# hguo/ftk

Hardware: NVIDIA B200
Metric: space_time_simplices_tested_per_sec (higher is better)
Workload: dtype f64+int64

## Files before the change

### ftk_b200/csrc/context.cpp

```cpp
#include <algorithm>
#include <cfloat>
#include <chrono>
#include <cmath>
#include <cstdio>
#include <cstdlib>
#include <cstring>
#include <deque>
#include <string>
#include <thread>
#include <atomic>
#include <vector>

#include <memory>
#include "kernels.h"
#include "online.h"
#include "curves.h"

using namespace ftkb;

namespace {

thread_local std::string g_create_error;

struct Layer {
  double *S = nullptr, *V = nullptr, *J = nullptr;
  bool ownS = false, ownV = false, ownJ = false;
  int slot = 0;
  bool res_pending = false;
  uint4 *cells = nullptr;
  bool cells_valid = false;
  bool cells_foreign = false;
};

}

template <class T>
struct NoInitAlloc : std::allocator<T> {
  template <class U> struct rebind { using other = NoInitAlloc<U>; };
  template <class U, class... A>
  void construct(U *q, A &&...a) {
    if constexpr (sizeof...(A) > 0) ::new ((void *)q) U(std::forward<A>(a)...);
  }
};
template <class T> using RawVec = std::vector<T, NoInitAlloc<T>>;

struct ftkb_ctx {
  ftkb_config cfg{};
  int n = 0;
  size_t nvert = 0;
  uint64_t ncore = 0;
  int n_ord = 0, n_int = 0;
  cudaStream_t stream = nullptr;
  cudaEvent_t ev[8] = {nullptr, nullptr, nullptr, nullptr, nullptr, nullptr, nullptr, nullptr};
  bool derive_timed = false;
  std::string error;

  bool slab = false;
  void *d_f32 = nullptr;
  size_t f32_cap = 0;
  std::deque<Layer> layers;
  std::vector<double *> freeS, freeV, freeJ;
  int current_timestep = 0;
  double resolution = DBL_MAX;
  double factor = 1.0;
  int nbits = 0;
  int next_slot = 0;
  int sm_count = 148;
  bool cellsV = true;
  bool keys2d = true;
  std::vector<uint4 *> freeCells;
  std::vector<uint4 *> exportedCells;
  size_t ncells = 0;
  bool fused3d = false;

  unsigned long long *d_scalars = nullptr;
  unsigned long long *h_scalars = nullptr;
  static constexpr int SLOT_WL = 8, SLOT_PT = 9, SLOT_UQ = 10, SLOT_POISON = 11, SLOT_WL2 = 12, SLOT_TICKET = 13, SLOT_POISON2 = 14, NSLOTS = 16;

  struct Pending {
    int ring = 0, evset = 0, pops = 0, nbits = 0, wl_sel = 0;
    uint64_t seq = 0, npts_before = 0, pt_cap = 0;
    bool has_next = false;
    int res_slots[2] = {-1, -1};
  };
  bool defer = true;
  std::deque<Pending> pend;
  std::deque<Layer> limbo;
  unsigned long long *h_ring = nullptr;
  static constexpr int RING = 4;
  uint64_t step_seq = 0;
  bool primed = false;
  int wl_sel = 0;
  cudaEvent_t dev[2][3] = {{nullptr, nullptr, nullptr}, {nullptr, nullptr, nullptr}};
  bool push_d2h_outstanding = false;
  uint64_t wl_hint = 1 << 16;
  cudaEvent_t ev_input = nullptr;
  cudaStream_t producer = nullptr;
  cudaStream_t stream2 = nullptr;
  cudaEvent_t ev_join = nullptr;
  bool debug_timing = false;
  double gap_ms = 0; uint64_t gap_n = 0, last_confirmed_seq = 0;
  std::vector<float> gaps, tl_scan_end, tl_test_end;
  cudaEvent_t dbg_prev = nullptr; bool dbg_prev_valid = false;
  double host_wait_us = 0, host_enq_us = 0; uint64_t host_wait_n = 0, host_enq_n = 0;
  bool last_test_overlapped = false;
  bool has_producer = false;

  unsigned long long *d_wl = nullptr;
  unsigned long long *d_wl2 = nullptr;
  int last_wl_sel = 0;
  uint64_t wl_cap = 0, last_wl = 0;
  ftkb_point *d_pts = nullptr;
  uint64_t pt_cap = 0, npts = 0;
  uint64_t max_step_points = 0;
  std::vector<ftkb_point *> retired_pts;

  struct Scratch { void *p = nullptr; size_t cap = 0; bool in_slab = false; };
  void *fz_slab = nullptr;
  size_t fz_slab_cap = 0;
  Scratch fz[14];
  void *grow_stage = nullptr;
  size_t grow_stage_cap = 0;

  bool sorted = false, traced = false;
  RawVec<ftkb_point> pts_sorted;
  ftkb_point *d_pts_sorted = nullptr;
  unsigned long long *d_keys_sorted = nullptr;
  uint64_t nsorted = 0;
  RawVec<uint64_t> labels;
  RawVec<int32_t> deg;
  std::vector<uint64_t> traj_off, traj_idx;
  std::vector<uint8_t> traj_loop, traj_complete;

  int coords_mode = 0, coords_ncomp = 0;
  double coords_bounds[6] = {0, 0, 0, 0, 0, 0};
  double *d_coords = nullptr;

  bool streaming = false;
  std::unique_ptr<ftkb::OnlineTracer> online;
  uint64_t grown = 0;
  bool grow_failed = false;

  ftkb_stats stats{};
};

#define CK(call)                                                                                         \
  do {                                                                                                   \
    cudaError_t e_ = (call);                                                                             \
    if (e_ != cudaSuccess) {                                                                             \
      c->error = std::string(#call) + ": " + cudaGetErrorString(e_);                                     \
      return e_ == cudaErrorMemoryAllocation ? FTKB_ERR_NOMEM : FTKB_ERR_CUDA;                           \
    }                                                                                                    \
  } while (0)

static int fail(ftkb_ctx *c, int code, const std::string &msg) {
  if (c) c->error = msg;
  else g_create_error = msg;
  return code;
}

static int scratch_plan(ftkb_ctx *c, const size_t *bytes, int nslots) {
  bool enough = true;
  size_t total = 0;
  for (int i = 0; i < nslots; i++)
    if (bytes[i]) { enough = enough && c->fz[i].cap >= bytes[i]; total += (bytes[i] + bytes[i] / 4 + 511) / 256 * 256; }
  if (enough) return FTKB_OK;
  for (int i = 0; i < (int)(sizeof(c->fz) / sizeof(c->fz[0])); i++)
    if (c->fz[i].in_slab) c->fz[i] = ftkb_ctx::Scratch{};
  if (c->fz_slab_cap < total) {
    cudaFree(c->fz_slab);
    c->fz_slab = nullptr; c->fz_slab_cap = 0;
    if (cudaMalloc(&c->fz_slab, total) != cudaSuccess) { cudaGetLastError(); c->error = "finalize: out of device memory"; return FTKB_ERR_NOMEM; }
    c->fz_slab_cap = total;
  }
  size_t off = 0;
  for (int i = 0; i < nslots; i++) {
    if (!bytes[i]) continue;
    ftkb_ctx::Scratch &s = c->fz[i];
    if (s.p && !s.in_slab) cudaFree(s.p);
    const size_t sz = (bytes[i] + bytes[i] / 4 + 511) / 256 * 256;
    s.p = (char *)c->fz_slab + off; s.cap = sz; s.in_slab = true;
    off += sz;
  }
  return FTKB_OK;
}

static int scratch(ftkb_ctx *c, int i, size_t bytes, void **out) {
  ftkb_ctx::Scratch &s = c->fz[i];
  if (s.cap < bytes) {
    if (!s.in_slab) cudaFree(s.p);
    s.in_slab = false;
    s.p = nullptr; s.cap = 0;
    const size_t want = bytes + bytes / 4 + 256;
    if (cudaMalloc(&s.p, want) != cudaSuccess) { cudaGetLastError(); c->error = "finalize: out of device memory"; return FTKB_ERR_NOMEM; }
    s.cap = want;
  }
  *out = s.p;
  return FTKB_OK;
}

static int check_launch(ftkb_ctx *c, const char *what) {
  cudaError_t e = cudaGetLastError();
  if (e != cudaSuccess) return fail(c, FTKB_ERR_CUDA, std::string(what) + ": " + cudaGetErrorString(e));
  return FTKB_OK;
}

extern "C" int ftkb_abi_version(void) { return FTKB_ABI_VERSION; }

extern "C" int ftkb_device_count(void) {
  int n = 0;
  if (cudaGetDeviceCount(&n) != cudaSuccess) { cudaGetLastError(); return 0; }
  int usable = 0;
  for (int i = 0; i < n; i++) {
    cudaDeviceProp prop;
    if (cudaGetDeviceProperties(&prop, i) == cudaSuccess && prop.major == 10) usable++;
  }
  return usable;
}

extern "C" const char *ftkb_last_error(const ftkb_ctx *c) { return c ? c->error.c_str() : g_create_error.c_str(); }

static void release_layer(ftkb_ctx *c, Layer &l) {
  if (l.ownS && l.S) c->freeS.push_back(l.S);
  if (l.ownV && l.V) c->freeV.push_back(l.V);
  if (l.ownJ && l.J) c->freeJ.push_back(l.J);
  if (l.cells && !l.cells_foreign) c->freeCells.push_back(l.cells);
  l = Layer();
}

static void fill_trace_params(const ftkb_ctx *c, TraceParams &tp);
static int drain(ftkb_ctx *c);

extern "C" void ftkb_destroy(ftkb_ctx *c) {
  if (!c) return;
  if (c->debug_timing && c->gaps.size() > 8) {
    auto med = [](std::vector<float> v) { std::sort(v.begin(), v.end()); return 1e3 * v[v.size() / 2]; };
    std::fprintf(stderr, "[ftkb] deferred steps, relative to the previous scan's end (medians over %zu): scan starts +%.1f us, ends +%.1f us, test ends +%.1f us\n",
                 c->gaps.size(), med(c->gaps), med(c->tl_scan_end), med(c->tl_test_end));
    std::fprintf(stderr, "[ftkb] host: %.1f us to enqueue a step, %.1f us blocked per confirmation (avg over %llu / %llu)\n",
                 c->host_enq_us / std::max<uint64_t>(1, c->host_enq_n), c->host_wait_us / std::max<uint64_t>(1, c->host_wait_n),
                 (unsigned long long)c->host_enq_n, (unsigned long long)c->host_wait_n);
  }
  cudaSetDevice(c->cfg.device);
  if (c->stream) cudaStreamSynchronize(c->stream);
  for (auto &l : c->layers) release_layer(c, l);
  for (auto &l : c->limbo) release_layer(c, l);
  c->limbo.clear();
  for (auto *p : c->freeS) cudaFree(p);
  for (auto *p : c->freeV) cudaFree(p);
  for (auto *p : c->freeJ) cudaFree(p);
  for (auto *p : c->freeCells) cudaFree(p);
  for (auto *p : c->exportedCells) cudaFree(p);
  cudaFree(c->d_scalars);
  if (c->h_scalars) cudaFreeHost(c->h_scalars);
  if (c->grow_stage) cudaFreeHost(c->grow_stage);
  for (ftkb_point *q : c->retired_pts) cudaFree(q);
  if (c->h_ring) cudaFreeHost(c->h_ring);
  for (auto &es : c->dev) for (auto &e : es) if (e) cudaEventDestroy(e);
  if (c->ev_input) cudaEventDestroy(c->ev_input);
  if (c->dbg_prev) cudaEventDestroy(c->dbg_prev);
  cudaFree(c->d_wl);
  cudaFree(c->d_wl2);
  if (c->stream2) { cudaStreamSynchronize(c->stream2); cudaStreamDestroy(c->stream2); }
  if (c->ev_join) cudaEventDestroy(c->ev_join);
  cudaFree(c->d_pts);
  cudaFree(c->d_coords);
  cudaFree(c->d_f32);
  for (auto &s : c->fz) if (!s.in_slab) cudaFree(s.p);
  cudaFree(c->fz_slab);
  for (auto &e : c->ev) if (e) cudaEventDestroy(e);
  if (c->stream) cudaStreamDestroy(c->stream);
  delete c;
}

extern "C" int ftkb_create(const ftkb_config *cfg, ftkb_ctx **out) {
  if (!cfg || !out) return fail(nullptr, FTKB_ERR_INVALID, "ftkb_create: null argument");
  *out = nullptr;
  if (cfg->abi_version != FTKB_ABI_VERSION) return fail(nullptr, FTKB_ERR_INVALID, "ftkb_create: ABI version mismatch");
  if (cfg->nd != 2 && cfg->nd != 3) return fail(nullptr, FTKB_ERR_INVALID, "ftkb_create: nd must be 2 or 3");
  const int n = cfg->nd;
  for (int j = 0; j < n; j++) {
    if (cfg->dims[j] < 2) return fail(nullptr, FTKB_ERR_INVALID, "ftkb_create: array dims must be >= 2");
    if (cfg->lb[j] < 0 || cfg->ub[j] > cfg->dims[j] - 1 || cfg->lb[j] > cfg->ub[j])
      return fail(nullptr, FTKB_ERR_INVALID, "ftkb_create: domain must lie inside the array");
  }
  if (cfg->start_timestep < 0) return fail(nullptr, FTKB_ERR_INVALID, "ftkb_create: start_timestep must be >= 0");
  int ndev = 0;
  if (cudaGetDeviceCount(&ndev) != cudaSuccess || ndev == 0) {
    cudaGetLastError();
    return fail(nullptr, FTKB_ERR_NO_DEVICE, "ftkb_create: no CUDA device (this engine has no CPU fallback)");
  }
  if (cfg->device < 0 || cfg->device >= ndev) return fail(nullptr, FTKB_ERR_NO_DEVICE, "ftkb_create: device ordinal out of range");
  cudaDeviceProp prop;
  if (cudaGetDeviceProperties(&prop, cfg->device) != cudaSuccess || prop.major != 10)
    return fail(nullptr, FTKB_ERR_NO_DEVICE, "ftkb_create: device is not compute capability 10.x (kernels are built for sm_100a only)");

  if (cfg->slab_global_dim != 0) {
    if (n != 3) return fail(nullptr, FTKB_ERR_INVALID, "ftkb_create: spatial slabs are 3D (along z)");
    if (cfg->slab_offset < 0 || cfg->slab_offset + cfg->dims[2] > cfg->slab_global_dim || cfg->slab_global_lb < 0 ||
        cfg->slab_global_ub >= cfg->slab_global_dim || cfg->slab_global_lb > cfg->slab_global_ub ||
        cfg->slab_offset + cfg->lb[2] < cfg->slab_global_lb || cfg->slab_offset + cfg->ub[2] > cfg->slab_global_ub)
      return fail(nullptr, FTKB_ERR_INVALID, "ftkb_create: the slab does not lie inside the whole array / domain");
  }
  ftkb_ctx *c = new ftkb_ctx();
  c->cfg = *cfg;
  c->slab = cfg->slab_global_dim != 0;
  c->sm_count = prop.multiProcessorCount > 0 ? prop.multiProcessorCount : 148;
  {
    const char *e = std::getenv("FTKB_SCAN3D");
    c->fused3d = n == 3 && cfg->vector_source == FTKB_SOURCE_DERIVED && cfg->robust_detection && cfg->dims[0] % 2 == 0 &&
                 !(e && std::string(e) == "plain");
    const char *ev = std::getenv("FTKB_VSCAN");
    c->cellsV = cfg->vector_source == FTKB_SOURCE_GIVEN && !(n == 3 && !cfg->robust_detection) && (n == 2 || cfg->dims[0] % 2 == 0) &&
                !(ev && std::string(ev) == "twolayer");
    const char *e2 = std::getenv("FTKB_SCAN2D");
    c->keys2d = !(e2 && std::string(e2) == "f32");
  }
  c->n = n;
  c->nvert = (size_t)cfg->dims[0] * cfg->dims[1] * (n == 3 ? cfg->dims[2] : 1);
  c->ncore = 1;
  for (int j = 0; j < n; j++) c->ncore *= (uint64_t)(cfg->ub[j] - cfg->lb[j] + 1);
  {
    const long double cap = 18446744073709551616.0L / (long double)(1ull << (KEY_TIME_BITS + KEY_TYPE_BITS));
    long double key_cells = (long double)c->ncore;
    if (c->slab) key_cells = key_cells / (long double)(cfg->ub[2] - cfg->lb[2] + 1) * (long double)(cfg->slab_global_ub - cfg->slab_global_lb + 1);
    if (key_cells >= cap) { delete c; return fail(nullptr, FTKB_ERR_OVERFLOW, "ftkb_create: domain too large for 64-bit element ids"); }
  }
  const MeshTables &mt = mesh_tables(n + 1);
  c->n_ord = (int)mt.ordinal_types[n].size();
  c->n_int = (int)mt.interval_types[n].size();
  c->current_timestep = cfg->start_timestep;
  c->resolution = cfg->resolution_init > 0 ? cfg->resolution_init : DBL_MAX;

  auto bail = [&](const std::string &m, int code) { g_create_error = m; ftkb_destroy(c); return code; };
  cudaError_t e;
  if ((e = cudaSetDevice(cfg->device)) != cudaSuccess) return bail(std::string("cudaSetDevice: ") + cudaGetErrorString(e), FTKB_ERR_CUDA);
  if ((e = cudaStreamCreateWithFlags(&c->stream, cudaStreamNonBlocking)) != cudaSuccess) return bail(std::string("cudaStreamCreate: ") + cudaGetErrorString(e), FTKB_ERR_CUDA);
  for (auto &ev : c->ev)
    if ((e = cudaEventCreate(&ev)) != cudaSuccess) return bail(std::string("cudaEventCreate: ") + cudaGetErrorString(e), FTKB_ERR_CUDA);
  if ((e = cudaMalloc(&c->d_scalars, sizeof(unsigned long long) * ftkb_ctx::NSLOTS)) != cudaSuccess) return bail("cudaMalloc(scalars) failed", FTKB_ERR_NOMEM);
  if ((e = cudaMallocHost(&c->h_scalars, sizeof(unsigned long long) * ftkb_ctx::NSLOTS)) != cudaSuccess) return bail("cudaMallocHost failed", FTKB_ERR_NOMEM);
  std::memset(c->h_scalars, 0, sizeof(unsigned long long) * ftkb_ctx::NSLOTS);
  if ((e = cudaHostAlloc(&c->h_ring, sizeof(unsigned long long) * 8 * ftkb_ctx::RING, cudaHostAllocMapped | cudaHostAllocPortable)) != cudaSuccess) return bail("cudaHostAlloc(ring) failed", FTKB_ERR_NOMEM);
  std::memset(c->h_ring, 0xff, sizeof(unsigned long long) * 8 * ftkb_ctx::RING);
  for (auto &es : c->dev)
    for (auto &ev : es)
      if ((e = cudaEventCreate(&ev)) != cudaSuccess) return bail(std::string("cudaEventCreate: ") + cudaGetErrorString(e), FTKB_ERR_CUDA);
  if ((e = cudaEventCreateWithFlags(&c->ev_input, cudaEventDisableTiming)) != cudaSuccess) return bail(std::string("cudaEventCreate: ") + cudaGetErrorString(e), FTKB_ERR_CUDA);
  if (const char *d = std::getenv("FTKB_DEFER")) c->defer = std::string(d) != "0";
  cudaMemsetAsync(c->d_scalars, 0, sizeof(unsigned long long) * ftkb_ctx::NSLOTS, c->stream);
  c->wl_cap = std::max<uint64_t>(1 << 16, c->ncore / 64);
  if (const char *w = std::getenv("FTKB_WL_CAP")) c->wl_cap = std::max<uint64_t>(1, std::strtoull(w, nullptr, 10));
  if ((e = cudaMalloc(&c->d_wl, sizeof(unsigned long long) * c->wl_cap)) != cudaSuccess) return bail("cudaMalloc(worklist) failed", FTKB_ERR_NOMEM);
  if ((e = cudaMalloc(&c->d_wl2, sizeof(unsigned long long) * c->wl_cap)) != cudaSuccess) return bail("cudaMalloc(worklist) failed", FTKB_ERR_NOMEM);
  {
    int lo = 0, hi = 0;
    cudaDeviceGetStreamPriorityRange(&lo, &hi);
    if ((e = cudaStreamCreateWithPriority(&c->stream2, cudaStreamNonBlocking, hi)) != cudaSuccess) return bail(std::string("cudaStreamCreate: ") + cudaGetErrorString(e), FTKB_ERR_CUDA);
    if ((e = cudaEventCreateWithFlags(&c->ev_join, cudaEventDisableTiming)) != cudaSuccess) return bail(std::string("cudaEventCreate: ") + cudaGetErrorString(e), FTKB_ERR_CUDA);
    if (const char *o = std::getenv("FTKB_DEBUG_TIMING")) c->debug_timing = std::string(o) == "1";
    if (c->debug_timing) cudaEventCreate(&c->dbg_prev);
  }
  c->pt_cap = cfg->point_capacity ? cfg->point_capacity : (1 << 20);
  if ((e = cudaMalloc(&c->d_pts, sizeof(ftkb_point) * c->pt_cap)) != cudaSuccess) return bail("cudaMalloc(points) failed", FTKB_ERR_NOMEM);
  DeviceMeshTables t2, t3;
  fill_device_tables(3, &t2);
  fill_device_tables(4, &t3);
  upload_mesh_tables(t2, t3);
  init_kernel_attributes();
  if ((e = cudaStreamSynchronize(c->stream)) != cudaSuccess) return bail(std::string("init: ") + cudaGetErrorString(e), FTKB_ERR_CUDA);
  *out = c;
  return FTKB_OK;
}

static int take_buffer(ftkb_ctx *c, std::vector<double *> &pool, size_t count, double **out) {
  if (pool.empty() && !c->pend.empty() && c->layers.size() + c->limbo.size() >= 4) {
    const int rc = drain(c);
    if (rc) return rc;
  }
  if (!pool.empty()) { *out = pool.back(); pool.pop_back(); return FTKB_OK; }
  CK(cudaMalloc(out, sizeof(double) * count));
  return FTKB_OK;
}

static int queue_resolution(ftkb_ctx *c, Layer &l, bool fused_in_gradient) {
  if (!fused_in_gradient) launch_resolution(l.V, (uint64_t)c->nvert * c->n, c->d_scalars + l.slot, c->stream);
  c->stats.kernel_launches += fused_in_gradient ? 0 : 1;
  CK(cudaMemcpyAsync(c->h_scalars + l.slot, c->d_scalars + l.slot, sizeof(unsigned long long), cudaMemcpyDeviceToHost, c->stream));
  c->stats.d2h_bytes += 8;
  c->push_d2h_outstanding = true;
  return check_launch(c, "resolution");
}

static int derive_layer(ftkb_ctx *c, Layer &l) {
  bool fused = false;
  if (!l.V && c->cfg.vector_source == FTKB_SOURCE_DERIVED && l.S && (c->n == 2 || (c->fused3d && (uintptr_t)l.S % 16 == 0))) {
    l.res_pending = true;
    c->h_scalars[l.slot] = ~0ull;
    return FTKB_OK;
  }
  if (l.V && c->cellsV && c->cfg.vector_source == FTKB_SOURCE_GIVEN && (uintptr_t)l.V % 16 == 0) {
    l.res_pending = true;
    c->h_scalars[l.slot] = ~0ull;
    return FTKB_OK;
  }
  CK(cudaMemsetAsync(c->d_scalars + l.slot, 0xff, sizeof(unsigned long long), c->stream));
  if (!l.V && c->cfg.vector_source == FTKB_SOURCE_DERIVED && l.S) {
    int rc = take_buffer(c, c->freeV, c->nvert * c->n, &l.V);
    if (rc) return rc;
    l.ownV = true;
    CK(cudaEventRecord(c->ev[4], c->stream));
    launch_gradient(c->n, l.S, l.V, c->cfg.dims[0], c->cfg.dims[1], c->n == 3 ? c->cfg.dims[2] : 1, c->d_scalars + l.slot, c->stream);
    CK(cudaEventRecord(c->ev[5], c->stream));
    c->derive_timed = true;
    c->stats.kernel_launches++;
    fused = true;
  }
  if (l.V) {
    int rc = queue_resolution(c, l, fused);
    if (rc) return rc;
  }
  return check_launch(c, "derive");
}

static int new_layer(ftkb_ctx *c, Layer &l) {
  if (c->layers.size() >= 4) return fail(c, FTKB_ERR_INVALID, "push: more than 4 resident snapshots (call advance_timestep)");
  l.slot = c->next_slot;
  c->next_slot = (c->next_slot + 1) % 8;
  return FTKB_OK;
}

extern "C" int ftkb_push_snapshot(ftkb_ctx *c, const double *scalar, const double *vector, const double *jacobian, int where) {
  if (!c) return FTKB_ERR_INVALID;
  if (where < FTKB_MEM_HOST || where > FTKB_MEM_DEVICE_BORROW) return fail(c, FTKB_ERR_INVALID, "push: bad memory kind");
  if (c->cfg.scalar_source == FTKB_SOURCE_GIVEN && !scalar) return fail(c, FTKB_ERR_INVALID, "push: scalar field is GIVEN but no scalar array was passed");
  if (c->cfg.vector_source == FTKB_SOURCE_GIVEN && !vector) return fail(c, FTKB_ERR_INVALID, "push: vector field is GIVEN but no vector array was passed");
  if (c->cfg.vector_source == FTKB_SOURCE_DERIVED && !vector && !scalar) return fail(c, FTKB_ERR_INVALID, "push: vector field is DERIVED but no scalar array was passed");
  if (c->cfg.jacobian_source == FTKB_SOURCE_GIVEN && !jacobian) return fail(c, FTKB_ERR_INVALID, "push: jacobian is GIVEN but no jacobian array was passed");
  CK(cudaSetDevice(c->cfg.device));
  for (const double *q : {scalar, vector, jacobian})
    if ((uintptr_t)q % 8 != 0) return fail(c, FTKB_ERR_INVALID, "push: arrays must be 8-byte aligned");
  Layer l;
  int rc = new_layer(c, l);
  if (rc) return rc;
  if (where != FTKB_MEM_HOST && c->has_producer) {
    CK(cudaEventRecord(c->ev_input, c->producer));
    CK(cudaStreamWaitEvent(c->stream, c->ev_input, 0));
  }
  const size_t nS = c->nvert, nV = c->nvert * c->n, nJ = c->nvert * c->n * c->n;
  auto ingest = [&](const double *src, size_t count, std::vector<double *> &pool, double **dst, bool *own) -> int {
    if (!src) return FTKB_OK;
    if (where == FTKB_MEM_DEVICE_BORROW) { *dst = const_cast<double *>(src); *own = false; return FTKB_OK; }
    int r = take_buffer(c, pool, count, dst);
    if (r) return r;
    *own = true;
    CK(cudaMemcpyAsync(*dst, src, sizeof(double) * count, where == FTKB_MEM_HOST ? cudaMemcpyHostToDevice : cudaMemcpyDeviceToDevice, c->stream));
    if (where == FTKB_MEM_HOST) c->stats.h2d_bytes += sizeof(double) * count;
    return FTKB_OK;
  };
  if ((rc = ingest(scalar, nS, c->freeS, &l.S, &l.ownS))) { release_layer(c, l); return rc; }
  if ((rc = ingest(vector, nV, c->freeV, &l.V, &l.ownV))) { release_layer(c, l); return rc; }
  if ((rc = ingest(jacobian, nJ, c->freeJ, &l.J, &l.ownJ))) { release_layer(c, l); return rc; }
  if ((rc = derive_layer(c, l))) { release_layer(c, l); return rc; }
  if (where != FTKB_MEM_DEVICE_BORROW) CK(cudaStreamSynchronize(c->stream));
  c->layers.push_back(l);
  return FTKB_OK;
}

extern "C" int ftkb_push_snapshot_f32(ftkb_ctx *c, const float *scalar, const float *vector) {
  if (!c) return FTKB_ERR_INVALID;
  if (c->cfg.jacobian_source == FTKB_SOURCE_GIVEN) return fail(c, FTKB_ERR_INVALID, "push_snapshot_f32: a GIVEN jacobian has no float32 form");
  if (c->cfg.scalar_source == FTKB_SOURCE_GIVEN && !scalar) return fail(c, FTKB_ERR_INVALID, "push: scalar field is GIVEN but no scalar array was passed");
  if (c->cfg.vector_source == FTKB_SOURCE_GIVEN && !vector) return fail(c, FTKB_ERR_INVALID, "push: vector field is GIVEN but no vector array was passed");
  if (c->cfg.vector_source == FTKB_SOURCE_DERIVED && !vector && !scalar) return fail(c, FTKB_ERR_INVALID, "push: vector field is DERIVED but no scalar array was passed");
  if ((uintptr_t)scalar % 4 != 0 || (uintptr_t)vector % 4 != 0) return fail(c, FTKB_ERR_INVALID, "push: arrays must be 4-byte aligned");
  CK(cudaSetDevice(c->cfg.device));
  Layer l;
  int rc = new_layer(c, l);
  if (rc) return rc;
  const size_t nS = c->nvert, nV = c->nvert * c->n;
  const size_t need = 4 * std::max(scalar ? nS : 0, vector ? nV : 0) + 16;
  if (c->f32_cap < need) {
    cudaFree(c->d_f32);
    c->d_f32 = nullptr; c->f32_cap = 0;
    CK(cudaMalloc(&c->d_f32, need));
    c->f32_cap = need;
  }
  auto ingest = [&](const float *src, size_t count, std::vector<double *> &pool, double **dst, bool *own) -> int {
    if (!src) return FTKB_OK;
    const int r = take_buffer(c, pool, count, dst);
    if (r) return r;
    *own = true;
    CK(cudaMemcpyAsync(c->d_f32, src, 4 * count, cudaMemcpyHostToDevice, c->stream));
    launch_widen_f32(static_cast<const float *>(c->d_f32), *dst, count, c->stream);
    c->stats.h2d_bytes += 4 * count;
    c->stats.kernel_launches++;
    return check_launch(c, "widen");
  };
  if ((rc = ingest(scalar, nS, c->freeS, &l.S, &l.ownS))) { release_layer(c, l); return rc; }
  if ((rc = ingest(vector, nV, c->freeV, &l.V, &l.ownV))) { release_layer(c, l); return rc; }
  if ((rc = derive_layer(c, l))) { release_layer(c, l); return rc; }
  CK(cudaStreamSynchronize(c->stream));
  c->layers.push_back(l);
  return FTKB_OK;
}

extern "C" int ftkb_set_producer_stream(ftkb_ctx *c, void *stream, int enable) {
  if (!c) return FTKB_ERR_INVALID;
  c->producer = reinterpret_cast<cudaStream_t>(stream);
  c->has_producer = enable != 0;
  return FTKB_OK;
}

extern "C" int ftkb_push_synthetic(ftkb_ctx *c, int kind, const double *params, int nparams, double t) {
  if (!c) return FTKB_ERR_INVALID;
  if (nparams < 0 || nparams > 8 || (nparams && !params)) return fail(c, FTKB_ERR_INVALID, "push_synthetic: bad params");
  const bool vector_kind = kind == FTKB_SYN_DOUBLE_GYRE || kind == FTKB_SYN_ABC || kind == FTKB_SYN_TORNADO;
  const bool ok2 = kind == FTKB_SYN_WOVEN || kind == FTKB_SYN_DOUBLE_GYRE || kind == FTKB_SYN_MERGER;
  if (kind < 0 || kind > FTKB_SYN_TORNADO || (ok2 && c->n != 2) || ((kind == FTKB_SYN_ABC || kind == FTKB_SYN_TORNADO) && c->n != 3))
    return fail(c, FTKB_ERR_INVALID, "push_synthetic: generator does not match the context's dimensionality");
  if (vector_kind ? c->cfg.vector_source != FTKB_SOURCE_GIVEN : c->cfg.scalar_source != FTKB_SOURCE_GIVEN)
    return fail(c, FTKB_ERR_INVALID, "push_synthetic: generator kind does not match the configured field sources");
  CK(cudaSetDevice(c->cfg.device));
  double p[8] = {0, 0, 0, 0, 0, 0, 0, 0};
  for (int i = 0; i < nparams; i++) p[i] = params[i];
  Layer l;
  int rc = new_layer(c, l);
  if (rc) return rc;
  double **dst = vector_kind ? &l.V : &l.S;
  if ((rc = take_buffer(c, vector_kind ? c->freeV : c->freeS, vector_kind ? c->nvert * c->n : c->nvert, dst))) { release_layer(c, l); return rc; }
  (vector_kind ? l.ownV : l.ownS) = true;
  launch_synthetic(kind, c->n, c->cfg.dims[0], c->cfg.dims[1], c->n == 3 ? c->cfg.dims[2] : 1, p, t, *dst, c->stream,
                   c->slab ? c->cfg.slab_offset : 0, c->slab ? c->cfg.slab_global_dim : 0);
  c->stats.kernel_launches++;
  if ((rc = derive_layer(c, l))) { release_layer(c, l); return rc; }
  c->layers.push_back(l);
  return FTKB_OK;
}

static int resolve_pending(ftkb_ctx *c, Layer &l);

static double slot_value(const ftkb_ctx *c, int slot) {
  double v;
  std::memcpy(&v, c->h_scalars + slot, 8);
  return (c->h_scalars[slot] >> 52) >= 0x7ff ? DBL_MAX : v;
}

extern "C" int ftkb_last_layer_resolution(ftkb_ctx *c, double *res) {
  if (!c || !res) return FTKB_ERR_INVALID;
  if (c->layers.empty()) return fail(c, FTKB_ERR_INVALID, "last_layer_resolution: no resident snapshot");
  CK(cudaSetDevice(c->cfg.device));
  { const int rc = drain(c); if (rc) return rc; }
  Layer &l = c->layers.back();
  if (l.res_pending) {
    const int rc = resolve_pending(c, l);
    if (rc) return rc;
  }
  CK(cudaStreamSynchronize(c->stream));
  *res = (l.V || l.S) ? slot_value(c, l.slot) : DBL_MAX;
  return FTKB_OK;
}

extern "C" int ftkb_set_resolution(ftkb_ctx *c, double res) {
  if (!c) return FTKB_ERR_INVALID;
  if (!c->pend.empty()) {
    cudaSetDevice(c->cfg.device);
    const int rc = drain(c);
    if (rc) return rc;
  }
  if (res > 0 && res < c->resolution) c->resolution = res;
  return FTKB_OK;
}

extern "C" int ftkb_current_timestep(const ftkb_ctx *c, int32_t *t) {
  if (!c || !t) return FTKB_ERR_INVALID;
  *t = c->current_timestep;
  return FTKB_OK;
}

static int grow_points(ftkb_ctx *c, uint64_t need) {
  uint64_t cap = c->pt_cap;
  while (cap < need) cap *= 2;
  ftkb_point *np = nullptr;
  CK(cudaMalloc(&np, sizeof(ftkb_point) * cap));
  CK(cudaMemcpyAsync(np, c->d_pts, sizeof(ftkb_point) * c->npts, cudaMemcpyDeviceToDevice, c->stream));
  CK(cudaStreamSynchronize(c->stream));
  cudaFree(c->d_pts);
  c->d_pts = np;
  c->pt_cap = cap;
  return FTKB_OK;
}

static int nbits_of(double resolution) {
  int nbits = (int)std::ceil(std::log2(1.0 / resolution));
  const int minbits = 8, maxbits = 21;
  return std::max(minbits, std::min(nbits, maxbits));
}

extern "C" int ftkb_set_coords(ftkb_ctx *c, int mode, const double *data, uint64_t n) {
  if (!c || mode < FTKB_COORDS_SIMPLE || mode > FTKB_COORDS_EXPLICIT || (mode != FTKB_COORDS_SIMPLE && !data)) return FTKB_ERR_INVALID;
  if (c->slab && mode != FTKB_COORDS_SIMPLE) return fail(c, FTKB_ERR_INVALID, "set_coords: physical coordinates are not available on a spatial slab");
  CK(cudaSetDevice(c->cfg.device));
  const uint64_t W = c->cfg.dims[0], H = c->cfg.dims[1], D = c->n == 3 ? c->cfg.dims[2] : 0;
  if (mode == FTKB_COORDS_BOUNDS && n != 2u * c->n) return fail(c, FTKB_ERR_INVALID, "set_coords: bounds take 2 * nd values");
  if (mode == FTKB_COORDS_RECTILINEAR && n != W + H + D) return fail(c, FTKB_ERR_INVALID, "set_coords: rectilinear coordinates take W + H [+ D] values");
  if (mode == FTKB_COORDS_EXPLICIT && (n % (W * H) != 0 || n / (W * H) < (c->n == 3 ? 3u : 2u)))
    return fail(c, FTKB_ERR_INVALID, "set_coords: explicit coordinates are (ncomp, W, H) with ncomp >= nd");
  { const int rc = drain(c); if (rc) return rc; }
  CK(cudaStreamSynchronize(c->stream));
  cudaFree(c->d_coords);
  c->d_coords = nullptr;
  c->coords_mode = mode;
  c->coords_ncomp = mode == FTKB_COORDS_EXPLICIT ? (int)(n / (W * H)) : 0;
  if (mode == FTKB_COORDS_BOUNDS) for (uint64_t k = 0; k < n; k++) c->coords_bounds[k] = data[k];
  if (mode == FTKB_COORDS_RECTILINEAR || mode == FTKB_COORDS_EXPLICIT) {
    CK(cudaMalloc(&c->d_coords, 8 * n));
    CK(cudaMemcpy(c->d_coords, data, 8 * n, cudaMemcpyHostToDevice));
    c->stats.h2d_bytes += 8 * n;
  }
  return FTKB_OK;
}

static void fill_sweep_geometry(const ftkb_ctx *c, SweepParams &p) {
  p.coords_mode = c->coords_mode;
  p.coords_ncomp = c->coords_ncomp;
  for (int k = 0; k < 6; k++) p.coords_bounds[k] = c->coords_bounds[k];
  p.coords = c->d_coords;
  p.nd = c->n;
  p.sm_count = c->sm_count;
  p.W = c->cfg.dims[0]; p.H = c->cfg.dims[1]; p.D = c->n == 3 ? c->cfg.dims[2] : 1;
  for (int j = 0; j < 3; j++) {
    const bool used = j < c->n;
    p.lb[j] = used ? c->cfg.lb[j] : 0;
    p.ub[j] = used ? c->cfg.ub[j] : 0;
    p.nc[j] = p.ub[j] - p.lb[j] + 1;
    p.vmax[j] = p.ub[j];
    p.voff[j] = 0; p.rank_lb[j] = p.lb[j]; p.rank_nc[j] = p.nc[j];
  }
  for (int j = 0; j < 3; j++)
    p.res_thr[j] = res_threshold_key(c->resolution, c->n == 2 ? (double)(c->cfg.dims[j < 2 ? j : 0] - 1) : 0.5);
  if (c->slab) {
    p.voff[2] = c->cfg.slab_offset;
    p.rank_lb[2] = c->cfg.slab_global_lb;
    p.rank_nc[2] = c->cfg.slab_global_ub - c->cfg.slab_global_lb + 1;
  }
}

static void fused2d_decomposition(const ftkb_ctx *c, SweepParams &p, bool aligned) {
  if (aligned) {
    const int R = SCAN2D_CELL_ROWS;
    p.nsx = std::max(1, (p.W + 7 * 62 - 1) / (7 * 62));
    const int64_t want = std::max<int64_t>(1, (8 * (int64_t)c->sm_count * 3) / p.nsx);
    p.rows = std::max(2 * R, (int)((p.H + want - 1) / want));
    p.rows = (p.rows + R - 1) / R * R;
    p.rows = std::min(p.rows, 64 * R);
  } else {
    p.nsx = std::max(1, (p.W - 1 + 59) / 60);
    int64_t nsy = (2 * (int64_t)c->sm_count * 2 * 8) / p.nsx;
    nsy = std::max<int64_t>(1, std::min<int64_t>(nsy, (p.H + 31) / 32));
    p.rows = (int)((p.H + nsy - 1) / nsy);
  }
  p.nsy = (p.H + p.rows - 1) / p.rows;
  p.nsz = 1;
}

static void fused3d_decomposition(const ftkb_ctx *c, SweepParams &p) {
  p.nsx = (p.W + F3_STRIDE - 1) / F3_STRIDE;
  p.nsy = (p.H + F3_TROWS - 1) / F3_TROWS;
  const int64_t tiles = (int64_t)p.nsx * p.nsy;
  const int64_t slots = 2 * (int64_t)c->sm_count;
  const int64_t nsz = std::max<int64_t>(1, std::min<int64_t>((6 * slots + tiles - 1) / tiles, std::max(1, p.D / 16)));
  p.rows = (int)((p.D + nsz - 1) / nsz);
  p.rows = std::min(p.rows, 63);
  p.nsz = (p.D + p.rows - 1) / p.rows;
}

static void vcells_decomposition(const ftkb_ctx *c, SweepParams &p) {
  if (c->n == 3) { fused3d_decomposition(c, p); return; }
  const int R = VSCAN2D_CELL_ROWS;
  p.nsx = std::max(1, (p.W + 61) / 62);
  const int64_t want = std::max<int64_t>(1, (6 * (int64_t)c->sm_count * 16) / p.nsx);
  p.rows = std::max(2 * R, (int)((p.H + want - 1) / want));
  p.rows = (p.rows + R - 1) / R * R;
  p.nsy = (p.H + p.rows - 1) / p.rows;
  p.nsz = 1;
}

static int ensure_cells(ftkb_ctx *c, Layer &l, const SweepParams &p) {
  if (l.cells) return FTKB_OK;
  if (!c->ncells) c->ncells = c->n == 3 ? scan3d_cells_per_layer(p) : (p.fused ? scan2d_cells_per_layer(p) : vscan2d_cells_per_layer(p));
  if (!c->freeCells.empty()) { l.cells = c->freeCells.back(); c->freeCells.pop_back(); return FTKB_OK; }
  CK(cudaMalloc(&l.cells, sizeof(uint4) * c->ncells));
  return FTKB_OK;
}

static int materialise_gradient(ftkb_ctx *c, Layer &l) {
  if (l.V || !l.S) return FTKB_OK;
  CK(cudaMemsetAsync(c->d_scalars + l.slot, 0xff, sizeof(unsigned long long), c->stream));
  int rc = take_buffer(c, c->freeV, c->nvert * c->n, &l.V);
  if (rc) return rc;
  l.ownV = true;
  l.cells_valid = false;
  launch_gradient(c->n, l.S, l.V, c->cfg.dims[0], c->cfg.dims[1], c->n == 3 ? c->cfg.dims[2] : 1, c->d_scalars + l.slot, c->stream);
  c->stats.kernel_launches++;
  l.res_pending = false;
  CK(cudaMemcpyAsync(c->h_scalars + l.slot, c->d_scalars + l.slot, sizeof(unsigned long long), cudaMemcpyDeviceToHost, c->stream));
  c->stats.d2h_bytes += 8;
  c->push_d2h_outstanding = true;
  return check_launch(c, "gradient");
}

static int abandon_fused3d(ftkb_ctx *c) {
  c->fused3d = false;
  for (Layer &l : c->layers) {
    const int rc = materialise_gradient(c, l);
    if (rc) return rc;
  }
  CK(cudaStreamSynchronize(c->stream));
  return FTKB_OK;
}

static bool rows_aligned16(const ftkb_ctx *c, const double *a, const double *b) {
  return (c->cfg.dims[0] % 2 == 0) && ((uintptr_t)a % 16 == 0) && (!b || (uintptr_t)b % 16 == 0);
}

static int resolve_pending(ftkb_ctx *c, Layer &l) {
  c->primed = false;
  CK(cudaMemsetAsync(c->d_scalars + l.slot, 0xff, sizeof(unsigned long long), c->stream));
  if (l.V) {
    if (c->cellsV && c->cfg.vector_source == FTKB_SOURCE_GIVEN && (uintptr_t)l.V % 16 == 0 && !l.cells_valid) {
      SweepParams p{};
      fill_sweep_geometry(c, p);
      p.fused = 0;
      p.has_next = 0;
      p.nbits = c->nbits ? c->nbits : 8;
      p.L[0].V = l.V; p.L[1].V = l.V;
      p.res_slot[0] = c->d_scalars + l.slot;
      p.poison = c->d_scalars + ftkb_ctx::SLOT_POISON;
      p.wl_count = c->d_scalars + ftkb_ctx::SLOT_WL;
      p.wl = c->d_wl; p.wl_cap = 0;
      vcells_decomposition(c, p);
      const int rc = ensure_cells(c, l, p);
      if (rc) return rc;
      CK(cudaMemsetAsync(p.poison, 0, sizeof(unsigned long long), c->stream));
      p.sum_mode = SUM_BUILD; p.build_layer = 0; p.sum_out = l.cells;
      launch_vscan_cells(p, c->stream);
      c->stats.kernel_launches++;
      CK(cudaMemcpyAsync(c->h_scalars + l.slot, c->d_scalars + l.slot, sizeof(unsigned long long), cudaMemcpyDeviceToHost, c->stream));
      CK(cudaMemcpyAsync(c->h_scalars + ftkb_ctx::SLOT_POISON, p.poison, sizeof(unsigned long long), cudaMemcpyDeviceToHost, c->stream));
      c->stats.d2h_bytes += 16;
      const int rl = check_launch(c, "resolution (vector cells)");
      if (rl) return rl;
      CK(cudaStreamSynchronize(c->stream));
      if (!c->h_scalars[ftkb_ctx::SLOT_POISON]) {
        l.cells_valid = true;
        l.res_pending = false;
        return FTKB_OK;
      }
      c->cellsV = false;
      for (Layer &x : c->layers) x.cells_valid = false;
      CK(cudaMemsetAsync(c->d_scalars + l.slot, 0xff, sizeof(unsigned long long), c->stream));
    }
    l.res_pending = false;
    return queue_resolution(c, l, false);
  }
  SweepParams p{};
  fill_sweep_geometry(c, p);
  p.lb[1] = 1; p.ub[1] = 0;
  p.fused = 1;
  p.has_next = 0;
  p.thrp_f = 1.f; p.thr2_f = 1.f; p.lim_f = 0.f;
  p.L[0].S = l.S; p.L[1].S = l.S;
  p.res_slot[0] = c->d_scalars + l.slot;
  p.wl_count = c->d_scalars + ftkb_ctx::SLOT_WL;
  p.wl = c->d_wl; p.wl_cap = 0;
  if (c->n == 3) {
    p.nbits = 8;
    p.poison = c->d_scalars + ftkb_ctx::SLOT_POISON;
    if (!encode_scalar_tmap3d(l.S, p.W, p.H, p.D, &p.tmap[0])) { c->fused3d = false; return materialise_gradient(c, l); }
    p.tmap[1] = p.tmap[0];
    CK(cudaMemsetAsync(p.poison, 0, sizeof(unsigned long long), c->stream));
    fused3d_decomposition(c, p);
    fill_sweep_geometry(c, p);
    int rc = ensure_cells(c, l, p);
    if (rc) return rc;
    p.sum_mode = SUM_BUILD; p.build_layer = 0; p.sum_out = l.cells;
    launch_scan3d_cells(p, c->stream);
    l.cells_valid = true;
    c->stats.kernel_launches++;
    CK(cudaMemcpyAsync(c->h_scalars + l.slot, c->d_scalars + l.slot, sizeof(unsigned long long), cudaMemcpyDeviceToHost, c->stream));
    CK(cudaMemcpyAsync(c->h_scalars + ftkb_ctx::SLOT_POISON, p.poison, sizeof(unsigned long long), cudaMemcpyDeviceToHost, c->stream));
    c->stats.d2h_bytes += 16;
    rc = check_launch(c, "resolution (fused 3D)");
    if (rc) return rc;
    CK(cudaStreamSynchronize(c->stream));
    l.res_pending = false;
    if (c->h_scalars[ftkb_ctx::SLOT_POISON]) return abandon_fused3d(c);
    return FTKB_OK;
  }
  const bool aligned = rows_aligned16(c, l.S, nullptr);
  fused2d_decomposition(c, p, aligned);
  if (aligned) {
    fill_sweep_geometry(c, p);
    int rc = ensure_cells(c, l, p);
    if (rc) return rc;
    p.sum_mode = SUM_BUILD; p.build_layer = 0; p.sum_out = l.cells;
    launch_scan2d_cells(p, c->stream);
    l.cells_valid = true;
  } else {
    launch_scan(p, c->stream);
  }
  c->stats.kernel_launches++;
  CK(cudaMemcpyAsync(c->h_scalars + l.slot, c->d_scalars + l.slot, sizeof(unsigned long long), cudaMemcpyDeviceToHost, c->stream));
  c->stats.d2h_bytes += 8;
  l.res_pending = false;
  c->push_d2h_outstanding = true;
  return check_launch(c, "resolution (fused)");
}

static int wait_grow(ftkb_ctx *c) {
  return c->grow_failed ? FTKB_ERR_NOMEM : FTKB_OK;
}

static int grow_trajectories(ftkb_ctx *c) {
  const uint64_t n = c->npts - c->grown;
  if (n >= 0xffffffffull) return fail(c, FTKB_ERR_OVERFLOW, "more than 2^32 punctured simplices in one step");
  { const int rc = wait_grow(c); if (rc) return rc; }
  const size_t per = 8 + 4 * 9 + 1;
  if (n && c->grow_stage_cap < per * n) {
    if (c->grow_stage) cudaFreeHost(c->grow_stage);
  for (ftkb_point *q : c->retired_pts) cudaFree(q);
    c->grow_stage = nullptr; c->grow_stage_cap = 0;
    const size_t want = per * (n + n / 2 + 1024);
    if (cudaMallocHost(&c->grow_stage, want) != cudaSuccess) { cudaGetLastError(); return fail(c, FTKB_ERR_NOMEM, "streaming grow step: out of page-locked memory"); }
    c->grow_stage_cap = want;
  }
  uint64_t *h_keys = (uint64_t *)c->grow_stage;
  uint32_t *h_nb = (uint32_t *)(h_keys + n);
  uint8_t *h_cnt = (uint8_t *)(h_nb + 9 * n);
  uint64_t nu = n;
  if (n) {
    TraceParams tp{};
    fill_trace_params(c, tp);
    unsigned long long *k0 = nullptr, *k1 = nullptr;
    uint32_t *i0 = nullptr, *i1 = nullptr, *d_nb = nullptr;
    uint8_t *d_cnt = nullptr;
    void *temp = nullptr;
    unsigned long long *d_nu = c->d_scalars + ftkb_ctx::SLOT_UQ;
    { int rs = scratch(c, 0, 8 * n, (void **)&k0); if (!rs) rs = scratch(c, 1, 8 * n, (void **)&k1); if (!rs) rs = scratch(c, 2, 4 * n, (void **)&i0);
      if (!rs) rs = scratch(c, 3, 4 * n, (void **)&i1);
      if (!rs) rs = scratch(c, 10, 4 * 9 * n, (void **)&d_nb); if (!rs) rs = scratch(c, 11, n, (void **)&d_cnt); if (rs) return rs; }
    CK(cudaEventRecord(c->ev[0], c->stream));
    launch_point_keys(c->d_pts + c->grown, n, tp, k0, i0, c->stream);
    const size_t tb = std::max(sort_pairs_u64(nullptr, 0, k0, k1, i0, i1, n, c->stream), unique_by_key_u64(nullptr, 0, k1, i1, k0, i0, d_nu, n, c->stream));
    { const int rs = scratch(c, 4, tb, &temp); if (rs) return rs; }
    sort_pairs_u64(temp, tb, k0, k1, i0, i1, n, c->stream);
    unique_by_key_u64(temp, tb, k1, i1, k0, i0, d_nu, n, c->stream);
    tp.keys = k0;
    launch_batch_neighbors(tp, d_nu, n, c->d_pts + c->grown, i0, nullptr, d_nb, d_cnt, c->stream);
    CK(cudaEventRecord(c->ev[1], c->stream));
    CK(cudaMemcpyAsync(c->h_scalars + ftkb_ctx::SLOT_UQ, d_nu, 8, cudaMemcpyDeviceToHost, c->stream));
    CK(cudaMemcpyAsync(h_keys, k0, 8 * n, cudaMemcpyDeviceToHost, c->stream));
    CK(cudaMemcpyAsync(h_nb, d_nb, 4 * 9 * n, cudaMemcpyDeviceToHost, c->stream));
    CK(cudaMemcpyAsync(h_cnt, d_cnt, n, cudaMemcpyDeviceToHost, c->stream));
    CK(cudaStreamSynchronize(c->stream));
    { const int rc = check_launch(c, "streaming grow step (batch preparation)"); if (rc) return rc; }
    nu = c->h_scalars[ftkb_ctx::SLOT_UQ];
    float ms = 0;
    CK(cudaEventElapsedTime(&ms, c->ev[0], c->ev[1]));
    c->stats.ms_finalize_device += ms;
    c->stats.kernel_launches += 4;
    c->stats.d2h_bytes += per * n + 8;
  }
  try {
    const auto t0 = std::chrono::steady_clock::now();
    if (n) c->online->grow_sorted(nullptr, h_keys, (uint32_t)nu, h_nb, h_cnt);
    else c->online->grow(nullptr, 0);
    c->stats.ms_finalize_host += std::chrono::duration<double, std::milli>(std::chrono::steady_clock::now() - t0).count();
  }
  catch (const std::bad_alloc &) { c->grow_failed = true; return fail(c, FTKB_ERR_NOMEM, "streaming grow step: out of memory (trajectories are incomplete)"); }
  catch (const std::exception &e) { c->grow_failed = true; return fail(c, FTKB_ERR_INVALID, std::string("streaming grow step: ") + e.what()); }
  c->grown = c->npts;
  c->traced = false;
  return FTKB_OK;
}

extern "C" int ftkb_set_streaming_trajectories(ftkb_ctx *c, int enable) {
  if (!c) return FTKB_ERR_INVALID;
  if (c->stats.scan_launches || c->npts) return fail(c, FTKB_ERR_INVALID, "set_streaming_trajectories: call it before the first update_timestep");
  if (c->slab && enable) return fail(c, FTKB_ERR_INVALID, "set_streaming_trajectories: not available on a spatial slab");
  c->streaming = enable != 0;
  c->grow_failed = false;
  c->online.reset(c->streaming ? new ftkb::OnlineTracer(c->n, c->cfg.lb, c->cfg.ub) : nullptr);
  c->grown = 0;
  return FTKB_OK;
}

static int update_impl(ftkb_ctx *c, bool allow_defer);
static int abandon_fused3d(ftkb_ctx *c);

static void absorb_resolutions(ftkb_ctx *c, const ftkb_ctx::Pending &pd) {
  const volatile unsigned long long *r = c->h_ring + 8 * pd.ring;
  if (r[5] != pd.seq) return;
  for (int k = 0; k < 2; k++)
    if (pd.res_slots[k] >= 0) {
      c->h_scalars[pd.res_slots[k]] = r[3 + k];
      c->resolution = std::min(c->resolution, slot_value(c, pd.res_slots[k]));
    }
}

static int replay(ftkb_ctx *c, bool poison) {
  CK(cudaStreamSynchronize(c->stream));
  CK(cudaStreamSynchronize(c->stream2));
  for (const auto &pd : c->pend) absorb_resolutions(c, pd);
  std::vector<int> pops;
  for (const auto &pd : c->pend) pops.push_back(pd.pops);
  const uint64_t npts0 = c->pend.front().npts_before;
  c->pend.clear();
  c->primed = false;
  while (!c->limbo.empty()) {
    c->layers.push_front(c->limbo.back());
    c->limbo.pop_back();
    c->current_timestep--;
  }
  c->npts = npts0;
  c->stats.points = npts0;
  c->sorted = false;
  c->traced = false;
  if (poison) {
    if (c->cfg.vector_source == FTKB_SOURCE_GIVEN) {
      c->cellsV = false;
      for (Layer &l : c->layers) l.cells_valid = false;
    } else if (c->n == 3) {
      const int rc = abandon_fused3d(c);
      if (rc) return rc;
    } else {
      c->keys2d = false;
      for (Layer &l : c->layers) l.cells_valid = false;
    }
  }
  c->stats.sweeps_repeated += pops.size();
  for (size_t i = 0; i < pops.size(); i++) {
    const int rc = update_impl(c, false);
    if (rc) return rc;
    for (int j = 0; j < pops[i] && !c->layers.empty(); j++) {
      release_layer(c, c->layers.front());
      c->layers.pop_front();
      c->current_timestep++;
    }
  }
  return FTKB_OK;
}

static int confirm_front(ftkb_ctx *c) {
  const ftkb_ctx::Pending pd = c->pend.front();
  const auto tw0 = std::chrono::steady_clock::now();
  CK(cudaEventSynchronize(c->dev[pd.evset][2]));
  if (c->debug_timing) { c->host_wait_us += std::chrono::duration<double, std::micro>(std::chrono::steady_clock::now() - tw0).count(); c->host_wait_n++; }
  const volatile unsigned long long *r = c->h_ring + 8 * pd.ring;
  if (r[5] != pd.seq) return fail(c, FTKB_ERR_CUDA, "deferred step: the test kernel did not publish its counters");
  const uint64_t nwl = r[0], npt = r[1];
  const bool poison = r[2] != 0;
  c->stats.d2h_bytes += 48;
  absorb_resolutions(c, pd);
  const bool stale = nbits_of(c->resolution) != pd.nbits;
  if (poison || stale || nwl > c->wl_cap || npt > pd.pt_cap) return replay(c, poison);
  c->nbits = pd.nbits;
  c->factor = (double)(uint64_t)(1 << pd.nbits);
  float ms_scan = 0, ms_test = 0;
  CK(cudaEventElapsedTime(&ms_scan, c->dev[pd.evset][0], c->dev[pd.evset][1]));
  CK(cudaEventElapsedTime(&ms_test, c->dev[pd.evset][1], c->dev[pd.evset][2]));
  c->stats.ms_scan += ms_scan; c->stats.ms_test += ms_test; c->stats.last_ms_scan = ms_scan;
  if (c->debug_timing) {
    float s0 = 0, s1 = 0, s2 = 0;
    if (c->dbg_prev_valid && cudaEventElapsedTime(&s0, c->dbg_prev, c->dev[pd.evset][0]) == cudaSuccess &&
        cudaEventElapsedTime(&s1, c->dbg_prev, c->dev[pd.evset][1]) == cudaSuccess && cudaEventElapsedTime(&s2, c->dbg_prev, c->dev[pd.evset][2]) == cudaSuccess) {
      c->gaps.push_back(s0);
      c->tl_scan_end.push_back(s1);
      c->tl_test_end.push_back(s2);
    } else cudaGetLastError();
    std::swap(c->dbg_prev, c->dev[pd.evset][1]);
    c->dbg_prev_valid = true;
  }
  c->stats.scan_launches++;
  c->stats.cells_scanned += c->ncore;
  c->stats.cells_refined += nwl;
  c->last_wl = nwl;
  c->last_wl_sel = pd.wl_sel;
  c->wl_hint = nwl;
  c->stats.simplices_tested += c->ncore * (uint64_t)(c->n_ord + (pd.has_next ? c->n_int : 0));
  if (npt != c->npts) { c->sorted = false; c->traced = false; }
  if (npt > c->npts) c->max_step_points = std::max(c->max_step_points, npt - c->npts);
  c->npts = npt;
  c->stats.points = npt;
  for (int j = 0; j < pd.pops && !c->limbo.empty(); j++) {
    release_layer(c, c->limbo.front());
    c->limbo.pop_front();
  }
  c->pend.pop_front();
  if (!c->pend.empty()) c->pend.front().npts_before = c->npts;
  return FTKB_OK;
}

static int drain(ftkb_ctx *c) {
  while (!c->pend.empty()) {
    const int rc = confirm_front(c);
    if (rc) return rc;
  }
  if (!c->retired_pts.empty()) {
    CK(cudaStreamSynchronize(c->stream));
    for (ftkb_point *q : c->retired_pts) cudaFree(q);
    c->retired_pts.clear();
  }
  return FTKB_OK;
}

static int grow_points_ahead(ftkb_ctx *c) {
  const uint64_t per = c->max_step_points;
  if (!per) return FTKB_OK;
  const uint64_t need = c->npts + (c->pend.size() + 2) * (per + per / 2);
  if (need <= c->pt_cap) return FTKB_OK;
  uint64_t cap = 4 * c->pt_cap;
  while (cap < need) cap *= 2;
  if (cap >= 0xffffffffull) return FTKB_OK;
  ftkb_point *np = nullptr;
  if (cudaMalloc(&np, sizeof(ftkb_point) * cap) != cudaSuccess) { cudaGetLastError(); return FTKB_OK; }
  if (!c->pend.empty()) CK(cudaStreamWaitEvent(c->stream, c->dev[c->pend.back().evset][2], 0));
  CK(cudaMemcpyAsync(np, c->d_pts, sizeof(ftkb_point) * c->pt_cap, cudaMemcpyDeviceToDevice, c->stream));
  c->retired_pts.push_back(c->d_pts);
  c->d_pts = np;
  c->pt_cap = cap;
  return FTKB_OK;
}

static int test_grid(const ftkb_ctx *c) {
  const uint64_t cpb = c->n == 2 ? 10 : 2;
  const uint64_t want = (c->wl_hint * 2 + 256 + cpb - 1) / cpb;
  return (int)std::max<uint64_t>(8, std::min<uint64_t>(want, (uint64_t)c->sm_count * 8));
}

extern "C" int ftkb_update_timestep(ftkb_ctx *c) {
  if (!c) return FTKB_ERR_INVALID;
  return update_impl(c, c->defer);
}

static int update_impl(ftkb_ctx *c, bool allow_defer) {
  if (c->layers.empty()) return fail(c, FTKB_ERR_INVALID, "update_timestep: no snapshot has been pushed");
  CK(cudaSetDevice(c->cfg.device));
  bool may_defer = allow_defer && !c->streaming && !c->push_d2h_outstanding;
  if (!may_defer) { const int rc = drain(c); if (rc) return rc; }
  if (c->n == 3 && c->fused3d && c->cfg.vector_source == FTKB_SOURCE_DERIVED) {
    bool anyV = false, anyS = false;
    for (const Layer &l : c->layers) { anyV = anyV || l.V; anyS = anyS || (!l.V && l.S); }
    if (anyV && anyS) c->fused3d = false;
  }
  if (c->n == 3 && !c->fused3d) {
    bool any = false;
    for (Layer &l : c->layers)
      if (!l.V && l.S && c->cfg.vector_source == FTKB_SOURCE_DERIVED) {
        int rc = drain(c);
        if (!rc) rc = materialise_gradient(c, l);
        if (rc) return rc;
        any = true;
      }
    if (any) { CK(cudaStreamSynchronize(c->stream)); may_defer = false; }
  }
  const bool fused = !c->layers[0].V && c->layers[0].S && c->cfg.vector_source == FTKB_SOURCE_DERIVED && (c->n == 2 || c->fused3d);
  if (!c->layers[0].V && !fused) return fail(c, FTKB_ERR_INVALID, "update_timestep: the snapshot has no vector field");
  if (c->current_timestep + 1 >= (1 << KEY_TIME_BITS)) return fail(c, FTKB_ERR_OVERFLOW, "update_timestep: timestep exceeds the element id range");
  if (c->push_d2h_outstanding) {
    CK(cudaStreamSynchronize(c->stream));
    c->push_d2h_outstanding = false;
  }
  if (c->derive_timed) {
    float ms = 0;
    if (cudaEventElapsedTime(&ms, c->ev[4], c->ev[5]) == cudaSuccess) { c->stats.ms_derive += ms; c->stats.last_ms_derive = ms; }
    else cudaGetLastError();
    c->derive_timed = false;
  }
  const bool has_next = c->layers.size() >= 2;
  if (has_next && !c->layers[1].V && !(fused && c->layers[1].S)) return fail(c, FTKB_ERR_INVALID, "update_timestep: the next snapshot has no vector field");
  bool vcells = !fused && c->cellsV && c->layers[0].V && c->cfg.vector_source == FTKB_SOURCE_GIVEN;
  for (size_t k = 0; vcells && k < (has_next ? 2u : 1u); k++)
    if (!c->layers[k].V || (uintptr_t)c->layers[k].V % 16 != 0) vcells = false;
  {
    bool any = false;
    for (size_t k = 0; k < c->layers.size(); k++) {
      Layer &l = c->layers[k];
      if (l.V && l.res_pending && !(vcells && k < 2)) {
        int rc = drain(c);
        if (!rc) rc = resolve_pending(c, l);
        if (rc) return rc;
        any = true;
      }
    }
    if (any) { CK(cudaStreamSynchronize(c->stream)); c->push_d2h_outstanding = false; may_defer = false; }
  }
  if (has_next && fused && c->layers[1].V) return fail(c, FTKB_ERR_INVALID, "update_timestep: resident snapshots mix derived and given vector fields");
  for (const Layer &l : c->layers)
    if ((l.V || l.S) && !l.res_pending) c->resolution = std::min(c->resolution, slot_value(c, l.slot));
  int nbits = nbits_of(c->resolution);

  SweepParams p{};
  fill_sweep_geometry(c, p);
  p.t = c->current_timestep;
  p.has_next = has_next;
  p.no_filter = (c->n == 3 && !c->cfg.robust_detection);
  p.scalar_source = c->layers[0].S ? c->cfg.scalar_source : FTKB_SOURCE_NONE;
  p.jacobian_source = c->cfg.jacobian_source;
  p.jacobian_symmetric = c->cfg.jacobian_symmetric;
  p.derived_symmetric = c->cfg.vector_source == FTKB_SOURCE_DERIVED;
  p.robust = c->cfg.robust_detection;
  p.compute_degrees = c->cfg.compute_degrees;
  p.use_type_filter = c->cfg.use_type_filter;
  p.type_filter = c->cfg.type_filter;
  Layer *lay[2] = {&c->layers[0], &c->layers[has_next ? 1 : 0]};
  for (int k = 0; k < 2; k++) { p.L[k].S = lay[k]->S; p.L[k].V = lay[k]->V; p.L[k].J = lay[k]->J; }
  if (has_next && p.scalar_source != FTKB_SOURCE_NONE && !c->layers[1].S) return fail(c, FTKB_ERR_INVALID, "update_timestep: the next snapshot has no scalar field");
  p.fused = fused;
  p.poison = c->d_scalars + ftkb_ctx::SLOT_POISON;
  const bool aligned = rows_aligned16(c, lay[0]->S, lay[1]->S);
  if (fused && c->n == 3) {
    if (!encode_scalar_tmap3d(lay[0]->S, p.W, p.H, p.D, &p.tmap[0]) || !encode_scalar_tmap3d(lay[1]->S, p.W, p.H, p.D, &p.tmap[1])) {
      int rc = drain(c);
      if (!rc) rc = abandon_fused3d(c);
      return rc ? rc : update_impl(c, allow_defer);
    }
    fused3d_decomposition(c, p);
  } else if (fused) {
    fused2d_decomposition(c, p, aligned);
  } else if (vcells) {
    vcells_decomposition(c, p);
  } else {
    p.nsx = (p.nc[0] + 30) / 31;
    if (c->n == 2) {
      p.rows = 64;
      p.nsy = (p.nc[1] + p.rows - 1) / p.rows;
      p.nsz = 1;
    } else {
      p.rows = 32;
      p.nsy = (p.nc[1] + 14) / 15;
      p.nsz = (p.nc[2] + p.rows - 1) / p.rows;
    }
  }
  p.keys2d = c->keys2d;
  p.pt_count = c->d_scalars + ftkb_ctx::SLOT_PT;
  p.ticket = c->d_scalars + ftkb_ctx::SLOT_TICKET;
  p.test_blocks = test_grid(c);
  const bool cells_path = vcells || (fused && (c->n == 3 || aligned));
  void (*launch_cells)(const SweepParams &, cudaStream_t) = vcells ? launch_vscan_cells : (c->n == 3 ? launch_scan3d_cells : launch_scan2d_cells);

  if (may_defer && cells_path && lay[0]->cells_valid && !p.no_filter) {
    if (has_next && !lay[1]->cells) {
      const int rc0 = ensure_cells(c, *lay[1], p);
      if (rc0) return rc0;
    }
    p.nbits = nbits;
    p.factor = (double)(uint64_t)(1 << nbits);
    p.thrp_f = (float)((1.0 / p.factor) * (1.0 + 1.0 / 1048576.0));
    p.thr2_f = (float)(2.0 / p.factor);
    p.lim_f = (float)(0.999 * 4.5e18 / (p.factor * p.factor));
    const auto te0 = std::chrono::steady_clock::now();
    ftkb_ctx::Pending pd;
    pd.seq = ++c->step_seq;
    pd.ring = (int)(pd.seq % ftkb_ctx::RING);
    pd.evset = (int)(pd.seq & 1);
    pd.has_next = has_next;
    pd.nbits = nbits;
    pd.npts_before = c->npts;
    p.res_slot[0] = p.res_slot[1] = nullptr;
    for (int k = 0; k < (has_next ? 2 : 1); k++)
      if (lay[k]->res_pending) {
        p.res_slot[k] = c->d_scalars + lay[k]->slot;
        pd.res_slots[k] = lay[k]->slot;
        lay[k]->res_pending = false;
      }
    pd.wl_sel = c->wl_sel;
    p.wl = c->wl_sel ? c->d_wl2 : c->d_wl; p.wl_cap = c->wl_cap;
    { const int rcg = grow_points_ahead(c); if (rcg) return rcg; }
    p.pts = c->d_pts; p.pt_cap = c->pt_cap;
    pd.pt_cap = c->pt_cap;
    p.wl_count = c->d_scalars + (c->wl_sel ? ftkb_ctx::SLOT_WL2 : ftkb_ctx::SLOT_WL);
    p.poison = c->d_scalars + (c->wl_sel ? ftkb_ctx::SLOT_POISON2 : ftkb_ctx::SLOT_POISON);
    p.step_out = c->h_ring + 8 * pd.ring;
    p.step_seq = pd.seq;
    auto slot_at = [&](size_t idx) { return idx < c->layers.size() ? c->layers[idx].slot : (int)((c->next_slot + (idx - c->layers.size())) % 8); };
    p.res_reset = c->d_scalars + slot_at(3);
    if (!c->primed) {
      c->h_scalars[ftkb_ctx::SLOT_WL] = 0;
      c->h_scalars[ftkb_ctx::SLOT_WL2] = 0;
      c->h_scalars[ftkb_ctx::SLOT_PT] = c->npts;
      c->h_scalars[ftkb_ctx::SLOT_UQ] = 0;
      c->h_scalars[ftkb_ctx::SLOT_POISON] = 0;
      c->h_scalars[ftkb_ctx::SLOT_POISON2] = 0;
      c->h_scalars[ftkb_ctx::SLOT_TICKET] = 0;
      if (c->layers.size() < 3) c->h_scalars[slot_at(2)] = ~0ull;
      CK(cudaMemcpyAsync(c->d_scalars, c->h_scalars, 15 * sizeof(unsigned long long), cudaMemcpyHostToDevice, c->stream));
    }
    CK(cudaEventRecord(c->dev[pd.evset][0], c->stream));
    p.sum_in[0] = lay[0]->cells; p.sum_in[1] = lay[1]->cells;
    if (has_next && !lay[1]->cells_valid) {
      p.sum_mode = SUM_BUILD_TEST2; p.build_layer = 1; p.sum_out = lay[1]->cells;
      lay[1]->cells_valid = true;
    } else {
      p.sum_mode = has_next ? SUM_TEST2 : SUM_TEST1;
    }
    launch_cells(p, c->stream);
    CK(cudaEventRecord(c->dev[pd.evset][1], c->stream));
    const bool overlap = c->wl_hint < 100000;
    if (!overlap && c->last_test_overlapped && !c->pend.empty())
      CK(cudaStreamWaitEvent(c->stream, c->dev[c->pend.back().evset][2], 0));
    c->last_test_overlapped = overlap;
    cudaStream_t ts = overlap ? c->stream2 : c->stream;
    if (overlap) CK(cudaStreamWaitEvent(c->stream2, c->dev[pd.evset][1], 0));
    launch_test(p, ts);
    CK(cudaEventRecord(c->dev[pd.evset][2], ts));
    c->stats.kernel_launches += 2;
    const int rc = check_launch(c, "sweep");
    if (rc) return rc;
    c->pend.push_back(pd);
    c->primed = true;
    c->wl_sel ^= 1;
    if (c->debug_timing) { c->host_enq_us += std::chrono::duration<double, std::micro>(std::chrono::steady_clock::now() - te0).count(); c->host_enq_n++; }
    while (c->pend.size() > 1) {
      const int rc2 = confirm_front(c);
      if (rc2) return rc2;
    }
    return FTKB_OK;
  }
  { const int rc = drain(c); if (rc) return rc; }
  c->primed = false;
  p.wl_count = c->d_scalars + ftkb_ctx::SLOT_WL;
  p.step_out = nullptr;

  for (int attempt = 0; attempt < 12; attempt++) {
    p.nbits = nbits;
    p.factor = (double)(uint64_t)(1 << nbits);
    p.thrp_f = (float)((1.0 / p.factor) * (1.0 + 1.0 / 1048576.0));
    p.thr2_f = (float)(2.0 / p.factor);
    p.lim_f = (float)(0.999 * 4.5e18 / (p.factor * p.factor));
    p.res_slot[0] = p.res_slot[1] = nullptr;
    bool pending = false;
    if (fused || vcells)
      for (int k = 0; k < (has_next ? 2 : 1); k++)
        if (lay[k]->res_pending) { p.res_slot[k] = c->d_scalars + lay[k]->slot; pending = true; }
    p.wl = c->d_wl; p.wl_cap = c->wl_cap;
    p.pts = c->d_pts; p.pt_cap = c->pt_cap;
    p.test_blocks = test_grid(c);
    c->h_scalars[ftkb_ctx::SLOT_WL] = 0;
    c->h_scalars[ftkb_ctx::SLOT_PT] = c->npts;
    c->h_scalars[ftkb_ctx::SLOT_UQ] = 0;
    c->h_scalars[ftkb_ctx::SLOT_POISON] = 0;
    c->h_scalars[ftkb_ctx::SLOT_WL2] = 0;
    c->h_scalars[ftkb_ctx::SLOT_TICKET] = 0;
    c->h_scalars[ftkb_ctx::SLOT_POISON2] = 0;
    CK(cudaMemcpyAsync(c->d_scalars, c->h_scalars, 15 * sizeof(unsigned long long), cudaMemcpyHostToDevice, c->stream));
    CK(cudaEventRecord(c->ev[0], c->stream));
    if (cells_path) {
      int rc0 = ensure_cells(c, *lay[0], p);
      if (!rc0 && has_next) rc0 = ensure_cells(c, *lay[1], p);
      if (rc0) return rc0;
      p.sum_in[0] = lay[0]->cells; p.sum_in[1] = lay[1]->cells;
      if (!lay[0]->cells_valid) {
        p.sum_mode = has_next ? SUM_BUILD : SUM_BUILD_TEST1; p.build_layer = 0; p.sum_out = lay[0]->cells;
        launch_cells(p, c->stream);
        lay[0]->cells_valid = true;
        if (has_next) {
          c->stats.kernel_launches++;
          p.sum_mode = lay[1]->cells_valid ? SUM_TEST2 : SUM_BUILD_TEST2; p.build_layer = 1; p.sum_out = lay[1]->cells;
          launch_cells(p, c->stream);
          lay[1]->cells_valid = true;
        }
      } else if (has_next && !lay[1]->cells_valid) {
        p.sum_mode = SUM_BUILD_TEST2; p.build_layer = 1; p.sum_out = lay[1]->cells;
        launch_cells(p, c->stream);
        lay[1]->cells_valid = true;
      } else {
        p.sum_mode = has_next ? SUM_TEST2 : SUM_TEST1;
        launch_cells(p, c->stream);
      }
    } else {
      launch_scan(p, c->stream);
    }
    CK(cudaEventRecord(c->ev[1], c->stream));
    launch_test(p, c->stream);
    CK(cudaEventRecord(c->ev[2], c->stream));
    c->stats.kernel_launches += 2;
    int rc = check_launch(c, "sweep");
    if (rc) return rc;
    if (pending) {
      CK(cudaMemcpyAsync(c->h_scalars, c->d_scalars, 12 * sizeof(unsigned long long), cudaMemcpyDeviceToHost, c->stream));
      c->stats.d2h_bytes += 64;
    } else {
      CK(cudaMemcpyAsync(c->h_scalars + ftkb_ctx::SLOT_WL, c->d_scalars + ftkb_ctx::SLOT_WL, 32, cudaMemcpyDeviceToHost, c->stream));
    }
    CK(cudaStreamSynchronize(c->stream));
    c->stats.d2h_bytes += 32;
    if (vcells && c->h_scalars[ftkb_ctx::SLOT_POISON]) {
      c->stats.sweeps_repeated++;
      c->cellsV = false;
      for (Layer &l : c->layers) l.cells_valid = false;
      return update_impl(c, false);
    }
    if (fused && c->n == 3 && c->h_scalars[ftkb_ctx::SLOT_POISON]) {
      c->stats.sweeps_repeated++;
      const int rc2 = abandon_fused3d(c);
      return rc2 ? rc2 : update_impl(c, false);
    }
    if (fused && c->n == 2 && c->h_scalars[ftkb_ctx::SLOT_POISON]) {
      c->stats.sweeps_repeated++;
      c->keys2d = false;
      for (Layer &l : c->layers) l.cells_valid = false;
      return update_impl(c, false);
    }
    float ms_scan = 0, ms_test = 0;
    CK(cudaEventElapsedTime(&ms_scan, c->ev[0], c->ev[1]));
    CK(cudaEventElapsedTime(&ms_test, c->ev[1], c->ev[2]));
    c->stats.ms_scan += ms_scan; c->stats.ms_test += ms_test; c->stats.last_ms_scan = ms_scan;
    c->stats.scan_launches++;
    if (pending) {
      for (int k = 0; k < (has_next ? 2 : 1); k++)
        if (lay[k]->res_pending) {
          lay[k]->res_pending = false;
          c->resolution = std::min(c->resolution, slot_value(c, lay[k]->slot));
        }
      const int nb = nbits_of(c->resolution);
      if (nb != nbits) {
        nbits = nb;
        c->stats.sweeps_repeated++;
        continue;
      }
    }
    const uint64_t nwl = c->h_scalars[ftkb_ctx::SLOT_WL], npt = c->h_scalars[ftkb_ctx::SLOT_PT];
    c->wl_hint = std::min<uint64_t>(nwl, c->wl_cap);
    if (nwl > c->wl_cap) {
      cudaFree(c->d_wl); cudaFree(c->d_wl2);
      c->d_wl = c->d_wl2 = nullptr;
      c->wl_cap = nwl + nwl / 8 + 1024;
      CK(cudaMalloc(&c->d_wl, sizeof(unsigned long long) * c->wl_cap));
      CK(cudaMalloc(&c->d_wl2, sizeof(unsigned long long) * c->wl_cap));
      c->wl_hint = nwl;
      c->stats.sweeps_repeated++;
      continue;
    }
    if (npt > c->pt_cap) {
      int rc2 = grow_points(c, npt);
      if (rc2) return rc2;
      c->stats.sweeps_repeated++;
      continue;
    }
    c->nbits = nbits;
    c->factor = p.factor;
    c->stats.cells_scanned += c->ncore;
    c->stats.cells_refined += nwl;
    c->last_wl = nwl;
    c->last_wl_sel = 0;
    c->stats.simplices_tested += c->ncore * (uint64_t)(c->n_ord + (has_next ? c->n_int : 0));
    if (npt != c->npts) { c->sorted = false; c->traced = false; }
    c->npts = npt;
    c->stats.points = npt;
    if (c->streaming && has_next) { const int rc2 = grow_trajectories(c); if (rc2) return rc2; }
    return FTKB_OK;
  }
  return fail(c, FTKB_ERR_CUDA, "update_timestep: buffers kept overflowing");
}

extern "C" int ftkb_advance_timestep(ftkb_ctx *c) {
  if (!c) return FTKB_ERR_INVALID;
  const int rc = ftkb_update_timestep(c);
  if (rc) return rc;
  if (!c->layers.empty()) {
    if (!c->pend.empty()) {
      c->limbo.push_back(c->layers.front());
      c->pend.back().pops++;
    } else {
      release_layer(c, c->layers.front());
    }
    c->layers.pop_front();
  }
  c->current_timestep++;
  return FTKB_OK;
}

static void fill_trace_params(const ftkb_ctx *c, TraceParams &tp) {
  tp.nd = c->n;
  for (int j = 0; j < 3; j++) {
    const bool used = j < c->n;
    tp.lb[j] = used ? c->cfg.lb[j] : 0;
    tp.ub[j] = used ? c->cfg.ub[j] : 0;
  }
  if (c->slab) { tp.lb[2] = c->cfg.slab_global_lb; tp.ub[2] = c->cfg.slab_global_ub; }
  tp.ny = tp.ub[1] - tp.lb[1] + 1;
  tp.nz = tp.ub[2] - tp.lb[2] + 1;
}

struct Laps {
  bool on;
  const char *what;
  std::chrono::steady_clock::time_point t;
  std::string line;
  Laps(bool enabled, const char *w) : on(enabled), what(w), t(std::chrono::steady_clock::now()) {}
  void lap(const char *name) {
    if (!on) return;
    const auto now = std::chrono::steady_clock::now();
    char buf[96];
    std::snprintf(buf, sizeof(buf), " %s=%.2f", name, std::chrono::duration<double, std::milli>(now - t).count());
    line += buf;
    t = now;
  }
  ~Laps() { if (on) std::fprintf(stderr, "[ftkb timing] %s (ms):%s\n", what, line.c_str()); }
};

static int ensure_sorted(ftkb_ctx *c) {
  CK(cudaSetDevice(c->cfg.device));
  { const int rc = drain(c); if (rc) return rc; }
  if (c->sorted) return FTKB_OK;
  c->d_pts_sorted = nullptr;
  c->d_keys_sorted = nullptr;
  c->pts_sorted.clear();
  c->nsorted = 0;
  const uint64_t n = c->npts;
  if (n == 0) { c->sorted = true; return FTKB_OK; }
  if (n >= 0xffffffffull) return fail(c, FTKB_ERR_OVERFLOW, "more than 2^32 punctured simplices");
  TraceParams tp{};
  fill_trace_params(c, tp);
  const auto tw0 = std::chrono::steady_clock::now();
  Laps laps(c->debug_timing, "sort");
  unsigned long long *k0 = nullptr, *k1 = nullptr;
  uint32_t *i0 = nullptr, *i1 = nullptr;
  void *temp = nullptr;
#define CKC(call) do { cudaError_t e_ = (call); if (e_ != cudaSuccess) { c->error = std::string(#call) + ": " + cudaGetErrorString(e_); return FTKB_ERR_CUDA; } } while (0)
  {
    const size_t tb0 = std::max(sort_pairs_u64(nullptr, 0, nullptr, nullptr, nullptr, nullptr, n, c->stream),
                                unique_by_key_u64(nullptr, 0, nullptr, nullptr, nullptr, nullptr, c->d_scalars + ftkb_ctx::SLOT_UQ, n, c->stream));
    const size_t plan[14] = {8 * n, 8 * n, 4 * n, 4 * n, tb0, c->streaming ? 0 : 4 * 8 * n, c->streaming ? 0 : 4 * n, c->streaming ? 0 : 4 * n, c->streaming ? 0 : 4 * n,
                             0, 0, 0, sizeof(ftkb_point) * n, 8 * n};
    const int rp = scratch_plan(c, plan, 14);
    if (rp) return rp;
  }
  { int rs = scratch(c, 0, 8 * n, (void **)&k0); if (!rs) rs = scratch(c, 1, 8 * n, (void **)&k1); if (!rs) rs = scratch(c, 2, 4 * n, (void **)&i0);
    if (!rs) rs = scratch(c, 3, 4 * n, (void **)&i1); if (rs) return rs; }
  CKC(cudaEventRecord(c->ev[0], c->stream));
  launch_point_keys(c->d_pts, n, tp, k0, i0, c->stream);
  size_t tb = std::max(sort_pairs_u64(nullptr, 0, k0, k1, i0, i1, n, c->stream),
                       unique_by_key_u64(nullptr, 0, k1, i1, k0, i0, c->d_scalars + ftkb_ctx::SLOT_UQ, n, c->stream));
  { const int rs = scratch(c, 4, tb, &temp); if (rs) return rs; }
  sort_pairs_u64(temp, tb, k0, k1, i0, i1, n, c->stream);
  unique_by_key_u64(temp, tb, k1, i1, k0, i0, c->d_scalars + ftkb_ctx::SLOT_UQ, n, c->stream);
  CKC(cudaMemcpyAsync(c->h_scalars + ftkb_ctx::SLOT_UQ, c->d_scalars + ftkb_ctx::SLOT_UQ, 8, cudaMemcpyDeviceToHost, c->stream));
  CKC(cudaStreamSynchronize(c->stream));
  const uint64_t nu = c->h_scalars[ftkb_ctx::SLOT_UQ];
  laps.lap("sort+unique");
  { int rs = scratch(c, 12, sizeof(ftkb_point) * nu, (void **)&c->d_pts_sorted); if (!rs) rs = scratch(c, 13, 8 * nu, (void **)&c->d_keys_sorted); if (rs) return rs; }
  launch_gather_points(c->d_pts, i0, nu, c->d_pts_sorted, c->stream);
  CKC(cudaMemcpyAsync(c->d_keys_sorted, k0, 8 * nu, cudaMemcpyDeviceToDevice, c->stream));
  CKC(cudaEventRecord(c->ev[1], c->stream));
  laps.lap("malloc+gather");
  CKC(cudaStreamSynchronize(c->stream));
  laps.lap("sync");
  CKC(cudaGetLastError());
  float ms = 0;
  CKC(cudaEventElapsedTime(&ms, c->ev[0], c->ev[1]));
  c->stats.ms_finalize_device += ms;
  c->stats.kernel_launches += 4;
  c->nsorted = nu;
  c->stats.ms_sort_wall += std::chrono::duration<double, std::milli>(std::chrono::steady_clock::now() - tw0).count();
#undef CKC
  c->sorted = true;
  return FTKB_OK;
}

static int host_points(ftkb_ctx *c) {
  const int rc = ensure_sorted(c);
  if (rc) return rc;
  if (c->pts_sorted.size() == c->nsorted) return FTKB_OK;
  c->pts_sorted.resize(c->nsorted);
  if (c->nsorted) {
    CK(cudaMemcpyAsync(c->pts_sorted.data(), c->d_pts_sorted, sizeof(ftkb_point) * c->nsorted, cudaMemcpyDeviceToHost, c->stream));
    CK(cudaStreamSynchronize(c->stream));
    c->stats.d2h_bytes += sizeof(ftkb_point) * c->nsorted;
  }
  return FTKB_OK;
}

extern "C" int ftkb_num_points(ftkb_ctx *c, uint64_t *n) {
  if (!c || !n) return FTKB_ERR_INVALID;
  const int rc = ensure_sorted(c);
  if (rc) return rc;
  *n = c->nsorted;
  return FTKB_OK;
}

extern "C" int ftkb_get_points(ftkb_ctx *c, ftkb_point *out, uint64_t cap) {
  if (!c || (!out && cap)) return FTKB_ERR_INVALID;
  const int rc = ensure_sorted(c);
  if (rc) return rc;
  if (cap < c->nsorted) return fail(c, FTKB_ERR_INVALID, "get_points: output buffer too small");
  if (!c->nsorted) return FTKB_OK;
  if (c->pts_sorted.size() == c->nsorted) { std::memcpy(out, c->pts_sorted.data(), sizeof(ftkb_point) * c->nsorted); return FTKB_OK; }
  CK(cudaSetDevice(c->cfg.device));
  CK(cudaMemcpyAsync(out, c->d_pts_sorted, sizeof(ftkb_point) * c->nsorted, cudaMemcpyDeviceToHost, c->stream));
  CK(cudaStreamSynchronize(c->stream));
  c->stats.d2h_bytes += sizeof(ftkb_point) * c->nsorted;
  return FTKB_OK;
}

extern "C" int ftkb_import_points(ftkb_ctx *c, const ftkb_point *pts, uint64_t n) {
  if (!c || (!pts && n)) return FTKB_ERR_INVALID;
  if (c->streaming) return fail(c, FTKB_ERR_INVALID, "import_points: not available with streaming trajectories");
  if (!n) return FTKB_OK;
  CK(cudaSetDevice(c->cfg.device));
  { const int rc = drain(c); if (rc) return rc; }
  c->primed = false;
  if (c->npts + n > c->pt_cap) {
    const int rc = grow_points(c, c->npts + n);
    if (rc) return rc;
  }
  CK(cudaMemcpyAsync(c->d_pts + c->npts, pts, sizeof(ftkb_point) * n, cudaMemcpyHostToDevice, c->stream));
  CK(cudaStreamSynchronize(c->stream));
  c->stats.h2d_bytes += sizeof(ftkb_point) * n;
  c->npts += n;
  c->stats.points = c->npts;
  c->sorted = false;
  c->traced = false;
  return FTKB_OK;
}

extern "C" int ftkb_finalize(ftkb_ctx *c) {
  if (!c) return FTKB_ERR_INVALID;
  int rc = drain(c);
  if (rc) return rc;
  if (c->traced) return FTKB_OK;
// ... 142 lines not shown
  c->traj_idx.reserve(n);
  for (size_t si = 0; si < S; si++) {
    const Piece &pc = pieces[si];
    const uint32_t *src = bufs[pc.thread].data() + pc.off;
    c->traj_idx.insert(c->traj_idx.end(), src, src + pc.len);
    c->traj_loop.push_back(pc.loop);
    c->traj_off.push_back(c->traj_idx.size());
  }
  laps.lap("layout");
  c->stats.ms_finalize_host += std::chrono::duration<double, std::milli>(std::chrono::steady_clock::now() - t0).count();
  c->stats.ms_trace_wall += std::chrono::duration<double, std::milli>(std::chrono::steady_clock::now() - tw0).count();
  c->traced = true;
  return FTKB_OK;
}

extern "C" int ftkb_num_trajectories(ftkb_ctx *c, uint64_t *n) {
  if (!c || !n) return FTKB_ERR_INVALID;
  if (!c->traced) return fail(c, FTKB_ERR_INVALID, "num_trajectories: call finalize first");
  *n = c->traj_loop.size();
  return FTKB_OK;
}

extern "C" int ftkb_get_trajectory_complete(ftkb_ctx *c, uint8_t *complete) {
  if (!c || !complete) return FTKB_ERR_INVALID;
  if (!c->traced) return fail(c, FTKB_ERR_INVALID, "get_trajectory_complete: call finalize first");
  for (size_t k = 0; k < c->traj_loop.size(); k++) complete[k] = k < c->traj_complete.size() ? c->traj_complete[k] : 0;
  return FTKB_OK;
}

extern "C" int ftkb_get_trajectories(ftkb_ctx *c, uint64_t *offsets, uint64_t *point_idx, uint8_t *loop) {
  if (!c || !offsets) return FTKB_ERR_INVALID;
  if (!c->traced) return fail(c, FTKB_ERR_INVALID, "get_trajectories: call finalize first");
  std::memcpy(offsets, c->traj_off.data(), 8 * c->traj_off.size());
  if (point_idx && !c->traj_idx.empty()) std::memcpy(point_idx, c->traj_idx.data(), 8 * c->traj_idx.size());
  if (loop && !c->traj_loop.empty()) std::memcpy(loop, c->traj_loop.data(), c->traj_loop.size());
  return FTKB_OK;
}

extern "C" int ftkb_ipc_export(const void *dev_ptr, ftkb_ipc_handle *out) {
  if (!dev_ptr || !out) return FTKB_ERR_INVALID;
  typedef CUresult (*RangeFn)(CUdeviceptr *, size_t *, CUdeviceptr);
  static RangeFn range = nullptr;
  if (!range) {
    void *fp = nullptr;
    cudaDriverEntryPointQueryResult q;
    if (cudaGetDriverEntryPoint("cuMemGetAddressRange", &fp, cudaEnableDefault, &q) != cudaSuccess || q != cudaDriverEntryPointSuccess) { cudaGetLastError(); return FTKB_ERR_CUDA; }
    range = reinterpret_cast<RangeFn>(fp);
  }
  CUdeviceptr base = 0;
  size_t size = 0;
  if (range(&base, &size, (CUdeviceptr)(uintptr_t)dev_ptr) != CUDA_SUCCESS) return FTKB_ERR_CUDA;
  cudaIpcMemHandle_t h;
  if (cudaIpcGetMemHandle(&h, reinterpret_cast<void *>(base)) != cudaSuccess) { cudaGetLastError(); return FTKB_ERR_CUDA; }
  static_assert(sizeof(h) == 64, "cudaIpcMemHandle_t is 64 bytes");
  std::memcpy(out->bytes, &h, 64);
  out->offset = (uint64_t)((uintptr_t)dev_ptr - (uintptr_t)base);
  return FTKB_OK;
}

extern "C" int ftkb_ipc_import(const ftkb_ipc_handle *h, int device, void **dev_ptr) {
  if (!h || !dev_ptr) return FTKB_ERR_INVALID;
  if (cudaSetDevice(device) != cudaSuccess) { cudaGetLastError(); return FTKB_ERR_NO_DEVICE; }
  cudaIpcMemHandle_t ih;
  std::memcpy(&ih, h->bytes, 64);
  void *base = nullptr;
  if (cudaIpcOpenMemHandle(&base, ih, cudaIpcMemLazyEnablePeerAccess) != cudaSuccess) { cudaGetLastError(); return FTKB_ERR_CUDA; }
  *dev_ptr = static_cast<char *>(base) + h->offset;
  return FTKB_OK;
}

extern "C" int ftkb_ipc_close(void *dev_ptr, const ftkb_ipc_handle *h) {
  if (!dev_ptr || !h) return FTKB_ERR_INVALID;
  if (cudaIpcCloseMemHandle(static_cast<char *>(dev_ptr) - h->offset) != cudaSuccess) { cudaGetLastError(); return FTKB_ERR_CUDA; }
  return FTKB_OK;
}

extern "C" int ftkb_export_layer_cells(ftkb_ctx *c, int index, void **cells, uint64_t *bytes, double *resolution) {
  if (!c || !cells || !bytes) return FTKB_ERR_INVALID;
  if (index < 0 || (size_t)index >= c->layers.size()) return fail(c, FTKB_ERR_INVALID, "export_layer_cells: no such resident layer");
  { const int rc = drain(c); if (rc) return rc; }
  if ((size_t)index >= c->layers.size()) return fail(c, FTKB_ERR_INVALID, "export_layer_cells: no such resident layer");
  Layer &l = c->layers[index];
  if (!l.cells || !l.cells_valid) return fail(c, FTKB_ERR_INVALID, "export_layer_cells: the layer has no range cells yet (a sweep must have read it)");
  CK(cudaSetDevice(c->cfg.device));
  CK(cudaStreamSynchronize(c->stream));
  if (!l.cells_foreign) { l.cells_foreign = true; c->exportedCells.push_back(l.cells); }
  *cells = l.cells;
  *bytes = (uint64_t)c->ncells * sizeof(uint4);
  if (resolution) *resolution = l.res_pending ? DBL_MAX : slot_value(c, l.slot);
  return FTKB_OK;
}

extern "C" int ftkb_push_snapshot_remote(ftkb_ctx *c, const double *scalar, const double *vector, const void *cells, double resolution) {
  if (!c || !cells || (!scalar && !vector)) return FTKB_ERR_INVALID;
  if (c->cfg.jacobian_source == FTKB_SOURCE_GIVEN) return fail(c, FTKB_ERR_INVALID, "push_snapshot_remote: a GIVEN jacobian cannot be remote");
  if (c->cfg.vector_source == FTKB_SOURCE_GIVEN ? !vector : !scalar) return fail(c, FTKB_ERR_INVALID, "push_snapshot_remote: the field the sweep reads is missing");
  CK(cudaSetDevice(c->cfg.device));
  if ((uintptr_t)scalar % 8 != 0 || (uintptr_t)vector % 8 != 0 || (uintptr_t)cells % 16 != 0)
    return fail(c, FTKB_ERR_INVALID, "push_snapshot_remote: arrays must be 8-byte aligned, cells 16-byte aligned");
  Layer l;
  int rc = new_layer(c, l);
  if (rc) return rc;
  l.S = const_cast<double *>(scalar);
  l.V = const_cast<double *>(vector);
  l.cells = reinterpret_cast<uint4 *>(const_cast<void *>(cells));
  l.cells_valid = true;
  l.cells_foreign = true;
  l.res_pending = false;
  unsigned long long bits;
  const double r = resolution > 0 ? resolution : DBL_MAX;
  std::memcpy(&bits, &r, 8);
  if (!(resolution > 0) || resolution >= DBL_MAX) bits = ~0ull;
  c->h_scalars[l.slot] = bits;
  CK(cudaMemcpyAsync(c->d_scalars + l.slot, c->h_scalars + l.slot, sizeof(unsigned long long), cudaMemcpyHostToDevice, c->stream));
  c->layers.push_back(l);
  return FTKB_OK;
}

extern "C" int ftkb_get_curveset(ftkb_ctx *c, ftkb_curveset **out) {
  if (!c || !out) return FTKB_ERR_INVALID;
  if (!c->traced) return fail(c, FTKB_ERR_INVALID, "get_curveset: call finalize first");
  const uint64_t ntraj = c->traj_off.empty() ? 0 : c->traj_off.size() - 1;
  static const uint64_t zero = 0;
  { const int rch = host_points(c); if (rch) return rch; }
  const int rc = ftkb_curveset_create(c->pts_sorted.data(), c->pts_sorted.size(), ntraj ? c->traj_off.data() : &zero, c->traj_idx.data(),
                                      c->traj_loop.data(), ntraj, out);
  if (rc == FTKB_OK)
    for (size_t k = 0; k < c->traj_complete.size() && k < (*out)->curves.size(); k++) (*out)->curves[k].complete = c->traj_complete[k] != 0;
  return rc;
}

extern "C" int ftkb_get_component_labels(ftkb_ctx *c, uint64_t *labels) {
  if (!c || !labels) return FTKB_ERR_INVALID;
  if (!c->traced) return fail(c, FTKB_ERR_INVALID, "get_component_labels: call finalize first");
  if (!c->labels.empty()) std::memcpy(labels, c->labels.data(), 8 * c->labels.size());
  return FTKB_OK;
}

extern "C" int ftkb_get_degrees(ftkb_ctx *c, int32_t *deg) {
  if (!c || !deg) return FTKB_ERR_INVALID;
  if (!c->traced) return fail(c, FTKB_ERR_INVALID, "get_degrees: call finalize first");
  if (!c->deg.empty()) std::memcpy(deg, c->deg.data(), 4 * c->deg.size());
  return FTKB_OK;
}

extern "C" int ftkb_get_last_worklist(ftkb_ctx *c, uint64_t *out, uint64_t cap, uint64_t *n) {
  if (!c || !n || (!out && cap)) return FTKB_ERR_INVALID;
  CK(cudaSetDevice(c->cfg.device));
  { const int rc = drain(c); if (rc) return rc; }
  CK(cudaStreamSynchronize(c->stream));
  const uint64_t have = std::min<uint64_t>(c->last_wl, c->wl_cap);
  *n = have;
  const uint64_t m = std::min(have, cap);
  if (m) CK(cudaMemcpy(out, c->last_wl_sel ? c->d_wl2 : c->d_wl, sizeof(uint64_t) * m, cudaMemcpyDeviceToHost));
  return FTKB_OK;
}

extern "C" int ftkb_get_layer(ftkb_ctx *c, int index, double *scalar, double *vector) {
  if (!c || (!scalar && !vector)) return FTKB_ERR_INVALID;
  CK(cudaSetDevice(c->cfg.device));
  { const int rc = drain(c); if (rc) return rc; }
  if (index < 0 || (size_t)index >= c->layers.size()) return fail(c, FTKB_ERR_INVALID, "get_layer: no such resident snapshot");
  const Layer &l = c->layers[index];
  if ((scalar && !l.S) || (vector && !l.V)) return fail(c, FTKB_ERR_INVALID, "get_layer: the snapshot does not hold that field");
  CK(cudaStreamSynchronize(c->stream));
  if (scalar) CK(cudaMemcpy(scalar, l.S, sizeof(double) * c->nvert, cudaMemcpyDeviceToHost));
  if (vector) CK(cudaMemcpy(vector, l.V, sizeof(double) * c->nvert * c->n, cudaMemcpyDeviceToHost));
  c->stats.d2h_bytes += sizeof(double) * c->nvert * ((scalar ? 1 : 0) + (vector ? c->n : 0));
  return FTKB_OK;
}

static bool device_local_cpus(int device, cpu_set_t *set) {
  char bus[32] = {0};
  if (cudaDeviceGetPCIBusId(bus, sizeof(bus) - 1, device) != cudaSuccess) { cudaGetLastError(); return false; }
  for (char *q = bus; *q; q++) *q = (char)std::tolower((unsigned char)*q);
  FILE *f = std::fopen((std::string("/sys/bus/pci/devices/") + bus + "/local_cpulist").c_str(), "r");
  if (!f) return false;
  char line[4096];
  const bool got = std::fgets(line, sizeof(line), f) != nullptr;
  std::fclose(f);
  cpu_set_t allowed;
  if (!got || sched_getaffinity(0, sizeof(allowed), &allowed) != 0) return false;
  CPU_ZERO(set);
  int n = 0;
  for (const char *q = line; *q && *q != '\n';) {
    char *e = nullptr;
    long a = std::strtol(q, &e, 10), b = a;
    if (e == q) break;
    if (*e == '-') { q = e + 1; b = std::strtol(q, &e, 10); }
    for (long i = a; i <= b && i < CPU_SETSIZE; i++)
      if (CPU_ISSET(i, &allowed)) { CPU_SET(i, set); n++; }
    if (*e != ',') break;
    q = e + 1;
  }
  return n > 0;
}

extern "C" int ftkb_bind_thread_to_device(int device) {
  cpu_set_t set;
  if (!device_local_cpus(device, &set)) return 0;
  if (sched_setaffinity(0, sizeof(set), &set) != 0) return 0;
  return CPU_COUNT(&set);
}

extern "C" int ftkb_host_alloc(uint64_t bytes, void **out) {
  if (!out || !bytes) return FTKB_ERR_INVALID;
  *out = nullptr;
  cpu_set_t before, local;
  int device = 0;
  bool moved = false;
  if (cudaGetDevice(&device) == cudaSuccess && sched_getaffinity(0, sizeof(before), &before) == 0 && device_local_cpus(device, &local))
    moved = sched_setaffinity(0, sizeof(local), &local) == 0;
  const cudaError_t e = cudaHostAlloc(out, bytes, cudaHostAllocPortable);
  if (moved) sched_setaffinity(0, sizeof(before), &before);
  if (e != cudaSuccess) { cudaGetLastError(); return FTKB_ERR_NOMEM; }
  return FTKB_OK;
}

extern "C" void ftkb_host_free(void *p) {
  if (p && cudaFreeHost(p) != cudaSuccess) cudaGetLastError();
}

extern "C" int ftkb_get_stats(ftkb_ctx *c, ftkb_stats *out) {
  if (!c || !out) return FTKB_ERR_INVALID;
  if (!c->pend.empty()) {
    cudaSetDevice(c->cfg.device);
    const int rc = drain(c);
    if (rc) return rc;
  }
  { const int rc = wait_grow(c); if (rc) return rc; }
  c->stats.scaling_factor = c->factor;
  c->stats.resolution = c->resolution;
  *out = c->stats;
  return FTKB_OK;
}

extern "C" int ftkb_reset_stats(ftkb_ctx *c) {
  if (!c) return FTKB_ERR_INVALID;
  if (!c->pend.empty()) {
    cudaSetDevice(c->cfg.device);
    const int rc = drain(c);
    if (rc) return rc;
  }
  { const int rc = wait_grow(c); if (rc) return rc; }
  const uint64_t pts = c->stats.points;
  c->stats = ftkb_stats{};
  c->stats.points = pts;
  return FTKB_OK;
}

extern "C" int ftkb_synchronize(ftkb_ctx *c) {
  if (!c) return FTKB_ERR_INVALID;
  CK(cudaSetDevice(c->cfg.device));
  { const int rc = drain(c); if (rc) return rc; }
  CK(cudaStreamSynchronize(c->stream));
  CK(cudaStreamSynchronize(c->stream2));
  return wait_grow(c);
}

extern "C" int ftkb_timer_start(ftkb_ctx *c) {
  if (!c) return FTKB_ERR_INVALID;
  CK(cudaSetDevice(c->cfg.device));
  CK(cudaEventRecord(c->ev[6], c->stream));
  return FTKB_OK;
}

extern "C" int ftkb_timer_stop(ftkb_ctx *c, double *ms) {
  if (!c || !ms) return FTKB_ERR_INVALID;
  CK(cudaSetDevice(c->cfg.device));
  CK(cudaEventRecord(c->ev_join, c->stream2));
  CK(cudaStreamWaitEvent(c->stream, c->ev_join, 0));
  CK(cudaEventRecord(c->ev[7], c->stream));
  CK(cudaEventSynchronize(c->ev[7]));
  float f = 0;
  CK(cudaEventElapsedTime(&f, c->ev[6], c->ev[7]));
  *ms = f;
  return FTKB_OK;
}

extern "C" int ftkb_mesh_ntypes(int nd_mesh, int k, int scope) {
  if ((nd_mesh != 3 && nd_mesh != 4) || k < 0 || k > nd_mesh) return -1;
  const MeshTables &m = mesh_tables(nd_mesh);
  return scope == 0 ? m.ntypes(k) : scope == 1 ? (int)m.ordinal_types[k].size() : (int)m.interval_types[k].size();
}

extern "C" int ftkb_mesh_unit_simplex(int nd_mesh, int k, int type, int32_t *out) {
  if ((nd_mesh != 3 && nd_mesh != 4) || k < 0 || k > nd_mesh || !out) return -1;
  const MeshTables &m = mesh_tables(nd_mesh);
  if (type < 0 || type >= m.ntypes(k)) return -1;
  for (int i = 0; i <= k; i++)
    for (int j = 0; j < nd_mesh; j++) out[i * nd_mesh + j] = (m.unit[k][type][i] >> j) & 1;
  return 0;
}

extern "C" int ftkb_mesh_scope_type(int nd_mesh, int k, int scope, int itype) {
  if ((nd_mesh != 3 && nd_mesh != 4) || k < 0 || k > nd_mesh) return -1;
  const MeshTables &m = mesh_tables(nd_mesh);
  const std::vector<int> *v = scope == 1 ? &m.ordinal_types[k] : scope == 2 ? &m.interval_types[k] : nullptr;
  if (!v) return itype;
  return itype >= 0 && itype < (int)v->size() ? (*v)[itype] : -1;
}

static int copy_offsets(const std::vector<TypeOffset> &v, int nd, int32_t *out) {
  for (size_t i = 0; i < v.size(); i++) {
    out[i * (nd + 1)] = v[i].type;
    for (int j = 0; j < nd; j++) out[i * (nd + 1) + 1 + j] = v[i].off[j];
  }
  return (int)v.size();
}

extern "C" int ftkb_mesh_sides(int nd_mesh, int k, int type, int32_t *out) {
  if ((nd_mesh != 3 && nd_mesh != 4) || k < 0 || k > nd_mesh || !out) return -1;
  const MeshTables &m = mesh_tables(nd_mesh);
  if (type < 0 || type >= m.ntypes(k)) return -1;
  return copy_offsets(m.sides[k][type], nd_mesh, out);
}

extern "C" int ftkb_mesh_side_of(int nd_mesh, int k, int type, int32_t *out) {
  if ((nd_mesh != 3 && nd_mesh != 4) || k < 0 || k > nd_mesh || !out) return -1;
  const MeshTables &m = mesh_tables(nd_mesh);
  if (type < 0 || type >= m.ntypes(k)) return -1;
  return copy_offsets(m.side_of[k][type], nd_mesh, out);
}
```

### ftk_b200/csrc/kernels.cu

```cuda
#include "kernels.h"

#include <algorithm>
#include <cfloat>
#include <cstdlib>
#include <string>
#include <climits>
#include <cub/device/device_radix_sort.cuh>
#include <cub/device/device_select.cuh>

namespace ftkb {

typedef long long i64;
typedef unsigned long long u64;

__constant__ DeviceMeshTables c_mesh[2];

void upload_mesh_tables(const DeviceMeshTables &t2, const DeviceMeshTables &t3) {
  DeviceMeshTables h[2] = {t2, t3};
  cudaMemcpyToSymbol(c_mesh, h, sizeof(h));
}

constexpr int KEY_ONE = 0x3FF00000;
constexpr int KEY_POISON_EXP = 0x43E00000;

// ... 489 lines not shown
    const double2 t = *reinterpret_cast<const double2 *>(lane_base + st * C2_SEG + 2);
    dst[0] = t.x; dst[1] = t.y;
  };
  auto release = [&](const int st) {
    __syncwarp();
    if (elect_one()) mbar_arrive(empty0 + 8u * st);
  };
  auto finish_block = [&](const int kb, FRange bx, FRange by, const uint4 prevc) {
    bx = fmerge(bx, fshfl_down1(bx));
    by = fmerge(by, fshfl_down1(by));
    sum_out[(size_t)kb * 32u] = make_uint4(__float_as_uint(bx.mn), __float_as_uint(bx.mx), __float_as_uint(by.mn), __float_as_uint(by.mx));
    if (TEST) {
      if (NPREV) {
        bx = fmerge(bx, FRange{__uint_as_float(prevc.x), __uint_as_float(prevc.y)});
        by = fmerge(by, FRange{__uint_as_float(prevc.z), __uint_as_float(prevc.w)});
      }
      const int y0 = kb * C2_R;
      const bool own = own_cols && y0 <= p.ub[1] && y0 + C2_R - 1 >= p.lb[1];
      cells2d_decide(p, bx, by, own, e, y0, NPREV + 1);
    }
  };

  double win[3][2];
  mbar_wait(full0, 0);
  centre(0, win[0]);
  mbar_wait(full0 + 8, 0);
  centre(1, win[1]);
  release(0);
  FRange bx{0.f, 0.f}, by{0.f, 0.f};
  uint4 prevc = make_uint4(0x7FC00000u, 0x7FC00000u, 0x7FC00000u, 0x7FC00000u);

  auto step = [&](auto KC, const int j, const int i) {
    constexpr int K = decltype(KC)::value;
    constexpr int ST_J = (1 + K) % C2_NST, ST_P = (2 + K) % C2_NST;
    double (&m1)[2] = win[K % 3];
    double (&c0v)[2] = win[(K + 1) % 3];
    double (&p1)[2] = win[(K + 2) % 3];
    mbar_wait(full0 + 8u * ST_P, (uint32_t)((i + (2 + K >= C2_NST ? 1 : 0)) & 1));
    centre(ST_P, p1);
    const double *rowj = lane_base + ST_J * C2_SEG;
    double left = rowj[1], right = rowj[4];
    double mid_e = c0v[1];
    if (BORDER) {
      if (e == 0) left = c0v[0];
      if (!o_in) mid_e = c0v[0];
      if (!o1_in) right = c0v[1];
    }
    const double dxe = mid_e - left, dxo = right - c0v[0], dye = p1[0] - m1[0], dyo = p1[1] - m1[1];
    const float fxe = __double2float_rn(dxe) * cwf, fxo = __double2float_rn(dxo) * cwf;
    const float fye = __double2float_rn(dye) * chf, fyo = __double2float_rn(dyo) * chf;
    if (want_res && j < H) {
      float a = fminf(fminf(fabsf(fxe), fabsf(fye)), fminf(fabsf(fxo), fabsf(fyo)));
      if (BORDER) a = fminf(e_in ? fminf(fabsf(fxe), fabsf(fye)) : 3.4028234e38f, o_in ? fminf(fabsf(fxo), fabsf(fyo)) : 3.4028234e38f);
      if (a < rminf) res_update4(rmin, rminf, e_in, o_in, dxe, dye, dxo, dyo, (double)(W - 1), (double)(H - 1));
    }
    const FRange rx{fminf(fxe, fxo), fmaxf(fxe, fxo)}, ry{fminf(fye, fyo), fmaxf(fye, fyo)};
    if (K == 0) {
      if (j > r0) finish_block(j / C2_R - 1, fmerge(bx, rx), fmerge(by, ry), prevc);
      bx = rx; by = ry;
      if (NPREV && j < jl) prevc = __ldg(sum_prev + (size_t)(j / C2_R) * 32u);
    } else {
      bx = fmerge(bx, rx); by = fmerge(by, ry);
    }
    release(ST_J);
  };

  for (int j = r0, i = 0; j <= jl; j += C2_NST, i++) {
    step(IC<0>{}, j, i);
    if (j + 1 <= jl) step(IC<1>{}, j + 1, i);
    if (j + 2 <= jl) step(IC<2>{}, j + 2, i);
    if (j + 3 <= jl) step(IC<3>{}, j + 3, i);
    if (j + 4 <= jl) step(IC<4>{}, j + 4, i);
    if (j + 5 <= jl) step(IC<5>{}, j + 5, i);
    if (j + 6 <= jl) step(IC<6>{}, j + 6, i);
    if (j + 7 <= jl) step(IC<7>{}, j + 7, i);
    if (j + 8 <= jl) step(IC<8>{}, j + 8, i);
  }
  if (jl % C2_R != 0) finish_block(jl / C2_R, bx, by, prevc);
  if (want_res) warp_res_commit(fabs(rmin), p.res_slot[B]);
}

template <int NPREV, bool TEST>
__global__ void __launch_bounds__((C2_CW + 1) * 32, 3) scan2d_build_kernel(const __grid_constant__ SweepParams p) {
  constexpr uint32_t STAGE_BYTES = C2_SEG * 8;
  extern __shared__ __align__(128) unsigned char fb_smem[];
  const int lane = threadIdx.x & 31;
  const int wib = __shfl_sync(0xffffffffu, (int)(threadIdx.x >> 5), 0);
  double *ring = reinterpret_cast<double *>(fb_smem);
  const uint32_t full0 = smem_u32(fb_smem + (size_t)C2_NST * STAGE_BYTES), empty0 = full0 + 8u * C2_NST;
  const int W = p.W, H = p.H;
  const int bx = blockIdx.x % p.nsx, cy = blockIdx.x / p.nsx;
  const int C0 = bx * (C2_CW * FB_STRIDE);
  const int nactive = min(C2_CW, (W - C0 + FB_STRIDE - 1) / FB_STRIDE);
  if (threadIdx.x == 0) {
#pragma unroll
    for (int q = 0; q < C2_NST; q++) { mbar_init(full0 + 8u * q, 1); mbar_init(empty0 + 8u * q, (uint32_t)nactive); }
    asm volatile("fence.mbarrier_init.release.cluster;" ::: "memory");
    asm volatile("fence.proxy.async.shared::cta;" ::: "memory");
  }
  __syncthreads();
  const int r0 = cy * p.rows;
  const int r1 = min(r0 + p.rows - 1, H - 1);
  const int nrows = (r1 + 1) - r0 + 3;
  if (wib == C2_CW) {
    if (elect_one()) {
      const double *S = p.L[p.build_layer].S;
      const int col_lo = max(C0 - 2, 0), col_hi = min(C0 - 2 + C2_SEG, W);
      const uint32_t seg_bytes = (uint32_t)(col_hi - col_lo) * 8u;
      const uint32_t dst0 = smem_u32(ring) + (uint32_t)(col_lo - (C0 - 2)) * 8u;
      for (int rr = 0; rr < nrows; rr++) {
        const int st = rr % C2_NST;
        if (rr >= C2_NST) mbar_wait(empty0 + 8u * st, (uint32_t)((rr / C2_NST - 1) & 1));
        const size_t off = (size_t)W * (size_t)clampi(r0 - 1 + rr, H) + (size_t)col_lo;
        mbar_expect_tx(full0 + 8u * st, seg_bytes);
        bulk_g2s(dst0 + (uint32_t)st * STAGE_BYTES, S + off, seg_bytes, full0 + 8u * st);
      }
    }
    return;
  }
  if (wib >= nactive) return;
  const int c0 = C0 + wib * FB_STRIDE;
  const double *tile = ring + wib * FB_STRIDE;
  const bool border = c0 == 0 || c0 + FB_SEG - 2 > W;
  if (border) cells2d_strip<true, NPREV, TEST>(p, c0, r0, r1, lane, tile, full0, empty0, bx * C2_CW + wib);
  else cells2d_strip<false, NPREV, TEST>(p, c0, r0, r1, lane, tile, full0, empty0, bx * C2_CW + wib);
}

template <int NL>
__global__ void __launch_bounds__(256) scan2d_cells_kernel(const __grid_constant__ SweepParams p, const int nstrips, const int nblk_used) {
  const int lane = threadIdx.x & 31;
  const long long w = (long long)blockIdx.x * 8 + (threadIdx.x >> 5);
  if (w >= (long long)nstrips * nblk_used) return;
  const int strip = (int)(w / nblk_used), kb = (int)(w % nblk_used);
  const int e = strip * FB_STRIDE + 2 * lane, y0 = kb * C2_R;
  const bool own = lane <= 30 && ((e >= p.lb[0] && e <= p.ub[0]) || (e + 1 >= p.lb[0] && e + 1 <= p.ub[0])) && y0 <= p.ub[1] && y0 + C2_R - 1 >= p.lb[1];
  if (!__any_sync(0xffffffffu, own)) return;
  const float nanf_ = __int_as_float(0x7FC00000);
  FRange ux{nanf_, nanf_}, uy{nanf_, nanf_};
#pragma unroll
  for (int L = 0; L < NL; L++) {
    const uint4 c = __ldg(p.sum_in[L] + cells2d_index(p, strip, kb, lane));
    ux = fmerge(ux, FRange{__uint_as_float(c.x), __uint_as_float(c.y)});
    uy = fmerge(uy, FRange{__uint_as_float(c.z), __uint_as_float(c.w)});
  }
  cells2d_decide(p, ux, uy, own, e, y0, NL);
}

constexpr int K2_R = 3;
constexpr int K2_NST = 4;
constexpr int K2_CTAS = 3;
constexpr uint32_t K2_ROW_BYTES = C2_SEG * 8;
constexpr uint32_t K2_STAGE_BYTES = K2_R * K2_ROW_BYTES;
static_assert(C2_R % K2_R == 0, "cell block = whole stages");

__device__ __forceinline__ double2 lds128_f64(uint32_t a) {
  double2 v;
  asm volatile("ld.shared.v2.f64 {%0, %1}, [%2];" : "=d"(v.x), "=d"(v.y) : "r"(a));
  return v;
}
__device__ __forceinline__ double lds64_f64(uint32_t a) {
  double v;
  asm volatile("ld.shared.f64 %0, [%1];" : "=d"(v) : "r"(a));
  return v;
}
__device__ __forceinline__ void cp_async16(uint32_t dst, const void *src) {
  asm volatile("cp.async.cg.shared.global [%0], [%1], 16;" ::"r"(dst), "l"(src) : "memory");
}
__device__ __forceinline__ void cp_async_wait_all() { asm volatile("cp.async.wait_all;" ::: "memory"); }
__device__ __forceinline__ void cp_async_commit() { asm volatile("cp.async.commit_group;" ::: "memory"); }
template <int N> __device__ __forceinline__ void cp_async_wait_group() { asm volatile("cp.async.wait_group %0;" ::"n"(N) : "memory"); }
__device__ __forceinline__ uint4 lds128_u32(uint32_t a) {
  uint4 v;
  asm volatile("ld.shared.v4.u32 {%0, %1, %2, %3}, [%4];" : "=r"(v.x), "=r"(v.y), "=r"(v.z), "=r"(v.w) : "r"(a) : "memory");
  return v;
}
__device__ __forceinline__ void sts64_f64(uint32_t a, double v) { asm volatile("st.shared.f64 [%0], %1;" ::"r"(a), "d"(v) : "memory"); }
__device__ __forceinline__ float fmax_nan(float a, float b) {
  float r;
  asm("max.NaN.f32 %0, %1, %2;" : "=f"(r) : "f"(a), "f"(b));
  return r;
}

__device__ __forceinline__ double nzmin(double m, double d) {
  double r;
  asm("{\n\t.reg .pred p, q;\n\t.reg .f64 ad, am;\n\tabs.f64 ad, %2;\n\tabs.f64 am, %1;\n\t"
      "setp.neu.f64 q, %2, 0d0000000000000000;\n\tsetp.lt.and.f64 p, ad, am, q;\n\tselp.f64 %0, %2, %1, p;\n\t}"
      : "=d"(r) : "d"(m), "d"(d));
  return r;
}

__device__ __forceinline__ FRange k2_vrange(float kmn, float kmx, double c) {
  const int a = __float_as_int(kmn), b = __float_as_int(kmx);
  const double lo = __hiloint2double(a < 0 ? a + 1 : a, 0);
  const double hi = __hiloint2double(b < 0 ? b : b + 1, 0);
  return FRange{__double2float_rd(lo * c), __double2float_ru(hi * c)};
}

__device__ __forceinline__ void prefetch_l2(const void *q) { asm volatile("prefetch.global.L2 [%0];" ::"l"(q)); }

struct K2Acc { double mdx, mdy; float big; };

template <bool BORDER, int NPREV, bool TEST>
__device__ __forceinline__ K2Acc keys2d_strip(const SweepParams &p, const int c0, const int r0, const int r1, const int lane,
                                           const uint32_t tile_u32 ,
                                           const uint32_t full0, const uint32_t empty0, const int strip,
                                           const uint32_t sbase ,
                                           const uint32_t res_u32 ,
                                           const uint32_t wl_stage ,
                                           const uint32_t cell_stage ,
                                           const K2Acc acc) {
  float big = acc.big;
  const int W = p.W, H = p.H, B = p.build_layer;
  const int e = c0 + 2 * lane, o = e + 1;
  const bool e_in = !BORDER || e < W, o_in = !BORDER || o < W, o1_in = !BORDER || o + 1 < W;
  const bool own_cols = lane <= 30 && ((e >= p.lb[0] && e <= p.ub[0]) || (o >= p.lb[0] && o <= p.ub[0]));
  const int jl = r1 + 1;
  const int nrows = jl - r0 + 1;
  const int ngroups = (nrows + K2_R - 1) / K2_R, nstages = (nrows + 2 + K2_R - 1) / K2_R;
  const double cw = (double)(W - 1), ch = (double)(H - 1);
  const bool want_res = p.res_slot[B] != nullptr;
  const float thrx = p.res_thr[0], thry = p.res_thr[1];
  const uint4 *sum_prev = NPREV ? p.sum_in[0] + cells2d_index(p, strip, 0, lane) : nullptr;
  uint4 *sum_out = p.sum_out + cells2d_index(p, strip, 0, lane);
  const uint32_t lane_u32 = tile_u32 + (uint32_t)lane * 16u;
  const int kb0 = r0 / C2_R;
  unsigned long long failbits = 0;
  const int kb_end = ((r1 + 1) + C2_R - 1) / C2_R;

  auto finish_block = [&](const int kb, float xmn, float xmx, float ymn, float ymx) {
    xmn = fminf(xmn, __shfl_down_sync(0xffffffffu, xmn, 1)); xmx = fmaxf(xmx, __shfl_down_sync(0xffffffffu, xmx, 1));
    ymn = fminf(ymn, __shfl_down_sync(0xffffffffu, ymn, 1)); ymx = fmaxf(ymx, __shfl_down_sync(0xffffffffu, ymx, 1));
    FRange bx = k2_vrange(xmn, xmx, cw), by = k2_vrange(ymn, ymx, ch);
    sum_out[(size_t)kb * 32u] = make_uint4(__float_as_uint(bx.mn), __float_as_uint(bx.mx), __float_as_uint(by.mn), __float_as_uint(by.mx));
    if (TEST) {
      if (NPREV && kb < kb_end) {
        cp_async_wait_all();
        const uint4 prevc = lds128_u32(cell_stage + ((uint32_t)kb & 1u) * 512u);
        bx = fmerge(bx, FRange{__uint_as_float(prevc.x), __uint_as_float(prevc.y)});
        by = fmerge(by, FRange{__uint_as_float(prevc.z), __uint_as_float(prevc.w)});
      }
      const int y0 = kb * C2_R;
      const bool own = own_cols && y0 <= p.ub[1] && y0 + C2_R - 1 >= p.lb[1];
      if (own && !cube_excluded2_f(bx, by, p.thrp_f, p.thr2_f, p.lim_f)) failbits |= 1ull << (kb - kb0);
    }
  };

  double C[2][K2_R][2];
  float KX[2][K2_R][2];
  auto load_stage = [&](auto PC, const int s) {
    constexpr int P = decltype(PC)::value;
    const uint32_t gs = sbase + (uint32_t)s, slot = gs % K2_NST;
    mbar_wait(full0 + 8u * slot, (gs / K2_NST) & 1u);
    const uint32_t base = lane_u32 + slot * K2_STAGE_BYTES;
    double nl[K2_R], nr[K2_R];
#pragma unroll
    for (int i = 0; i < K2_R; i++) {
      const double2 c = lds128_f64(base + (uint32_t)i * K2_ROW_BYTES + 16u);
      C[P][i][0] = c.x; C[P][i][1] = c.y;
      nl[i] = lds64_f64(base + (uint32_t)i * K2_ROW_BYTES + 8u);
      nr[i] = lds64_f64(base + (uint32_t)i * K2_ROW_BYTES + 32u);
    }
    float ax = __int_as_float(0x7F800000);
#pragma unroll
    for (int i = 0; i < K2_R; i++) {
      const float ke = fabsf(hikey(C[P][i][0])), ko = fabsf(hikey(C[P][i][1]));
      big = fmax_nan(big, BORDER ? (e_in ? ke : 0.f) : ke);
      big = fmax_nan(big, BORDER ? (o_in ? ko : 0.f) : ko);
      double left = nl[i], right = nr[i], mid_e = C[P][i][1];
      if (BORDER) {
        if (e == 0) left = C[P][i][0];
        if (!o_in) mid_e = C[P][i][0];
        if (!o1_in) right = C[P][i][1];
      }
      const double dxe = mid_e - left, dxo = right - C[P][i][0];
      KX[P][i][0] = hikey(dxe); KX[P][i][1] = hikey(dxo);
      ax = fminf(ax, fminf(fabsf(KX[P][i][0]), fabsf(KX[P][i][1])));
    }
    if (want_res && __any_sync(0xffffffffu, ax <= thrx)) {
      double mdx = lds64_f64(res_u32);
#pragma unroll
      for (int i = 0; i < K2_R; i++) {
        const int j = r0 + K2_R * s + i - 1;
        if (j >= r0 && j <= jl && j < H) {
          double left = lds64_f64(base + (uint32_t)i * K2_ROW_BYTES + 8u), right = lds64_f64(base + (uint32_t)i * K2_ROW_BYTES + 32u), mid_e = C[P][i][1];
          if (BORDER) {
            if (e == 0) left = C[P][i][0];
            if (!o_in) mid_e = C[P][i][0];
            if (!o1_in) right = C[P][i][1];
          }
          if (e_in) mdx = nzmin(mdx, mid_e - left);
          if (o_in) mdx = nzmin(mdx, right - C[P][i][0]);
        }
      }
      sts64_f64(res_u32, mdx);
    }
    __syncwarp();
    if (elect_one()) mbar_arrive(empty0 + 8u * slot);
  };

  float bxmn = 0.f, bxmx = 0.f, bymn = 0.f, bymx = 0.f;
  const uint4 nanc = make_uint4(0x7FC00000u, 0x7FC00000u, 0x7FC00000u, 0x7FC00000u);
  int kb = r0 / C2_R;
  if (NPREV && kb < kb_end) prefetch_l2(sum_prev + (size_t)kb * 32u);
  if (NPREV && kb + 1 < kb_end) prefetch_l2(sum_prev + (size_t)(kb + 1) * 32u);

  int gphase = 0;
  static_assert(C2_R == 3 * K2_R, "a cell block is three groups");
  auto group = [&](auto PC, const int g) {
    constexpr int P = decltype(PC)::value;
    if (g + 1 < nstages) load_stage(IC<1 - P>{}, g + 1);
    const bool opens_group = gphase == 0;
    gphase = gphase == 2 ? 0 : gphase + 1;
    const int j0 = r0 + K2_R * g;
    const bool full = j0 + K2_R - 1 <= min(jl, H - 1);
    float ay = __int_as_float(0x7F800000);
#pragma unroll
    for (int i = 0; i < K2_R; i++) {
      const int j = j0 + i;
      if (!full && j > jl) break;
      const double *m1 = C[P][i];
      const float *kx = i + 1 < K2_R ? KX[P][i + 1] : KX[1 - P][i + 1 - K2_R];
      const double *p1 = i + 2 < K2_R ? C[P][i + 2] : C[1 - P][i + 2 - K2_R];
      const double dye = p1[0] - m1[0], dyo = p1[1] - m1[1];
      const float kxe = kx[0], kxo = kx[1], kye = hikey(dye), kyo = hikey(dyo);
      ay = fminf(ay, fminf(fabsf(kye), fabsf(kyo)));
      if (i == 0 && opens_group) {
        const float rxmn = fminf(kxe, kxo), rxmx = fmaxf(kxe, kxo), rymn = fminf(kye, kyo), rymx = fmaxf(kye, kyo);
        if (j > r0) finish_block(kb - 1, fminf(bxmn, rxmn), fmaxf(bxmx, rxmx), fminf(bymn, rymn), fmaxf(bymx, rymx));
        bxmn = rxmn; bxmx = rxmx; bymn = rymn; bymx = rymx;
        if (NPREV && kb < kb_end) cp_async16(cell_stage + ((uint32_t)kb & 1u) * 512u, sum_prev + (size_t)kb * 32u);
        kb++;
        if (NPREV && kb + 1 < kb_end) prefetch_l2(sum_prev + (size_t)(kb + 1) * 32u);
      } else {
        bxmn = fminf(fminf(bxmn, kxe), kxo); bxmx = fmaxf(fmaxf(bxmx, kxe), kxo);
        bymn = fminf(fminf(bymn, kye), kyo); bymx = fmaxf(fmaxf(bymx, kye), kyo);
      }
    }
    if (want_res && __any_sync(0xffffffffu, ay <= thry)) {
      double mdy = lds64_f64(res_u32 + 8u);
#pragma unroll
      for (int i = 0; i < K2_R; i++) {
        const int j = j0 + i;
        if (!full && (j > jl || j >= H)) break;
        const double *m1 = C[P][i];
        const double *p1 = i + 2 < K2_R ? C[P][i + 2] : C[1 - P][i + 2 - K2_R];
        if (e_in) mdy = nzmin(mdy, p1[0] - m1[0]);
        if (o_in) mdy = nzmin(mdy, p1[1] - m1[1]);
      }
      sts64_f64(res_u32 + 8u, mdy);
    }
  };

  load_stage(IC<0>{}, 0);
#pragma unroll 1
  for (int g = 0; g < ngroups; g += 2) {
    group(IC<0>{}, g);
    if (g + 1 < ngroups) group(IC<1>{}, g + 1);
  }
  if (jl % C2_R != 0) finish_block(jl / C2_R, bxmn, bxmx, bymn, bymx);
  if (TEST) {
    for (int b = 0; b < 64; b++) {
      if (!__any_sync(0xffffffffu, (failbits >> b) != 0)) break;
      const unsigned fm = __ballot_sync(0xffffffffu, (failbits >> b) & 1ull);
      if (fm) cells2d_slow_cubes(p, fm, c0, (kb0 + b) * C2_R, NPREV + 1, wl_stage);
    }
    flush_survivors(p, wl_stage);
  }
  return K2Acc{lds64_f64(res_u32), lds64_f64(res_u32 + 8u), big};
}

template <int NPREV, bool TEST>
__global__ void __launch_bounds__((C2_CW + 1) * 32, K2_CTAS) scan2d_keys_build_kernel(const __grid_constant__ SweepParams p) {
  extern __shared__ __align__(128) unsigned char fb_smem[];
  const int lane = threadIdx.x & 31;
  const int wib = __shfl_sync(0xffffffffu, (int)(threadIdx.x >> 5), 0);
  const uint32_t ring0 = smem_u32(fb_smem);
  const uint32_t full0 = ring0 + (uint32_t)K2_NST * K2_STAGE_BYTES, empty0 = full0 + 8u * K2_NST;
  const uint32_t res_u32 = empty0 + 8u * K2_NST + 16u * threadIdx.x;
  const uint32_t wl_stage = empty0 + 8u * K2_NST + 16u * (C2_CW + 1) * 32u + 32u + WL_STAGE_BYTES * (uint32_t)wib;
  const uint32_t cell_stage = empty0 + 8u * K2_NST + 16u * (C2_CW + 1) * 32u + 32u + WL_STAGE_BYTES * (uint32_t)C2_CW + 1024u * (uint32_t)wib + 16u * (uint32_t)lane;
  const int W = p.W, H = p.H;
  const int bx = blockIdx.x % p.nsx, cy = blockIdx.x / p.nsx;
  const int C0 = bx * (C2_CW * FB_STRIDE);
  const int nactive = min(C2_CW, (W - C0 + FB_STRIDE - 1) / FB_STRIDE);
  if (threadIdx.x == 0) {
#pragma unroll
    for (int q = 0; q < K2_NST; q++) { mbar_init(full0 + 8u * q, 1); mbar_init(empty0 + 8u * q, (uint32_t)nactive); }
    asm volatile("fence.mbarrier_init.release.cluster;" ::: "memory");
    asm volatile("fence.proxy.async.shared::cta;" ::: "memory");
  }
  __syncthreads();
  const int r0 = cy * p.rows;
  const int r1 = min(r0 + p.rows - 1, H - 1);
  const int nstages = ((r1 + 1) - r0 + 1 + 2 + K2_R - 1) / K2_R;
  if (wib == C2_CW) {
    if (elect_one()) {
      const double *S = p.L[p.build_layer].S;
      const int col_lo = max(C0 - 2, 0), col_hi = min(C0 - 2 + C2_SEG, W);
      const uint32_t seg_bytes = (uint32_t)(col_hi - col_lo) * 8u;
      const uint32_t dst0 = ring0 + (uint32_t)(col_lo - (C0 - 2)) * 8u;
      for (int s = 0; s < nstages; s++) {
        const uint32_t slot = (uint32_t)s % K2_NST;
        if (s >= K2_NST) mbar_wait(empty0 + 8u * slot, (uint32_t)((s / K2_NST - 1) & 1));
        mbar_expect_tx(full0 + 8u * slot, seg_bytes * K2_R);
#pragma unroll
        for (int i = 0; i < K2_R; i++) {
          const size_t off = (size_t)W * (size_t)clampi(r0 - 1 + K2_R * s + i, H) + (size_t)col_lo;
          bulk_g2s(dst0 + slot * K2_STAGE_BYTES + (uint32_t)i * K2_ROW_BYTES, S + off, seg_bytes, full0 + 8u * slot);
        }
      }
    }
    return;
  }
  if (wib >= nactive) return;
  const int c0 = C0 + wib * FB_STRIDE;
  const uint32_t tile_u32 = ring0 + (uint32_t)(wib * FB_STRIDE) * 8u;
  const bool border = c0 == 0 || c0 + FB_SEG - 2 > W;
  K2Acc acc{DBL_MAX, DBL_MAX, 0.f};
  sts64_f64(res_u32, DBL_MAX); sts64_f64(res_u32 + 8u, DBL_MAX);
  if (lane == 0) asm volatile("st.shared.s32 [%0], %1;" ::"r"(wl_stage), "r"(0) : "memory");
  __syncwarp();
  if (border) acc = keys2d_strip<true, NPREV, TEST>(p, c0, r0, r1, lane, tile_u32, full0, empty0, bx * C2_CW + wib, 0u, res_u32, wl_stage, cell_stage, acc);
  else acc = keys2d_strip<false, NPREV, TEST>(p, c0, r0, r1, lane, tile_u32, full0, empty0, bx * C2_CW + wib, 0u, res_u32, wl_stage, cell_stage, acc);
  if (p.res_slot[p.build_layer] != nullptr) {
    const double cw = (double)(W - 1), ch = (double)(H - 1);
    const double ax = fabs(acc.mdx), ay = fabs(acc.mdy);
    const double vx = ax < DBL_MAX ? ax * cw : DBL_MAX, vy = ay < DBL_MAX ? ay * ch : DBL_MAX;
    warp_res_commit(fmin(vx > 0.0 ? vx : DBL_MAX, vy > 0.0 ? vy : DBL_MAX), p.res_slot[p.build_layer]);
  }
  if (!(acc.big < __int_as_float(KEYF_BIG))) atomicExch(p.poison, 1ull);
}

static size_t k2_smem_bytes() { return (size_t)K2_NST * K2_STAGE_BYTES + (size_t)2 * K2_NST * 8 + (size_t)16 * (C2_CW + 1) * 32 + 32 + (size_t)WL_STAGE_BYTES * C2_CW + (size_t)1024 * C2_CW; }
static size_t c2_smem_bytes() { return (size_t)C2_NST * C2_SEG * 8 + (size_t)2 * C2_NST * 8; }

size_t scan2d_cells_per_layer(const SweepParams &p) {
  return (size_t)p.nsx * C2_CW * (size_t)(p.H / C2_R + 2) * 32u;
}

void launch_scan2d_cells(const SweepParams &p, cudaStream_t s) {
  const unsigned grid = (unsigned)((i64)p.nsx * p.nsy);
  const int nstrips = (p.W + FB_STRIDE - 1) / FB_STRIDE, nblk = (p.H + C2_R - 1) / C2_R;
  const unsigned tgrid = (unsigned)(((i64)nstrips * nblk + 7) / 8);
  if (p.keys2d && p.sum_mode <= SUM_BUILD_TEST2) {
    switch (p.sum_mode) {
      case SUM_BUILD: scan2d_keys_build_kernel<0, false><<<grid, (C2_CW + 1) * 32, k2_smem_bytes(), s>>>(p); break;
      case SUM_BUILD_TEST1: scan2d_keys_build_kernel<0, true><<<grid, (C2_CW + 1) * 32, k2_smem_bytes(), s>>>(p); break;
      default: scan2d_keys_build_kernel<1, true><<<grid, (C2_CW + 1) * 32, k2_smem_bytes(), s>>>(p); break;
    }
    return;
  }
  switch (p.sum_mode) {
    case SUM_BUILD: scan2d_build_kernel<0, false><<<grid, (C2_CW + 1) * 32, c2_smem_bytes(), s>>>(p); break;
    case SUM_BUILD_TEST1: scan2d_build_kernel<0, true><<<grid, (C2_CW + 1) * 32, c2_smem_bytes(), s>>>(p); break;
    case SUM_BUILD_TEST2: scan2d_build_kernel<1, true><<<grid, (C2_CW + 1) * 32, c2_smem_bytes(), s>>>(p); break;
    case SUM_TEST1: scan2d_cells_kernel<1><<<tgrid, 256, 0, s>>>(p, nstrips, nblk); break;
    default: scan2d_cells_kernel<2><<<tgrid, 256, 0, s>>>(p, nstrips, nblk); break;
  }
}

constexpr int F3_LAYER_BYTES = ((F3_ROWS * F3_COLS * 8 + 127) / 128) * 128;
constexpr uint32_t F3_BOX_BYTES = F3_ROWS * F3_COLS * 8;

__device__ __noinline__ void fused3d_slow_cubes(const SweepParams &p, unsigned failmask, const int C0, const int y0, const int z, const int nl) {
  static_assert(2 * F3_RW * 4 == 32, "four lanes per cube");
  const int lane = threadIdx.x & 31;
  const bool vec = !p.fused;
  const int nbits20 = (p.nbits - (vec ? 0 : 1)) << 20;
  const size_t sy = (size_t)p.W, sz = (size_t)p.W * (size_t)p.H;
  const int cube = lane >> 2, sub = lane & 3;
  const int r = cube >> 1, q = cube & 1;
  while (failmask) {
    const int src = __ffs(failmask) - 1;
    failmask &= failmask - 1;
    const int x = C0 + 2 * src + q, y = y0 + r;
    const bool in = x >= p.lb[0] && x <= p.ub[0] && y >= p.lb[1] && y <= p.ub[1];
    KeyRange rg[3] = {neutral_range(), neutral_range(), neutral_range()};
#pragma unroll
    for (int vv = 0; vv < 2; vv++) {
      const int v = 2 * sub + vv;
      const int vx = x + (v & 1), vy = y + ((v >> 1) & 1), vz = z + (v >> 2);
      if (!in || vx > p.ub[0] || vy > p.ub[1] || vz > p.ub[2]) continue;
      const bool border = vx < 1 || vx > p.W - 2 || vy < 1 || vy > p.H - 2 || vz < 1 || vz > p.D - 2;
      const size_t idx = (size_t)vx + sy * (size_t)vy + sz * (size_t)vz;
      for (int L = 0; L < nl; L++) {
        const double *S = p.L[L].S;
        int h0 = 0, h1 = 0, h2 = 0;
        if (vec) {
          const int *Vh = reinterpret_cast<const int *>(p.L[L].V) + idx * 6 + 1;
          h0 = __ldg(Vh); h1 = __ldg(Vh + 2); h2 = __ldg(Vh + 4);
        } else if (!border) {
          h0 = __double2hiint(__ldg(S + idx + 1) - __ldg(S + idx - 1));
          h1 = __double2hiint(__ldg(S + idx + sy) - __ldg(S + idx - sy));
          h2 = __double2hiint(__ldg(S + idx + sz) - __ldg(S + idx - sz));
        }
        rg[0] = merge(rg[0], vertex_range(h0, nbits20));
        rg[1] = merge(rg[1], vertex_range(h1, nbits20));
        rg[2] = merge(rg[2], vertex_range(h2, nbits20));
      }
    }
#pragma unroll
    for (int c = 0; c < 3; c++)
#pragma unroll
      for (int off = 1; off <= 2; off <<= 1) {
        rg[c].mn = min(rg[c].mn, __shfl_xor_sync(0xffffffffu, rg[c].mn, off));
        rg[c].mx = max(rg[c].mx, __shfl_xor_sync(0xffffffffu, rg[c].mx, off));
      }
    const bool surv = in && sub == 0 && !cube_excluded3(rg[0], rg[1], rg[2]);
    append_survivors(p, surv, (u64)(x - p.lb[0]) + (u64)p.nc[0] * ((u64)(y - p.lb[1]) + (u64)p.nc[1] * (u64)(z - p.lb[2])));
  }
}

__device__ __forceinline__ void res_update3(double &m, const bool in, const double dx, const double dy, const double dz) {
  if (!in) return;
  const double vx = 0.5 * dx, vy = 0.5 * dy, vz = 0.5 * dz;
  if (vx != 0.0 && fabs(vx) < fabs(m)) m = vx;
  if (vy != 0.0 && fabs(vy) < fabs(m)) m = vy;
  if (vz != 0.0 && fabs(vz) < fabs(m)) m = vz;
}

constexpr int S3_RW = F3_RW;
constexpr int S3_WR = S3_RW + 1;
constexpr int S3_NST = 5;
constexpr int S3_STAGE_BYTES = F3_LAYER_BYTES;

__device__ __forceinline__ uint32_t pack_keys(float mn, float mx) {
  return __byte_perm((uint32_t)__float_as_int(mn), (uint32_t)__float_as_int(mx), 0x7632);
}
__device__ __forceinline__ void merge_cell(float (&mn)[3], float (&mx)[3], const uint4 w) {
  mn[0] = fminf(mn[0], __int_as_float((int)(w.x << 16))); mx[0] = fmaxf(mx[0], __int_as_float((int)(w.x & 0xffff0000u)));
  mn[1] = fminf(mn[1], __int_as_float((int)(w.y << 16))); mx[1] = fmaxf(mx[1], __int_as_float((int)(w.y & 0xffff0000u)));
  mn[2] = fminf(mn[2], __int_as_float((int)(w.z << 16))); mx[2] = fmaxf(mx[2], __int_as_float((int)(w.z & 0xffff0000u)));
}

struct S3Thresholds { float kthr, kfloor; int esum_max, nbits20; double half_factor; };
__device__ __forceinline__ S3Thresholds s3_thresholds(const int nbits, const bool vec) {
  const int s = vec ? 1 : 0;
  S3Thresholds t;
  t.kthr = __int_as_float((1023 + 1 - s - nbits) << 20);
  t.kfloor = __int_as_float((1023 - s - nbits) << 20);
  t.esum_max = 3119 - 3 * s - 3 * nbits;
  t.nbits20 = (nbits - 1 + s) << 20;
  t.half_factor = __hiloint2double((1023 + nbits - 1 + s) << 20, 0);
  return t;
}

__device__ __noinline__ bool s3_union_excluded_precise(const float mn0, const float mx0, const float mn1, const float mx1,
                                                       const float mn2, const float mx2, const int nbits20) {
  const auto lo = [](float f) { const int k = __float_as_int(f); return k < 0 ? (k | 0xFFFF) : k; };
  const auto hi = [](float f) { const int k = __float_as_int(f); return k < 0 ? k : (k | 0xFFFF); };
  const KeyRange x{vertex_range(lo(mn0), nbits20).mn, vertex_range(hi(mx0), nbits20).mx};
  const KeyRange y{vertex_range(lo(mn1), nbits20).mn, vertex_range(hi(mx1), nbits20).mx};
  const KeyRange z{vertex_range(lo(mn2), nbits20).mn, vertex_range(hi(mx2), nbits20).mx};
  return cube_excluded3(x, y, z);
}

__device__ __forceinline__ bool s3_excluded_level1(const S3Thresholds &T, const float (&cmn)[3], const float (&cmx)[3]) {
  bool sided = false;
  int esum = 0;
#pragma unroll
  for (int c = 0; c < 3; c++) {
    sided = sided || cmn[c] >= T.kthr || cmx[c] <= -T.kthr;
    esum += (__float_as_int(fmaxf(fmaxf(fabsf(cmn[c]), fabsf(cmx[c])), T.kfloor)) >> 20);
  }
  return sided && esum <= T.esum_max && !(cmn[0] != cmn[0]);
}

__device__ __noinline__ bool s3_excluded_levels23(const float mn0, const float mx0, const float mn1, const float mx1, const float mn2, const float mx2,
                                                  const double half_factor, const int nbits20) {
  const float mag[3] = {fmaxf(fabsf(mn0), fabsf(mx0)), fmaxf(fabsf(mn1), fabsf(mx1)), fmaxf(fabsf(mn2), fabsf(mx2))};
  double P = 48.0;
#pragma unroll
  for (int c = 0; c < 3; c++) P *= fma(__hiloint2double((__float_as_int(mag[c]) | 0xFFFF) + 1, 0), half_factor, 1.0);
  if (P < 9.0e18) return true;
  return s3_union_excluded_precise(mn0, mx0, mn1, mx1, mn2, mx2, nbits20);
}

__device__ __forceinline__ void s3_test(const SweepParams &p, const S3Thresholds &T, const float (&cmn)[3], const float (&cmx)[3],
                                        const bool own_any, const int e, const int y0, const int zc, const int nl) {
  bool sided = false;
  int esum = 0;
  float mag[3];
#pragma unroll
  for (int c = 0; c < 3; c++) {
    sided = sided || cmn[c] >= T.kthr || cmx[c] <= -T.kthr;
    mag[c] = fmaxf(fabsf(cmn[c]), fabsf(cmx[c]));
    esum += (__float_as_int(fmaxf(mag[c], T.kfloor)) >> 20);
  }
  bool excl = sided && esum <= T.esum_max && !(cmn[0] != cmn[0]);
  if (sided && !excl && own_any && !(cmn[0] != cmn[0])) {
    double P = 48.0;
#pragma unroll
    for (int c = 0; c < 3; c++) P *= fma(__hiloint2double((__float_as_int(mag[c]) | 0xFFFF) + 1, 0), T.half_factor, 1.0);
    excl = P < 9.0e18;
    if (!excl) excl = s3_union_excluded_precise(cmn[0], cmx[0], cmn[1], cmx[1], cmn[2], cmx[2], T.nbits20);
  }
  const bool fail = own_any && !excl;
  const unsigned fm = __ballot_sync(0xffffffffu, fail);
  if (fm) fused3d_slow_cubes(p, fm, e - 2 * (int)(threadIdx.x & 31), y0, zc, nl);
}

__device__ __forceinline__ size_t s3_cell_index(const SweepParams &p, const int tile, const int wib, const int z, const int lane) {
  return (((size_t)tile * F3_CW + (size_t)wib) * (size_t)(p.D + 1) + (size_t)z) * 32u + (size_t)lane;
}

__device__ __noinline__ void s3_retest_plane(const SweepParams &p, const uint4 *built, const uint4 *other, const bool fail, const bool vec,
                                             const int e, const int y0, const int zc, const int zc0) {
  if (!__any_sync(0xffffffffu, fail)) return;
  const S3Thresholds T = s3_thresholds(p.nbits, vec);
  const float nanf_ = __int_as_float(KEYF_NAN);
  float cmn[3] = {nanf_, nanf_, nanf_}, cmx[3] = {nanf_, nanf_, nanf_};
// ... 526 lines not shown
  const size_t cell0 = s3_cell_index(p, tile, wib, zc0, lane);
  const uint4 *sum_prev = NPREV ? p.sum_in[0] + cell0 : nullptr;
  uint4 *sum_out = p.sum_out + cell0;
  const size_t row3 = (size_t)W * 3 / 2;
  for (int zg = zc0; zg <= zc1 + 1; zg++) {
    uint4 prev = make_uint4(0x7FC07FC0u, 0x7FC07FC0u, 0x7FC07FC0u, 0u);
    if (NPREV) prev = __ldg(sum_prev);
    const bool zok = zg < D;
    const bool zdom = zg >= p.lb[2] && zg <= p.ub[2];
    float umin[3] = {nanf_, nanf_, nanf_}, umax[3] = {nanf_, nanf_, nanf_};
    if (zok) {
      unsigned m2 = mk;
      if (EDGE) asm volatile("" : "+r"(m2));
      int4 a[S3_RW + 1][3];
      const int4 *base = V + ((size_t)zg * (size_t)H + (size_t)y0) * row3 + (size_t)e * 3 / 2;
#pragma unroll
      for (int r = 0; r <= S3_RW; r++) {
        const bool ld = !EDGE || (((m2 >> r) | (m2 >> (r + 8))) & 1u);
#pragma unroll
        for (int q = 0; q < 3; q++) a[r][q] = ld ? __ldg(base + (size_t)r * row3 + q) : make_int4(0, 0, 0, 0);
      }
#pragma unroll
      for (int r = 0; r <= S3_RW; r++) {
        float kxe = __int_as_float(a[r][0].y), kye = __int_as_float(a[r][0].w), kze = __int_as_float(a[r][1].y);
        float kxo = __int_as_float(a[r][1].w), kyo = __int_as_float(a[r][2].y), kzo = __int_as_float(a[r][2].w);
        big = max(big, max(max(a[r][0].y & 0x7fffffff, a[r][0].w & 0x7fffffff), a[r][1].y & 0x7fffffff));
        big = max(big, max(max(a[r][1].w & 0x7fffffff, a[r][2].y & 0x7fffffff), a[r][2].w & 0x7fffffff));
        if (want_res) {
          float ma = fminf(fminf(fabsf(kxe), fabsf(kye)), fabsf(kze)), mb = fminf(fminf(fabsf(kxo), fabsf(kyo)), fabsf(kzo));
          bool in_e = true, in_o = true;
          if (EDGE) { in_e = (m2 >> r) & 1u; in_o = (m2 >> (r + 8)) & 1u; ma = in_e ? ma : inff_; mb = in_o ? mb : inff_; }
          const float m = fminf(ma, mb);
          if (m <= rkey) {
            const double vxe = __hiloint2double(a[r][0].y, a[r][0].x), vye = __hiloint2double(a[r][0].w, a[r][0].z), vze = __hiloint2double(a[r][1].y, a[r][1].x);
            const double vxo = __hiloint2double(a[r][1].w, a[r][1].z), vyo = __hiloint2double(a[r][2].y, a[r][2].x), vzo = __hiloint2double(a[r][2].w, a[r][2].z);
            bool go = m < rkey;
            const double ar = fabs(rmin);
            if (!go) go = (in_e && (fabs(vxe) < ar || fabs(vye) < ar || fabs(vze) < ar)) || (in_o && (fabs(vxo) < ar || fabs(vyo) < ar || fabs(vzo) < ar));
            if (go) {
              if (in_e) rmin = vres_vertex<3>(rmin, vxe, vye, vze);
              if (in_o) rmin = vres_vertex<3>(rmin, vxo, vyo, vzo);
              rkey = rmin == DBL_MAX ? inff_ : hikey(fabs(rmin));
            }
          }
        }
        if (EDGE) {
          const bool de = (m2 >> (r + 16)) & 1u, dq = (m2 >> (r + 24)) & 1u;
          kxe = de ? kxe : nanf_; kye = de ? kye : nanf_; kze = de ? kze : nanf_;
          kxo = dq ? kxo : nanf_; kyo = dq ? kyo : nanf_; kzo = dq ? kzo : nanf_;
        }
        umin[0] = fminf(umin[0], fminf(kxe, kxo)); umax[0] = fmaxf(umax[0], fmaxf(kxe, kxo));
        umin[1] = fminf(umin[1], fminf(kye, kyo)); umax[1] = fmaxf(umax[1], fmaxf(kye, kyo));
        umin[2] = fminf(umin[2], fminf(kze, kzo)); umax[2] = fmaxf(umax[2], fmaxf(kze, kzo));
      }
    }
    if (!zdom) {
#pragma unroll
      for (int c = 0; c < 3; c++) { umin[c] = nanf_; umax[c] = nanf_; }
    }
#pragma unroll
    for (int c = 0; c < 3; c++) {
      umin[c] = fminf(umin[c], __shfl_down_sync(0xffffffffu, umin[c], 1));
      umax[c] = fmaxf(umax[c], __shfl_down_sync(0xffffffffu, umax[c], 1));
    }
    *sum_out = make_uint4(pack_keys(umin[0], umax[0]), pack_keys(umin[1], umax[1]), pack_keys(umin[2], umax[2]), 0u);
    sum_out += 32;
    if (NPREV) sum_prev += 32;
    if (TEST) {
      if (NPREV) merge_cell(umin, umax, prev);
      if (zg > zc0) {
        const int zc_ = zg - 1;
        if (zc_ >= p.lb[2] && zc_ <= p.ub[2]) {
          float cmn[3] = {umin[0], umin[1], umin[2]}, cmx[3] = {umax[0], umax[1], umax[2]};
          merge_cell(cmn, cmx, make_uint4(pcell[0], pcell[1], pcell[2], 0u));
          s3_test(p, T, cmn, cmx, own_any, e, y0, zc_, NPREV + 1);
        }
      }
#pragma unroll
      for (int c = 0; c < 3; c++) pcell[c] = pack_keys(umin[c], umax[c]);
    }
  }
  if (want_res) warp_res_commit(fabs(rmin), p.res_slot[B]);
  if (big >= KEYF_BIG) atomicExch(p.poison, 1ull);
}

template <int NPREV, bool TEST>
__global__ void __launch_bounds__(F3_CW * 32, 2) vscan3d_build_kernel(const __grid_constant__ SweepParams p) {
  const int lane = threadIdx.x & 31, wib = threadIdx.x >> 5;
  int b = blockIdx.x;
  const int bx = b % p.nsx; b /= p.nsx;
  const int by = b % p.nsy;
  const int bz = b / p.nsy;
  const int C0 = bx * F3_STRIDE, Y0 = by * F3_TROWS;
  const int zc0 = bz * p.rows, zc1 = min(zc0 + p.rows - 1, p.D - 1);
  const int tile = by * p.nsx + bx;
  const bool interior = C0 >= p.lb[0] && C0 + 63 <= min(p.W - 1, p.ub[0]) && Y0 >= p.lb[1] && Y0 + F3_TROWS <= min(p.H - 1, p.ub[1]);
  if (interior) vs3_consume<false, NPREV, TEST>(p, tile, C0, Y0, zc0, zc1, wib, lane);
  else vs3_consume<true, NPREV, TEST>(p, tile, C0, Y0, zc0, zc1, wib, lane);
}

size_t vscan2d_cells_per_layer(const SweepParams &p) { return (size_t)p.nsx * (size_t)(p.H / V2_R + 2) * 32u; }

void launch_vscan_cells(const SweepParams &p, cudaStream_t s) {
  if (p.nd == 3) {
    const unsigned grid = (unsigned)((i64)p.nsx * p.nsy * p.nsz);
    switch (p.sum_mode) {
      case SUM_BUILD: vscan3d_build_kernel<0, false><<<grid, F3_CW * 32, 0, s>>>(p); break;
      case SUM_BUILD_TEST1: vscan3d_build_kernel<0, true><<<grid, F3_CW * 32, 0, s>>>(p); break;
      case SUM_BUILD_TEST2: vscan3d_build_kernel<1, true><<<grid, F3_CW * 32, 0, s>>>(p); break;
      case SUM_TEST1: scan3d_cells_kernel<1><<<grid, F3_CW * 32, 0, s>>>(p); break;
      default: scan3d_cells_kernel<2><<<grid, F3_CW * 32, 0, s>>>(p); break;
    }
    return;
  }
  const unsigned grid = (unsigned)(((i64)p.nsx * p.nsy + 7) / 8);
  const int nblk = (p.H + V2_R - 1) / V2_R;
  const unsigned tgrid = (unsigned)(((i64)p.nsx * nblk + 7) / 8);
  switch (p.sum_mode) {
    case SUM_BUILD: vscan2d_build_kernel<0, false><<<grid, 256, 0, s>>>(p); break;
    case SUM_BUILD_TEST1: vscan2d_build_kernel<0, true><<<grid, 256, 0, s>>>(p); break;
    case SUM_BUILD_TEST2: vscan2d_build_kernel<1, true><<<grid, 256, 0, s>>>(p); break;
    case SUM_TEST1: vscan2d_cells_kernel<1><<<tgrid, 256, 0, s>>>(p, p.nsx, nblk); break;
    default: vscan2d_cells_kernel<2><<<tgrid, 256, 0, s>>>(p, p.nsx, nblk); break;
  }
}


typedef CUresult (*TmapEncodeFn)(CUtensorMap *, CUtensorMapDataType, cuuint32_t, void *, const cuuint64_t *, const cuuint64_t *, const cuuint32_t *,
                                 const cuuint32_t *, CUtensorMapInterleave, CUtensorMapSwizzle, CUtensorMapL2promotion, CUtensorMapFloatOOBfill);

bool encode_scalar_tmap3d(const double *S, int W, int H, int D, CUtensorMap *out) {
  static TmapEncodeFn fn = nullptr;
  static bool tried = false;
  if (!tried) {
    tried = true;
    void *ptr = nullptr;
    cudaDriverEntryPointQueryResult qres;
    if (cudaGetDriverEntryPoint("cuTensorMapEncodeTiled", &ptr, cudaEnableDefault, &qres) == cudaSuccess && qres == cudaDriverEntryPointSuccess)
      fn = reinterpret_cast<TmapEncodeFn>(ptr);
    else cudaGetLastError();
  }
  if (!fn || (W & 1) || ((uintptr_t)S & 15)) return false;
  const cuuint64_t gdim[3] = {(cuuint64_t)W, (cuuint64_t)H, (cuuint64_t)D};
  const cuuint64_t gstride[2] = {(cuuint64_t)W * 8, (cuuint64_t)W * (cuuint64_t)H * 8};
  const cuuint32_t box[3] = {F3_COLS, F3_ROWS, 1}, estr[3] = {1, 1, 1};
  return fn(out, CU_TENSOR_MAP_DATA_TYPE_FLOAT64, 3, const_cast<double *>(S), gdim, gstride, box, estr, CU_TENSOR_MAP_INTERLEAVE_NONE,
            CU_TENSOR_MAP_SWIZZLE_NONE, CU_TENSOR_MAP_L2_PROMOTION_L2_256B, CU_TENSOR_MAP_FLOAT_OOB_FILL_NONE) == CUDA_SUCCESS;
}

void init_kernel_attributes() {
  cudaFuncSetAttribute(scan2d_build_kernel<0, false>, cudaFuncAttributeMaxDynamicSharedMemorySize, (int)c2_smem_bytes());
  cudaFuncSetAttribute(scan2d_build_kernel<0, true>, cudaFuncAttributeMaxDynamicSharedMemorySize, (int)c2_smem_bytes());
  cudaFuncSetAttribute(scan2d_build_kernel<1, true>, cudaFuncAttributeMaxDynamicSharedMemorySize, (int)c2_smem_bytes());
  cudaFuncSetAttribute(scan2d_keys_build_kernel<0, false>, cudaFuncAttributeMaxDynamicSharedMemorySize, (int)k2_smem_bytes());
  cudaFuncSetAttribute(scan2d_keys_build_kernel<0, true>, cudaFuncAttributeMaxDynamicSharedMemorySize, (int)k2_smem_bytes());
  cudaFuncSetAttribute(scan2d_keys_build_kernel<1, true>, cudaFuncAttributeMaxDynamicSharedMemorySize, (int)k2_smem_bytes());
  cudaFuncSetAttribute(scan3d_build_kernel<0, false>, cudaFuncAttributeMaxDynamicSharedMemorySize, (int)s3_smem_bytes());
  cudaFuncSetAttribute(scan3d_build_kernel<0, true>, cudaFuncAttributeMaxDynamicSharedMemorySize, (int)s3_smem_bytes());
  cudaFuncSetAttribute(scan3d_build_kernel<1, true>, cudaFuncAttributeMaxDynamicSharedMemorySize, (int)s3_smem_bytes());
}

void launch_scan3d_cells(const SweepParams &p, cudaStream_t s) {
  const unsigned grid = (unsigned)((i64)p.nsx * p.nsy * p.nsz);
  switch (p.sum_mode) {
    case SUM_BUILD: scan3d_build_kernel<0, false><<<grid, F3_CW * 32, s3_smem_bytes(), s>>>(p); break;
    case SUM_BUILD_TEST1: scan3d_build_kernel<0, true><<<grid, F3_CW * 32, s3_smem_bytes(), s>>>(p); break;
    case SUM_BUILD_TEST2: scan3d_build_kernel<1, true><<<grid, F3_CW * 32, s3_smem_bytes(), s>>>(p); break;
    case SUM_TEST1: scan3d_cells_kernel<1><<<grid, F3_CW * 32, 0, s>>>(p); break;
    default: scan3d_cells_kernel<2><<<grid, F3_CW * 32, 0, s>>>(p); break;
  }
}

void launch_scan(const SweepParams &p, cudaStream_t s) {
  const unsigned grid = p.nd == 2 ? (unsigned)(((i64)p.nsx * p.nsy + 7) / 8) : (unsigned)((i64)p.nsx * p.nsy * p.nsz);
  if (p.nd == 2 && p.fused) {
    if (p.has_next) scan2d_fused_kernel<true><<<grid, 256, 0, s>>>(p);
    else scan2d_fused_kernel<false><<<grid, 256, 0, s>>>(p);
  } else if (p.nd == 2) {
    if (p.has_next) scan2d_kernel<true><<<grid, 256, 0, s>>>(p);
    else scan2d_kernel<false><<<grid, 256, 0, s>>>(p);
  } else {
    const dim3 block(32, SCAN3_BY);
    if (p.has_next) scan3d_kernel<true><<<grid, block, 0, s>>>(p);
    else scan3d_kernel<false><<<grid, block, 0, s>>>(p);
  }
}

__device__ __forceinline__ int sgn(i64 v) { return (v > 0) - (v < 0); }
__device__ __forceinline__ u64 U(i64 v) { return (u64)v; }

__device__ __forceinline__ i64 det3_h(i64 a0, i64 a1, i64 b0, i64 b1, i64 c0, i64 c1) {
  return (i64)(U(a0) * (U(b1) - U(c1)) - U(a1) * (U(b0) - U(c0)) + (U(b0) * U(c1) - U(b1) * U(c0)));
}

__device__ __forceinline__ i64 det4_h(const i64 X[4][3]) {
  u64 d[3][3];
#pragma unroll
  for (int i = 0; i < 3; i++)
#pragma unroll
    for (int j = 0; j < 3; j++) d[i][j] = U(X[i + 1][j]) - U(X[0][j]);
  const u64 det = d[0][0] * (d[1][1] * d[2][2] - d[1][2] * d[2][1])
                - d[0][1] * (d[1][0] * d[2][2] - d[1][2] * d[2][0])
                + d[0][2] * (d[1][0] * d[2][1] - d[1][1] * d[2][0]);
  return (i64)(0 - det);
}

__device__ int sos_sign3(const i64 X[3][2]) {
  int s = sgn(det3_h(X[0][0], X[0][1], X[1][0], X[1][1], X[2][0], X[2][1]));
  if (s) return s;
  s = -sgn((i64)(U(X[1][0]) - U(X[2][0])));
  if (s) return s;
  s = sgn((i64)(U(X[1][1]) - U(X[2][1])));
  if (s) return s;
  s = sgn((i64)(U(X[0][0]) - U(X[2][0])));
  if (s) return s;
  return 1;
}

__device__ int sos_sign4(const i64 X[4][3]) {
  int s = sgn(det4_h(X));
  if (s) return s;
#define D3(r0, r1, r2, c0, c1) det3_h(X[r0][c0], X[r0][c1], X[r1][c0], X[r1][c1], X[r2][c0], X[r2][c1])
#define D2(r0, r1, c) ((i64)(U(X[r0][c]) - U(X[r1][c])))
  s = sgn(D3(1, 2, 3, 0, 1)); if (s) return s;
  s = -sgn(D3(1, 2, 3, 0, 2)); if (s) return s;
  s = sgn(D3(1, 2, 3, 1, 2)); if (s) return s;
  s = -sgn(D3(0, 2, 3, 0, 1)); if (s) return s;
  s = sgn(D2(2, 3, 0)); if (s) return s;
  s = -sgn(D2(2, 3, 1)); if (s) return s;
  s = sgn(D3(0, 2, 3, 0, 2)); if (s) return s;
  s = sgn(D2(2, 3, 2)); if (s) return s;
  s = -sgn(D3(0, 2, 3, 1, 2)); if (s) return s;
  s = sgn(D3(0, 1, 3, 0, 1)); if (s) return s;
  s = -sgn(D2(1, 3, 0)); if (s) return s;
  s = sgn(D2(1, 3, 1)); if (s) return s;
  s = sgn(D2(0, 3, 0)); if (s) return s;
#undef D3
#undef D2
  return 1;
}

template <int NV, int NC>
__device__ int oriented_sign(const i64 Xin[NV][NC], const int idx_in[NV]) {
  int idx[NV], ord[NV];
#pragma unroll
  for (int i = 0; i < NV; i++) { idx[i] = idx_in[i]; ord[i] = i; }
  int swaps = 0;
#pragma unroll
  for (int i = 0; i < NV - 1; i++)
#pragma unroll
    for (int j = 0; j < NV - 1 - i; j++)
      if (idx[j] > idx[j + 1]) {
        int t = idx[j]; idx[j] = idx[j + 1]; idx[j + 1] = t;
        t = ord[j]; ord[j] = ord[j + 1]; ord[j + 1] = t;
        swaps++;
      }
  i64 X[NV][NC];
#pragma unroll
  for (int i = 0; i < NV; i++)
#pragma unroll
    for (int j = 0; j < NC; j++) {
      i64 v = 0;
#pragma unroll
      for (int q = 0; q < NV; q++) v = (ord[i] == q) ? Xin[q][j] : v;
      X[i][j] = v;
    }
  int s;
  if constexpr (NV == 3) s = sos_sign3(X);
  else s = sos_sign4(X);
  return (swaps & 1) ? -s : s;
}

template <int NV, int NC>
__device__ __noinline__ bool origin_in_simplex(const i64 X[NV][NC], const int idx[NV]) {
  const int s = oriented_sign<NV, NC>(X, idx);
#pragma unroll 1
  for (int i = 0; i < NV; i++) {
    i64 Y[NV][NC];
    int my[NV];
#pragma unroll
    for (int j = 0; j < NV; j++) {
      const bool rep = (j == i);
      my[j] = rep ? -1 : idx[j];
#pragma unroll
      for (int c = 0; c < NC; c++) Y[j][c] = rep ? 0 : X[j][c];
    }
    if (oriented_sign<NV, NC>(Y, my) != s) return false;
  }
  return true;
}

__device__ __forceinline__ bool usable_det(i64 v) { return v != 0 && v != LLONG_MIN; }

__device__ __forceinline__ bool origin_in_simplex_fast(const i64 X[3][2], const int idx[3]) {
  const u64 a0 = U(X[0][0]), a1 = U(X[0][1]), b0 = U(X[1][0]), b1 = U(X[1][1]), c0 = U(X[2][0]), c1 = U(X[2][1]);
  const i64 Da = (i64)(b0 * c1 - b1 * c0);
  const i64 Db = (i64)(a1 * c0 - a0 * c1);
  const i64 Dc = (i64)(a0 * b1 - a1 * b0);
  const i64 D = (i64)(U(Da) + U(Db) + U(Dc));
  if (usable_det(D) && usable_det(Da) && usable_det(Db) && usable_det(Dc)) {
    const bool pos = D > 0;
    return (Da > 0) == pos && (Db > 0) == pos && (Dc > 0) == pos;
  }
  return origin_in_simplex<3, 2>(X, idx);
}

__device__ __forceinline__ u64 det3_rows(const u64 r0[3], const u64 r1[3], const u64 r2[3]) {
  return r0[0] * (r1[1] * r2[2] - r1[2] * r2[1]) - r0[1] * (r1[0] * r2[2] - r1[2] * r2[0]) + r0[2] * (r1[0] * r2[1] - r1[1] * r2[0]);
}
// ... 904 lines not shown
```

### ftk_b200/csrc/kernels.h

```cpp
#pragma once
#include <cuda.h>
#include <cuda_runtime.h>
#include <cstdint>

#include "../../include/ftkb200.h"
#include "mesh_tables.h"

namespace ftkb {

struct LayerPtrs {
  const double *S;
  const double *V;
  const double *J;
};

struct SweepParams {
  int32_t nd;
  int32_t W, H, D;
  int32_t lb[3], ub[3];
  int32_t nc[3];
  int32_t vmax[3];
  int32_t voff[3], rank_lb[3], rank_nc[3];
  int32_t t;
  int32_t has_next;
  int32_t nbits;
  double factor;
  int32_t no_filter;
  int32_t scalar_source, jacobian_source, jacobian_symmetric, derived_symmetric;
  int32_t robust, compute_degrees, use_type_filter;
  uint32_t type_filter;
  LayerPtrs L[2];
  int32_t coords_mode, coords_ncomp;
  double coords_bounds[6];
  const double *coords;
  int32_t fused;
  int32_t keys2d;
  float thrp_f;
  float thr2_f;
  float lim_f;
  unsigned long long *res_slot[2];
  float res_thr[3];
  unsigned long long *poison;
  alignas(64) CUtensorMap tmap[2];
  int32_t sum_mode;
  int32_t build_layer;
  const uint4 *sum_in[2];
  uint4 *sum_out;
  int32_t nsx;
  int32_t nsy;
  int32_t nsz;
  int32_t rows;
  unsigned long long *wl_count;
  unsigned long long wl_cap;
  unsigned long long *wl;
  unsigned long long *pt_count;
  unsigned long long pt_cap;
  ftkb_point *pts;
  unsigned long long *step_out;
  unsigned long long step_seq;
  unsigned long long *ticket;
  unsigned long long *res_reset;
  int32_t test_blocks;
  int32_t sm_count;
};

inline float res_threshold_key(double R, double scale) {
  if (!(R < 0x1p1000) || !(scale > 0.0)) return __builtin_inff();
  const double T = R / scale;
  unsigned long long bits;
  __builtin_memcpy(&bits, &T, 8);
  const int hi = (int)(bits >> 32) + 2;
  float f;
  __builtin_memcpy(&f, &hi, 4);
  return f;
}

void upload_mesh_tables(const DeviceMeshTables &t2, const DeviceMeshTables &t3);
void init_kernel_attributes();

constexpr int F3_CW = 8;
constexpr int F3_RW = 4;
constexpr int F3_STRIDE = 62;
constexpr int F3_COLS = 68;
constexpr int F3_TROWS = F3_CW * F3_RW;
constexpr int F3_ROWS = F3_TROWS + 3;
bool encode_scalar_tmap3d(const double *S, int W, int H, int D, CUtensorMap *out);

void launch_scan(const SweepParams &p, cudaStream_t s);
enum { SUM_BUILD = 0,
       SUM_BUILD_TEST1 = 1,
       SUM_BUILD_TEST2 = 2,
       SUM_TEST1 = 3,
       SUM_TEST2 = 4 };
void launch_scan3d_cells(const SweepParams &p, cudaStream_t s);
size_t scan3d_cells_per_layer(const SweepParams &p);
constexpr int SCAN2D_CELL_ROWS = 9;
void launch_scan2d_cells(const SweepParams &p, cudaStream_t s);
size_t scan2d_cells_per_layer(const SweepParams &p);
constexpr int VSCAN2D_CELL_ROWS = 8;
void launch_vscan_cells(const SweepParams &p, cudaStream_t s);
size_t vscan2d_cells_per_layer(const SweepParams &p);
void launch_test(const SweepParams &p, cudaStream_t s);

void launch_gradient(int nd, const double *S, double *V, int W, int H, int D, unsigned long long *res_bits, cudaStream_t s);
void launch_resolution(const double *p, uint64_t n, unsigned long long *res_bits, cudaStream_t s);
void launch_fill_u64(unsigned long long *p, unsigned long long v, cudaStream_t s);
void launch_widen_f32(const float *in, double *out, uint64_t n, cudaStream_t s);

void launch_synthetic(int kind, int nd, int W, int H, int D, const double *params, double t, double *out, cudaStream_t s, int zoff = 0, int Dg = 0);

struct TraceParams {
  int32_t nd;
  int32_t lb[3], ub[3];
  int64_t ny, nz;
  uint64_t n;
  const unsigned long long *keys;
  const ftkb_point *pts;
  uint32_t *nb;
  int32_t *deg;
  uint32_t *parent_all;
  uint32_t *parent_ord;
};
constexpr int KEY_TYPE_BITS = 6;
constexpr int KEY_TIME_BITS = 22;

void launch_point_keys(const ftkb_point *pts, uint64_t n, const TraceParams &tp, unsigned long long *keys, uint32_t *idx, cudaStream_t s);
void launch_gather_points(const ftkb_point *src, const uint32_t *idx, uint64_t n, ftkb_point *dst, cudaStream_t s);
void launch_neighbors(const TraceParams &tp, cudaStream_t s);
void launch_union_find(const TraceParams &tp, cudaStream_t s);
void launch_batch_neighbors(const TraceParams &tp, const unsigned long long *n_ptr, uint64_t n_max, const ftkb_point *src, const uint32_t *idx,
                            ftkb_point *dst, uint32_t *nb9, uint8_t *cnt, cudaStream_t s);

size_t sort_pairs_u64(void *temp, size_t temp_bytes, const unsigned long long *kin, unsigned long long *kout,
                      const uint32_t *vin, uint32_t *vout, uint64_t n, cudaStream_t s);
size_t unique_by_key_u64(void *temp, size_t temp_bytes, const unsigned long long *kin, const uint32_t *vin,
                         unsigned long long *kout, uint32_t *vout, unsigned long long *n_out, uint64_t n, cudaStream_t s);

}
```

Measured before the change: 5597 billion.

## Pair consecutive 2D timesteps into one fused scan-build kernel launch

```diff
diff --git a/ftk_b200/csrc/context.cpp b/ftk_b200/csrc/context.cpp
--- a/ftk_b200/csrc/context.cpp
+++ b/ftk_b200/csrc/context.cpp
@@ -75,15 +75,20 @@
 
   unsigned long long *d_scalars = nullptr;
   unsigned long long *h_scalars = nullptr;
-  static constexpr int SLOT_WL = 8, SLOT_PT = 9, SLOT_UQ = 10, SLOT_POISON = 11, SLOT_WL2 = 12, SLOT_TICKET = 13, SLOT_POISON2 = 14, NSLOTS = 16;
+  static constexpr int SLOT_WL = 8, SLOT_PT = 9, SLOT_UQ = 10, SLOT_POISON = 11, SLOT_TICKET = 13, NSLOTS = 24, NARMED = 20;
+  static constexpr int NSETS = 4;
+  static constexpr int SLOT_WLS[NSETS] = {8, 12, 16, 17}, SLOT_POISONS[NSETS] = {11, 14, 18, 19};
 
   struct Pending {
     int ring = 0, evset = 0, pops = 0, nbits = 0, wl_sel = 0;
     uint64_t seq = 0, npts_before = 0, pt_cap = 0;
     bool has_next = false;
+    bool paired = false;
+    int test_after = -1;
     int res_slots[2] = {-1, -1};
   };
   bool defer = true;
+  bool held = false;
   std::deque<Pending> pend;
   std::deque<Layer> limbo;
   unsigned long long *h_ring = nullptr;
@@ -91,7 +96,7 @@
   uint64_t step_seq = 0;
   bool primed = false;
   int wl_sel = 0;
-  cudaEvent_t dev[2][3] = {{nullptr, nullptr, nullptr}, {nullptr, nullptr, nullptr}};
+  cudaEvent_t dev[NSETS][3] = {};
   bool push_d2h_outstanding = false;
   uint64_t wl_hint = 1 << 16;
   cudaEvent_t ev_input = nullptr;
@@ -106,8 +111,7 @@
   bool last_test_overlapped = false;
   bool has_producer = false;
 
-  unsigned long long *d_wl = nullptr;
-  unsigned long long *d_wl2 = nullptr;
+  unsigned long long *d_wls[NSETS] = {};
   int last_wl_sel = 0;
   uint64_t wl_cap = 0, last_wl = 0;
   ftkb_point *d_pts = nullptr;
@@ -259,8 +263,7 @@
   for (auto &es : c->dev) for (auto &e : es) if (e) cudaEventDestroy(e);
   if (c->ev_input) cudaEventDestroy(c->ev_input);
   if (c->dbg_prev) cudaEventDestroy(c->dbg_prev);
-  cudaFree(c->d_wl);
-  cudaFree(c->d_wl2);
+  for (auto *w : c->d_wls) cudaFree(w);
   if (c->stream2) { cudaStreamSynchronize(c->stream2); cudaStreamDestroy(c->stream2); }
   if (c->ev_join) cudaEventDestroy(c->ev_join);
   cudaFree(c->d_pts);
@@ -351,8 +354,8 @@
   cudaMemsetAsync(c->d_scalars, 0, sizeof(unsigned long long) * ftkb_ctx::NSLOTS, c->stream);
   c->wl_cap = std::max<uint64_t>(1 << 16, c->ncore / 64);
   if (const char *w = std::getenv("FTKB_WL_CAP")) c->wl_cap = std::max<uint64_t>(1, std::strtoull(w, nullptr, 10));
-  if ((e = cudaMalloc(&c->d_wl, sizeof(unsigned long long) * c->wl_cap)) != cudaSuccess) return bail("cudaMalloc(worklist) failed", FTKB_ERR_NOMEM);
-  if ((e = cudaMalloc(&c->d_wl2, sizeof(unsigned long long) * c->wl_cap)) != cudaSuccess) return bail("cudaMalloc(worklist) failed", FTKB_ERR_NOMEM);
+  for (auto &w : c->d_wls)
+    if ((e = cudaMalloc(&w, sizeof(unsigned long long) * c->wl_cap)) != cudaSuccess) return bail("cudaMalloc(worklist) failed", FTKB_ERR_NOMEM);
   {
     int lo = 0, hi = 0;
     cudaDeviceGetStreamPriorityRange(&lo, &hi);
@@ -563,7 +566,7 @@
 
 extern "C" int ftkb_set_resolution(ftkb_ctx *c, double res) {
   if (!c) return FTKB_ERR_INVALID;
-  if (!c->pend.empty()) {
+  if (!c->pend.empty() || c->held) {
     cudaSetDevice(c->cfg.device);
     const int rc = drain(c);
     if (rc) return rc;
@@ -738,7 +741,7 @@
       p.res_slot[0] = c->d_scalars + l.slot;
       p.poison = c->d_scalars + ftkb_ctx::SLOT_POISON;
       p.wl_count = c->d_scalars + ftkb_ctx::SLOT_WL;
-      p.wl = c->d_wl; p.wl_cap = 0;
+      p.wl = c->d_wls[0]; p.wl_cap = 0;
       vcells_decomposition(c, p);
       const int rc = ensure_cells(c, l, p);
       if (rc) return rc;
@@ -773,7 +776,7 @@
   p.L[0].S = l.S; p.L[1].S = l.S;
   p.res_slot[0] = c->d_scalars + l.slot;
   p.wl_count = c->d_scalars + ftkb_ctx::SLOT_WL;
-  p.wl = c->d_wl; p.wl_cap = 0;
+  p.wl = c->d_wls[0]; p.wl_cap = 0;
   if (c->n == 3) {
     p.nbits = 8;
     p.poison = c->d_scalars + ftkb_ctx::SLOT_POISON;
@@ -896,7 +899,7 @@
   return FTKB_OK;
 }
 
-static int update_impl(ftkb_ctx *c, bool allow_defer);
+static int update_impl(ftkb_ctx *c, bool allow_defer, bool may_hold);
 static int abandon_fused3d(ftkb_ctx *c);
 
 static void absorb_resolutions(ftkb_ctx *c, const ftkb_ctx::Pending &pd) {
@@ -941,7 +944,7 @@
   }
   c->stats.sweeps_repeated += pops.size();
   for (size_t i = 0; i < pops.size(); i++) {
-    const int rc = update_impl(c, false);
+    const int rc = update_impl(c, false, false);
     if (rc) return rc;
     for (int j = 0; j < pops[i] && !c->layers.empty(); j++) {
       release_layer(c, c->layers.front());
@@ -969,7 +972,8 @@
   c->factor = (double)(uint64_t)(1 << pd.nbits);
   float ms_scan = 0, ms_test = 0;
   CK(cudaEventElapsedTime(&ms_scan, c->dev[pd.evset][0], c->dev[pd.evset][1]));
-  CK(cudaEventElapsedTime(&ms_test, c->dev[pd.evset][1], c->dev[pd.evset][2]));
+  CK(cudaEventElapsedTime(&ms_test, pd.test_after >= 0 ? c->dev[pd.test_after][2] : c->dev[pd.evset][1], c->dev[pd.evset][2]));
+  if (pd.paired) ms_scan /= 2;
   c->stats.ms_scan += ms_scan; c->stats.ms_test += ms_test; c->stats.last_ms_scan = ms_scan;
   if (c->debug_timing) {
     float s0 = 0, s1 = 0, s2 = 0;
@@ -1002,7 +1006,32 @@
   return FTKB_OK;
 }
 
+static void pop_front_layer(ftkb_ctx *c) {
+  if (c->layers.empty()) return;
+  if (c->held || !c->pend.empty()) {
+    c->limbo.push_back(c->layers.front());
+    if (!c->held) c->pend.back().pops++;
+  } else {
+    release_layer(c, c->layers.front());
+  }
+  c->layers.pop_front();
+}
+
+static int flush_held(ftkb_ctx *c) {
+  if (!c->held) return FTKB_OK;
+  c->held = false;
+  c->layers.push_front(c->limbo.back());
+  c->limbo.pop_back();
+  c->current_timestep--;
+  const int rc = update_impl(c, c->defer, false);
+  if (rc) return rc;
+  pop_front_layer(c);
+  c->current_timestep++;
+  return FTKB_OK;
+}
+
 static int drain(ftkb_ctx *c) {
+  { const int rc = flush_held(c); if (rc) return rc; }
   while (!c->pend.empty()) {
     const int rc = confirm_front(c);
     if (rc) return rc;
@@ -1041,10 +1070,10 @@
 
 extern "C" int ftkb_update_timestep(ftkb_ctx *c) {
   if (!c) return FTKB_ERR_INVALID;
-  return update_impl(c, c->defer);
-}
-
-static int update_impl(ftkb_ctx *c, bool allow_defer) {
+  return update_impl(c, c->defer, false);
+}
+
+static int update_impl(ftkb_ctx *c, bool allow_defer, bool may_hold) {
   if (c->layers.empty()) return fail(c, FTKB_ERR_INVALID, "update_timestep: no snapshot has been pushed");
   CK(cudaSetDevice(c->cfg.device));
   bool may_defer = allow_defer && !c->streaming && !c->push_d2h_outstanding;
@@ -1124,7 +1153,7 @@
     if (!encode_scalar_tmap3d(lay[0]->S, p.W, p.H, p.D, &p.tmap[0]) || !encode_scalar_tmap3d(lay[1]->S, p.W, p.H, p.D, &p.tmap[1])) {
       int rc = drain(c);
       if (!rc) rc = abandon_fused3d(c);
-      return rc ? rc : update_impl(c, allow_defer);
+      return rc ? rc : update_impl(c, allow_defer, may_hold);
     }
     fused3d_decomposition(c, p);
   } else if (fused) {
@@ -1150,7 +1179,26 @@
   const bool cells_path = vcells || (fused && (c->n == 3 || aligned));
   void (*launch_cells)(const SweepParams &, cudaStream_t) = vcells ? launch_vscan_cells : (c->n == 3 ? launch_scan3d_cells : launch_scan2d_cells);
 
-  if (may_defer && cells_path && lay[0]->cells_valid && !p.no_filter) {
+  const bool pairable = c->n == 2 && fused && aligned && c->keys2d && has_next && !lay[1]->cells_valid && !lay[1]->cells_foreign &&
+                        p.rows <= SCAN2D_PAIR_MAX_ROWS
+#ifdef FTKB_EXP_NOPAIR
+                        && false
+#endif
+                        ;
+  if (c->held && !(may_defer && cells_path && pairable)) {
+    const int rc = flush_held(c);
+    return rc ? rc : update_impl(c, allow_defer, may_hold);
+  }
+  if (may_defer && cells_path && (lay[0]->cells_valid || c->held) && !p.no_filter) {
+    if (!c->held && may_hold && pairable) {
+      c->held = true;
+      return FTKB_OK;
+    }
+    const bool pair = c->held;
+    c->held = false;
+    const int nsteps = pair ? 2 : 1;
+    struct Step { Layer *l0, *l1; int t; } steps[2] = {{lay[0], lay[1], p.t}, {lay[0], lay[1], p.t}};
+    if (pair) steps[0] = Step{&c->limbo.back(), lay[0], p.t - 1};
     if (has_next && !lay[1]->cells) {
       const int rc0 = ensure_cells(c, *lay[1], p);
       if (rc0) return rc0;
@@ -1161,68 +1209,86 @@
     p.thr2_f = (float)(2.0 / p.factor);
     p.lim_f = (float)(0.999 * 4.5e18 / (p.factor * p.factor));
     const auto te0 = std::chrono::steady_clock::now();
-    ftkb_ctx::Pending pd;
-    pd.seq = ++c->step_seq;
-    pd.ring = (int)(pd.seq % ftkb_ctx::RING);
-    pd.evset = (int)(pd.seq & 1);
-    pd.has_next = has_next;
-    pd.nbits = nbits;
-    pd.npts_before = c->npts;
-    p.res_slot[0] = p.res_slot[1] = nullptr;
-    for (int k = 0; k < (has_next ? 2 : 1); k++)
-      if (lay[k]->res_pending) {
-        p.res_slot[k] = c->d_scalars + lay[k]->slot;
-        pd.res_slots[k] = lay[k]->slot;
-        lay[k]->res_pending = false;
-      }
-    pd.wl_sel = c->wl_sel;
-    p.wl = c->wl_sel ? c->d_wl2 : c->d_wl; p.wl_cap = c->wl_cap;
     { const int rcg = grow_points_ahead(c); if (rcg) return rcg; }
     p.pts = c->d_pts; p.pt_cap = c->pt_cap;
-    pd.pt_cap = c->pt_cap;
-    p.wl_count = c->d_scalars + (c->wl_sel ? ftkb_ctx::SLOT_WL2 : ftkb_ctx::SLOT_WL);
-    p.poison = c->d_scalars + (c->wl_sel ? ftkb_ctx::SLOT_POISON2 : ftkb_ctx::SLOT_POISON);
-    p.step_out = c->h_ring + 8 * pd.ring;
-    p.step_seq = pd.seq;
-    auto slot_at = [&](size_t idx) { return idx < c->layers.size() ? c->layers[idx].slot : (int)((c->next_slot + (idx - c->layers.size())) % 8); };
-    p.res_reset = c->d_scalars + slot_at(3);
     if (!c->primed) {
-      c->h_scalars[ftkb_ctx::SLOT_WL] = 0;
-      c->h_scalars[ftkb_ctx::SLOT_WL2] = 0;
+      for (int k = 0; k < ftkb_ctx::NSETS; k++) { c->h_scalars[ftkb_ctx::SLOT_WLS[k]] = 0; c->h_scalars[ftkb_ctx::SLOT_POISONS[k]] = 0; }
       c->h_scalars[ftkb_ctx::SLOT_PT] = c->npts;
       c->h_scalars[ftkb_ctx::SLOT_UQ] = 0;
-      c->h_scalars[ftkb_ctx::SLOT_POISON] = 0;
-      c->h_scalars[ftkb_ctx::SLOT_POISON2] = 0;
       c->h_scalars[ftkb_ctx::SLOT_TICKET] = 0;
-      if (c->layers.size() < 3) c->h_scalars[slot_at(2)] = ~0ull;
-      CK(cudaMemcpyAsync(c->d_scalars, c->h_scalars, 15 * sizeof(unsigned long long), cudaMemcpyHostToDevice, c->stream));
-    }
-    CK(cudaEventRecord(c->dev[pd.evset][0], c->stream));
-    p.sum_in[0] = lay[0]->cells; p.sum_in[1] = lay[1]->cells;
-    if (has_next && !lay[1]->cells_valid) {
-      p.sum_mode = SUM_BUILD_TEST2; p.build_layer = 1; p.sum_out = lay[1]->cells;
+      const size_t nres = c->layers.size() + (pair ? 1 : 0);
+      for (size_t d = nres; d <= 4; d++) c->h_scalars[(steps[0].l0->slot + d) % 8] = ~0ull;
+      CK(cudaMemcpyAsync(c->d_scalars, c->h_scalars, ftkb_ctx::NARMED * sizeof(unsigned long long), cudaMemcpyHostToDevice, c->stream));
+    }
+    SweepParams ps[2];
+    ftkb_ctx::Pending pds[2];
+    for (int i = 0; i < nsteps; i++) {
+      SweepParams &q = ps[i];
+      ftkb_ctx::Pending &pd = pds[i];
+      const Step &st = steps[i];
+      q = p;
+      q.t = st.t;
+      q.L[0] = LayerPtrs{st.l0->S, st.l0->V, st.l0->J};
+      q.L[1] = LayerPtrs{st.l1->S, st.l1->V, st.l1->J};
+      pd.seq = ++c->step_seq;
+      pd.ring = (int)(pd.seq % ftkb_ctx::RING);
+      pd.evset = (int)(pd.seq % ftkb_ctx::NSETS);
+      pd.has_next = has_next;
+      pd.nbits = nbits;
+      pd.npts_before = c->npts;
+      pd.pt_cap = c->pt_cap;
+      pd.paired = pair;
+      pd.pops = pair && i == 0 ? 1 : 0;
+      if (pair && i == 1) pd.test_after = pds[0].evset;
+      q.res_slot[0] = q.res_slot[1] = nullptr;
+      Layer *lk[2] = {st.l0, st.l1};
+      for (int k = 0; k < (has_next ? 2 : 1); k++)
+        if (lk[k]->res_pending) {
+          q.res_slot[k] = c->d_scalars + lk[k]->slot;
+          pd.res_slots[k] = lk[k]->slot;
+          lk[k]->res_pending = false;
+        }
+      pd.wl_sel = c->wl_sel;
+      c->wl_sel = (c->wl_sel + 1) % ftkb_ctx::NSETS;
+      q.wl = c->d_wls[pd.wl_sel]; q.wl_cap = c->wl_cap;
+      q.wl_count = c->d_scalars + ftkb_ctx::SLOT_WLS[pd.wl_sel];
+      q.poison = c->d_scalars + ftkb_ctx::SLOT_POISONS[pd.wl_sel];
+      q.step_out = c->h_ring + 8 * pd.ring;
+      q.step_seq = pd.seq;
+      q.res_reset = c->d_scalars + (st.l0->slot + 5) % 8;
+      q.sum_in[0] = st.l0->cells; q.sum_in[1] = st.l1->cells;
+      if (has_next && !st.l1->cells_valid) {
+        q.sum_mode = SUM_BUILD_TEST2; q.build_layer = 1; q.sum_out = st.l1->cells;
+      } else {
+        q.sum_mode = has_next ? SUM_TEST2 : SUM_TEST1;
+      }
+    }
+    for (int i = 0; i < nsteps; i++) CK(cudaEventRecord(c->dev[pds[i].evset][0], c->stream));
+    if (pair) {
+      launch_scan2d_pair(ps[0], ps[1], c->stream);
       lay[1]->cells_valid = true;
     } else {
-      p.sum_mode = has_next ? SUM_TEST2 : SUM_TEST1;
-    }
-    launch_cells(p, c->stream);
-    CK(cudaEventRecord(c->dev[pd.evset][1], c->stream));
+      launch_cells(ps[0], c->stream);
+      if (ps[0].sum_mode == SUM_BUILD_TEST2) lay[1]->cells_valid = true;
+    }
+    for (int i = 0; i < nsteps; i++) CK(cudaEventRecord(c->dev[pds[i].evset][1], c->stream));
     const bool overlap = c->wl_hint < 100000;
     if (!overlap && c->last_test_overlapped && !c->pend.empty())
       CK(cudaStreamWaitEvent(c->stream, c->dev[c->pend.back().evset][2], 0));
     c->last_test_overlapped = overlap;
     cudaStream_t ts = overlap ? c->stream2 : c->stream;
-    if (overlap) CK(cudaStreamWaitEvent(c->stream2, c->dev[pd.evset][1], 0));
-    launch_test(p, ts);
-    CK(cudaEventRecord(c->dev[pd.evset][2], ts));
-    c->stats.kernel_launches += 2;
+    if (overlap) CK(cudaStreamWaitEvent(c->stream2, c->dev[pds[0].evset][1], 0));
+    for (int i = 0; i < nsteps; i++) {
+      launch_test(ps[i], ts);
+      CK(cudaEventRecord(c->dev[pds[i].evset][2], ts));
+    }
+    c->stats.kernel_launches += 1 + nsteps;
     const int rc = check_launch(c, "sweep");
     if (rc) return rc;
-    c->pend.push_back(pd);
+    for (int i = 0; i < nsteps; i++) c->pend.push_back(pds[i]);
     c->primed = true;
-    c->wl_sel ^= 1;
     if (c->debug_timing) { c->host_enq_us += std::chrono::duration<double, std::micro>(std::chrono::steady_clock::now() - te0).count(); c->host_enq_n++; }
-    while (c->pend.size() > 1) {
+    while (c->pend.size() > (size_t)nsteps) {
       const int rc2 = confirm_front(c);
       if (rc2) return rc2;
     }
@@ -1244,17 +1310,15 @@
     if (fused || vcells)
       for (int k = 0; k < (has_next ? 2 : 1); k++)
         if (lay[k]->res_pending) { p.res_slot[k] = c->d_scalars + lay[k]->slot; pending = true; }
-    p.wl = c->d_wl; p.wl_cap = c->wl_cap;
+    p.wl = c->d_wls[0]; p.wl_cap = c->wl_cap;
     p.pts = c->d_pts; p.pt_cap = c->pt_cap;
     p.test_blocks = test_grid(c);
     c->h_scalars[ftkb_ctx::SLOT_WL] = 0;
     c->h_scalars[ftkb_ctx::SLOT_PT] = c->npts;
     c->h_scalars[ftkb_ctx::SLOT_UQ] = 0;
     c->h_scalars[ftkb_ctx::SLOT_POISON] = 0;
-    c->h_scalars[ftkb_ctx::SLOT_WL2] = 0;
     c->h_scalars[ftkb_ctx::SLOT_TICKET] = 0;
-    c->h_scalars[ftkb_ctx::SLOT_POISON2] = 0;
-    CK(cudaMemcpyAsync(c->d_scalars, c->h_scalars, 15 * sizeof(unsigned long long), cudaMemcpyHostToDevice, c->stream));
+    CK(cudaMemcpyAsync(c->d_scalars, c->h_scalars, 14 * sizeof(unsigned long long), cudaMemcpyHostToDevice, c->stream));
     CK(cudaEventRecord(c->ev[0], c->stream));
     if (cells_path) {
       int rc0 = ensure_cells(c, *lay[0], p);
@@ -1300,18 +1364,18 @@
       c->stats.sweeps_repeated++;
       c->cellsV = false;
       for (Layer &l : c->layers) l.cells_valid = false;
-      return update_impl(c, false);
+      return update_impl(c, false, false);
     }
     if (fused && c->n == 3 && c->h_scalars[ftkb_ctx::SLOT_POISON]) {
       c->stats.sweeps_repeated++;
       const int rc2 = abandon_fused3d(c);
-      return rc2 ? rc2 : update_impl(c, false);
+      return rc2 ? rc2 : update_impl(c, false, false);
     }
     if (fused && c->n == 2 && c->h_scalars[ftkb_ctx::SLOT_POISON]) {
       c->stats.sweeps_repeated++;
       c->keys2d = false;
       for (Layer &l : c->layers) l.cells_valid = false;
-      return update_impl(c, false);
+      return update_impl(c, false, false);
     }
     float ms_scan = 0, ms_test = 0;
     CK(cudaEventElapsedTime(&ms_scan, c->ev[0], c->ev[1]));
@@ -1334,11 +1398,12 @@
     const uint64_t nwl = c->h_scalars[ftkb_ctx::SLOT_WL], npt = c->h_scalars[ftkb_ctx::SLOT_PT];
     c->wl_hint = std::min<uint64_t>(nwl, c->wl_cap);
     if (nwl > c->wl_cap) {
-      cudaFree(c->d_wl); cudaFree(c->d_wl2);
-      c->d_wl = c->d_wl2 = nullptr;
       c->wl_cap = nwl + nwl / 8 + 1024;
-      CK(cudaMalloc(&c->d_wl, sizeof(unsigned long long) * c->wl_cap));
-      CK(cudaMalloc(&c->d_wl2, sizeof(unsigned long long) * c->wl_cap));
+      for (auto &w : c->d_wls) {
+        cudaFree(w);
+        w = nullptr;
+        CK(cudaMalloc(&w, sizeof(unsigned long long) * c->wl_cap));
+      }
       c->wl_hint = nwl;
       c->stats.sweeps_repeated++;
       continue;
@@ -1367,17 +1432,9 @@
 
 extern "C" int ftkb_advance_timestep(ftkb_ctx *c) {
   if (!c) return FTKB_ERR_INVALID;
-  const int rc = ftkb_update_timestep(c);
+  const int rc = update_impl(c, c->defer, true);
   if (rc) return rc;
-  if (!c->layers.empty()) {
-    if (!c->pend.empty()) {
-      c->limbo.push_back(c->layers.front());
-      c->pend.back().pops++;
-    } else {
-      release_layer(c, c->layers.front());
-    }
-    c->layers.pop_front();
-  }
+  pop_front_layer(c);
   c->current_timestep++;
   return FTKB_OK;
 }
@@ -1826,7 +1883,7 @@
   const uint64_t have = std::min<uint64_t>(c->last_wl, c->wl_cap);
   *n = have;
   const uint64_t m = std::min(have, cap);
-  if (m) CK(cudaMemcpy(out, c->last_wl_sel ? c->d_wl2 : c->d_wl, sizeof(uint64_t) * m, cudaMemcpyDeviceToHost));
+  if (m) CK(cudaMemcpy(out, c->d_wls[c->last_wl_sel], sizeof(uint64_t) * m, cudaMemcpyDeviceToHost));
   return FTKB_OK;
 }
 
@@ -1897,7 +1954,7 @@
 
 extern "C" int ftkb_get_stats(ftkb_ctx *c, ftkb_stats *out) {
   if (!c || !out) return FTKB_ERR_INVALID;
-  if (!c->pend.empty()) {
+  if (!c->pend.empty() || c->held) {
     cudaSetDevice(c->cfg.device);
     const int rc = drain(c);
     if (rc) return rc;
@@ -1911,7 +1968,7 @@
 
 extern "C" int ftkb_reset_stats(ftkb_ctx *c) {
   if (!c) return FTKB_ERR_INVALID;
-  if (!c->pend.empty()) {
+  if (!c->pend.empty() || c->held) {
     cudaSetDevice(c->cfg.device);
     const int rc = drain(c);
     if (rc) return rc;
@@ -1935,6 +1992,7 @@
 extern "C" int ftkb_timer_start(ftkb_ctx *c) {
   if (!c) return FTKB_ERR_INVALID;
   CK(cudaSetDevice(c->cfg.device));
+  { const int rc = flush_held(c); if (rc) return rc; }
   CK(cudaEventRecord(c->ev[6], c->stream));
   return FTKB_OK;
 }
@@ -1942,6 +2000,7 @@
 extern "C" int ftkb_timer_stop(ftkb_ctx *c, double *ms) {
   if (!c || !ms) return FTKB_ERR_INVALID;
   CK(cudaSetDevice(c->cfg.device));
+  { const int rc = flush_held(c); if (rc) return rc; }
   CK(cudaEventRecord(c->ev_join, c->stream2));
   CK(cudaStreamWaitEvent(c->stream, c->ev_join, 0));
   CK(cudaEventRecord(c->ev[7], c->stream));
diff --git a/ftk_b200/csrc/kernels.cu b/ftk_b200/csrc/kernels.cu
--- a/ftk_b200/csrc/kernels.cu
+++ b/ftk_b200/csrc/kernels.cu
@@ -665,6 +665,8 @@
 constexpr uint32_t K2_ROW_BYTES = C2_SEG * 8;
 constexpr uint32_t K2_STAGE_BYTES = K2_R * K2_ROW_BYTES;
 static_assert(C2_R % K2_R == 0, "cell block = whole stages");
+constexpr uint32_t K2_KEEP_STRIDE = 16u * 32u * C2_CW;
+static_assert(SCAN2D_PAIR_MAX_ROWS % C2_R == 0, "whole cell blocks");
 
 __device__ __forceinline__ double2 lds128_f64(uint32_t a) {
   double2 v;
@@ -688,6 +690,9 @@
   return v;
 }
 __device__ __forceinline__ void sts64_f64(uint32_t a, double v) { asm volatile("st.shared.f64 [%0], %1;" ::"r"(a), "d"(v) : "memory"); }
+__device__ __forceinline__ void sts128_u32(uint32_t a, uint4 v) {
+  asm volatile("st.shared.v4.u32 [%0], {%1, %2, %3, %4};" ::"r"(a), "r"(v.x), "r"(v.y), "r"(v.z), "r"(v.w) : "memory");
+}
 __device__ __forceinline__ float fmax_nan(float a, float b) {
   float r;
   asm("max.NaN.f32 %0, %1, %2;" : "=f"(r) : "f"(a), "f"(b));
@@ -713,7 +718,7 @@
 
 struct K2Acc { double mdx, mdy; float big; };
 
-template <bool BORDER, int NPREV, bool TEST>
+template <bool BORDER, int NPREV, bool TEST, int HALF>
 __device__ __forceinline__ K2Acc keys2d_strip(const SweepParams &p, const int c0, const int r0, const int r1, const int lane,
                                            const uint32_t tile_u32 ,
                                            const uint32_t full0, const uint32_t empty0, const int strip,
@@ -721,7 +726,9 @@
                                            const uint32_t res_u32 ,
                                            const uint32_t wl_stage ,
                                            const uint32_t cell_stage ,
+                                           const uint32_t keep_u32 ,
                                            const K2Acc acc) {
+  constexpr bool PREV_HBM = NPREV && HALF != 2;
   float big = acc.big;
   const int W = p.W, H = p.H, B = p.build_layer;
   const int e = c0 + 2 * lane, o = e + 1;
@@ -733,8 +740,8 @@
   const double cw = (double)(W - 1), ch = (double)(H - 1);
   const bool want_res = p.res_slot[B] != nullptr;
   const float thrx = p.res_thr[0], thry = p.res_thr[1];
-  const uint4 *sum_prev = NPREV ? p.sum_in[0] + cells2d_index(p, strip, 0, lane) : nullptr;
-  uint4 *sum_out = p.sum_out + cells2d_index(p, strip, 0, lane);
+  const uint4 *sum_prev = PREV_HBM ? p.sum_in[0] + cells2d_index(p, strip, 0, lane) : nullptr;
+  uint4 *sum_out = HALF == 1 ? nullptr : p.sum_out + cells2d_index(p, strip, 0, lane);
   const uint32_t lane_u32 = tile_u32 + (uint32_t)lane * 16u;
   const int kb0 = r0 / C2_R;
   unsigned long long failbits = 0;
@@ -744,11 +751,13 @@
     xmn = fminf(xmn, __shfl_down_sync(0xffffffffu, xmn, 1)); xmx = fmaxf(xmx, __shfl_down_sync(0xffffffffu, xmx, 1));
     ymn = fminf(ymn, __shfl_down_sync(0xffffffffu, ymn, 1)); ymx = fmaxf(ymx, __shfl_down_sync(0xffffffffu, ymx, 1));
     FRange bx = k2_vrange(xmn, xmx, cw), by = k2_vrange(ymn, ymx, ch);
-    sum_out[(size_t)kb * 32u] = make_uint4(__float_as_uint(bx.mn), __float_as_uint(bx.mx), __float_as_uint(by.mn), __float_as_uint(by.mx));
+    const uint4 cell = make_uint4(__float_as_uint(bx.mn), __float_as_uint(bx.mx), __float_as_uint(by.mn), __float_as_uint(by.mx));
+    if (HALF == 1) sts128_u32(keep_u32 + (uint32_t)(kb - kb0) * K2_KEEP_STRIDE, cell);
+    else sum_out[(size_t)kb * 32u] = cell;
     if (TEST) {
       if (NPREV && kb < kb_end) {
-        cp_async_wait_all();
-        const uint4 prevc = lds128_u32(cell_stage + ((uint32_t)kb & 1u) * 512u);
+        if (PREV_HBM) cp_async_wait_all();
+        const uint4 prevc = lds128_u32(PREV_HBM ? cell_stage + ((uint32_t)kb & 1u) * 512u : keep_u32 + (uint32_t)(kb - kb0) * K2_KEEP_STRIDE);
         bx = fmerge(bx, FRange{__uint_as_float(prevc.x), __uint_as_float(prevc.y)});
         by = fmerge(by, FRange{__uint_as_float(prevc.z), __uint_as_float(prevc.w)});
       }
@@ -814,8 +823,8 @@
   float bxmn = 0.f, bxmx = 0.f, bymn = 0.f, bymx = 0.f;
   const uint4 nanc = make_uint4(0x7FC00000u, 0x7FC00000u, 0x7FC00000u, 0x7FC00000u);
   int kb = r0 / C2_R;
-  if (NPREV && kb < kb_end) prefetch_l2(sum_prev + (size_t)kb * 32u);
-  if (NPREV && kb + 1 < kb_end) prefetch_l2(sum_prev + (size_t)(kb + 1) * 32u);
+  if (PREV_HBM && kb < kb_end) prefetch_l2(sum_prev + (size_t)kb * 32u);
+  if (PREV_HBM && kb + 1 < kb_end) prefetch_l2(sum_prev + (size_t)(kb + 1) * 32u);
 
   int gphase = 0;
   static_assert(C2_R == 3 * K2_R, "a cell block is three groups");
@@ -841,9 +850,9 @@
         const float rxmn = fminf(kxe, kxo), rxmx = fmaxf(kxe, kxo), rymn = fminf(kye, kyo), rymx = fmaxf(kye, kyo);
         if (j > r0) finish_block(kb - 1, fminf(bxmn, rxmn), fmaxf(bxmx, rxmx), fminf(bymn, rymn), fmaxf(bymx, rymx));
         bxmn = rxmn; bxmx = rxmx; bymn = rymn; bymx = rymx;
-        if (NPREV && kb < kb_end) cp_async16(cell_stage + ((uint32_t)kb & 1u) * 512u, sum_prev + (size_t)kb * 32u);
+        if (PREV_HBM && kb < kb_end) cp_async16(cell_stage + ((uint32_t)kb & 1u) * 512u, sum_prev + (size_t)kb * 32u);
         kb++;
-        if (NPREV && kb + 1 < kb_end) prefetch_l2(sum_prev + (size_t)(kb + 1) * 32u);
+        if (PREV_HBM && kb + 1 < kb_end) prefetch_l2(sum_prev + (size_t)(kb + 1) * 32u);
       } else {
         bxmn = fminf(fminf(bxmn, kxe), kxo); bxmx = fmaxf(fmaxf(bxmx, kxe), kxo);
         bymn = fminf(fminf(bymn, kye), kyo); bymx = fmaxf(fmaxf(bymx, kye), kyo);
@@ -882,16 +891,22 @@
   return K2Acc{lds64_f64(res_u32), lds64_f64(res_u32 + 8u), big};
 }
 
-template <int NPREV, bool TEST>
-__global__ void __launch_bounds__((C2_CW + 1) * 32, K2_CTAS) scan2d_keys_build_kernel(const __grid_constant__ SweepParams p) {
+template <int N> struct SweepSteps { SweepParams s[N]; };
+
+template <int NPREV, bool TEST, int NSTEPS>
+__global__ void __launch_bounds__((C2_CW + 1) * 32, K2_CTAS) scan2d_keys_build_kernel(const __grid_constant__ SweepSteps<NSTEPS> ps) {
+  static_assert(NSTEPS == 1 || (NSTEPS == 2 && NPREV == 1 && TEST), "a pair builds and tests both of its new layers");
   extern __shared__ __align__(128) unsigned char fb_smem[];
+  const SweepParams &p = ps.s[0];
   const int lane = threadIdx.x & 31;
   const int wib = __shfl_sync(0xffffffffu, (int)(threadIdx.x >> 5), 0);
   const uint32_t ring0 = smem_u32(fb_smem);
   const uint32_t full0 = ring0 + (uint32_t)K2_NST * K2_STAGE_BYTES, empty0 = full0 + 8u * K2_NST;
   const uint32_t res_u32 = empty0 + 8u * K2_NST + 16u * threadIdx.x;
   const uint32_t wl_stage = empty0 + 8u * K2_NST + 16u * (C2_CW + 1) * 32u + 32u + WL_STAGE_BYTES * (uint32_t)wib;
-  const uint32_t cell_stage = empty0 + 8u * K2_NST + 16u * (C2_CW + 1) * 32u + 32u + WL_STAGE_BYTES * (uint32_t)C2_CW + 1024u * (uint32_t)wib + 16u * (uint32_t)lane;
+  const uint32_t cells_u32 = empty0 + 8u * K2_NST + 16u * (C2_CW + 1) * 32u + 32u + WL_STAGE_BYTES * (uint32_t)C2_CW;
+  const uint32_t cell_stage = cells_u32 + 1024u * (uint32_t)wib + 16u * (uint32_t)lane;
+  const uint32_t keep_u32 = cells_u32 + 1024u * (uint32_t)C2_CW + 16u * (uint32_t)(wib * 32 + lane);
   const int W = p.W, H = p.H;
   const int bx = blockIdx.x % p.nsx, cy = blockIdx.x / p.nsx;
   const int C0 = bx * (C2_CW * FB_STRIDE);
@@ -908,18 +923,22 @@
   const int nstages = ((r1 + 1) - r0 + 1 + 2 + K2_R - 1) / K2_R;
   if (wib == C2_CW) {
     if (elect_one()) {
-      const double *S = p.L[p.build_layer].S;
       const int col_lo = max(C0 - 2, 0), col_hi = min(C0 - 2 + C2_SEG, W);
       const uint32_t seg_bytes = (uint32_t)(col_hi - col_lo) * 8u;
       const uint32_t dst0 = ring0 + (uint32_t)(col_lo - (C0 - 2)) * 8u;
-      for (int s = 0; s < nstages; s++) {
-        const uint32_t slot = (uint32_t)s % K2_NST;
-        if (s >= K2_NST) mbar_wait(empty0 + 8u * slot, (uint32_t)((s / K2_NST - 1) & 1));
-        mbar_expect_tx(full0 + 8u * slot, seg_bytes * K2_R);
-#pragma unroll
-        for (int i = 0; i < K2_R; i++) {
-          const size_t off = (size_t)W * (size_t)clampi(r0 - 1 + K2_R * s + i, H) + (size_t)col_lo;
-          bulk_g2s(dst0 + slot * K2_STAGE_BYTES + (uint32_t)i * K2_ROW_BYTES, S + off, seg_bytes, full0 + 8u * slot);
+#pragma unroll
+      for (int h = 0; h < NSTEPS; h++) {
+        const double *S = ps.s[h].L[ps.s[h].build_layer].S;
+        for (int s = 0; s < nstages; s++) {
+          const int gs = h * nstages + s;
+          const uint32_t slot = (uint32_t)gs % K2_NST;
+          if (gs >= K2_NST) mbar_wait(empty0 + 8u * slot, (uint32_t)((gs / K2_NST - 1) & 1));
+          mbar_expect_tx(full0 + 8u * slot, seg_bytes * K2_R);
+#pragma unroll
+          for (int i = 0; i < K2_R; i++) {
+            const size_t off = (size_t)W * (size_t)clampi(r0 - 1 + K2_R * s + i, H) + (size_t)col_lo;
+            bulk_g2s(dst0 + slot * K2_STAGE_BYTES + (uint32_t)i * K2_ROW_BYTES, S + off, seg_bytes, full0 + 8u * slot);
+          }
         }
       }
     }
@@ -929,22 +948,34 @@
   const int c0 = C0 + wib * FB_STRIDE;
   const uint32_t tile_u32 = ring0 + (uint32_t)(wib * FB_STRIDE) * 8u;
   const bool border = c0 == 0 || c0 + FB_SEG - 2 > W;
-  K2Acc acc{DBL_MAX, DBL_MAX, 0.f};
-  sts64_f64(res_u32, DBL_MAX); sts64_f64(res_u32 + 8u, DBL_MAX);
-  if (lane == 0) asm volatile("st.shared.s32 [%0], %1;" ::"r"(wl_stage), "r"(0) : "memory");
-  __syncwarp();
-  if (border) acc = keys2d_strip<true, NPREV, TEST>(p, c0, r0, r1, lane, tile_u32, full0, empty0, bx * C2_CW + wib, 0u, res_u32, wl_stage, cell_stage, acc);
-  else acc = keys2d_strip<false, NPREV, TEST>(p, c0, r0, r1, lane, tile_u32, full0, empty0, bx * C2_CW + wib, 0u, res_u32, wl_stage, cell_stage, acc);
-  if (p.res_slot[p.build_layer] != nullptr) {
-    const double cw = (double)(W - 1), ch = (double)(H - 1);
-    const double ax = fabs(acc.mdx), ay = fabs(acc.mdy);
-    const double vx = ax < DBL_MAX ? ax * cw : DBL_MAX, vy = ay < DBL_MAX ? ay * ch : DBL_MAX;
-    warp_res_commit(fmin(vx > 0.0 ? vx : DBL_MAX, vy > 0.0 ? vy : DBL_MAX), p.res_slot[p.build_layer]);
-  }
-  if (!(acc.big < __int_as_float(KEYF_BIG))) atomicExch(p.poison, 1ull);
-}
-
-static size_t k2_smem_bytes() { return (size_t)K2_NST * K2_STAGE_BYTES + (size_t)2 * K2_NST * 8 + (size_t)16 * (C2_CW + 1) * 32 + 32 + (size_t)WL_STAGE_BYTES * C2_CW + (size_t)1024 * C2_CW; }
+  auto sweep = [&](auto HC, const SweepParams &q, const uint32_t sbase) {
+    constexpr int HALF = decltype(HC)::value;
+    K2Acc acc{DBL_MAX, DBL_MAX, 0.f};
+    sts64_f64(res_u32, DBL_MAX); sts64_f64(res_u32 + 8u, DBL_MAX);
+    if (lane == 0) asm volatile("st.shared.s32 [%0], %1;" ::"r"(wl_stage), "r"(0) : "memory");
+    __syncwarp();
+    if (border) acc = keys2d_strip<true, NPREV, TEST, HALF>(q, c0, r0, r1, lane, tile_u32, full0, empty0, bx * C2_CW + wib, sbase, res_u32, wl_stage, cell_stage, keep_u32, acc);
+    else acc = keys2d_strip<false, NPREV, TEST, HALF>(q, c0, r0, r1, lane, tile_u32, full0, empty0, bx * C2_CW + wib, sbase, res_u32, wl_stage, cell_stage, keep_u32, acc);
+    if (q.res_slot[q.build_layer] != nullptr) {
+      const double cw = (double)(W - 1), ch = (double)(H - 1);
+      const double ax = fabs(acc.mdx), ay = fabs(acc.mdy);
+      const double vx = ax < DBL_MAX ? ax * cw : DBL_MAX, vy = ay < DBL_MAX ? ay * ch : DBL_MAX;
+      warp_res_commit(fmin(vx > 0.0 ? vx : DBL_MAX, vy > 0.0 ? vy : DBL_MAX), q.res_slot[q.build_layer]);
+    }
+    if (!(acc.big < __int_as_float(KEYF_BIG))) atomicExch(q.poison, 1ull);
+  };
+  if constexpr (NSTEPS == 1) {
+    sweep(IC<0>{}, p, 0u);
+  } else {
+    sweep(IC<1>{}, p, 0u);
+    sweep(IC<2>{}, ps.s[NSTEPS - 1], (uint32_t)nstages);
+  }
+}
+
+static size_t k2_smem_bytes(int nsteps = 1, int rows = 0) {
+  return (size_t)K2_NST * K2_STAGE_BYTES + (size_t)2 * K2_NST * 8 + (size_t)16 * (C2_CW + 1) * 32 + 32 + (size_t)WL_STAGE_BYTES * C2_CW +
+         (size_t)1024 * C2_CW + (nsteps == 2 ? (size_t)(rows / C2_R) * K2_KEEP_STRIDE : 0);
+}
 static size_t c2_smem_bytes() { return (size_t)C2_NST * C2_SEG * 8 + (size_t)2 * C2_NST * 8; }
 
 size_t scan2d_cells_per_layer(const SweepParams &p) {
@@ -957,9 +988,9 @@
   const unsigned tgrid = (unsigned)(((i64)nstrips * nblk + 7) / 8);
   if (p.keys2d && p.sum_mode <= SUM_BUILD_TEST2) {
     switch (p.sum_mode) {
-      case SUM_BUILD: scan2d_keys_build_kernel<0, false><<<grid, (C2_CW + 1) * 32, k2_smem_bytes(), s>>>(p); break;
-      case SUM_BUILD_TEST1: scan2d_keys_build_kernel<0, true><<<grid, (C2_CW + 1) * 32, k2_smem_bytes(), s>>>(p); break;
-      default: scan2d_keys_build_kernel<1, true><<<grid, (C2_CW + 1) * 32, k2_smem_bytes(), s>>>(p); break;
+      case SUM_BUILD: scan2d_keys_build_kernel<0, false, 1><<<grid, (C2_CW + 1) * 32, k2_smem_bytes(), s>>>(SweepSteps<1>{{p}}); break;
+      case SUM_BUILD_TEST1: scan2d_keys_build_kernel<0, true, 1><<<grid, (C2_CW + 1) * 32, k2_smem_bytes(), s>>>(SweepSteps<1>{{p}}); break;
+      default: scan2d_keys_build_kernel<1, true, 1><<<grid, (C2_CW + 1) * 32, k2_smem_bytes(), s>>>(SweepSteps<1>{{p}}); break;
     }
     return;
   }
@@ -970,6 +1001,11 @@
     case SUM_TEST1: scan2d_cells_kernel<1><<<tgrid, 256, 0, s>>>(p, nstrips, nblk); break;
     default: scan2d_cells_kernel<2><<<tgrid, 256, 0, s>>>(p, nstrips, nblk); break;
   }
+}
+
+void launch_scan2d_pair(const SweepParams &a, const SweepParams &b, cudaStream_t s) {
+  const unsigned grid = (unsigned)((i64)a.nsx * a.nsy);
+  scan2d_keys_build_kernel<1, true, 2><<<grid, (C2_CW + 1) * 32, k2_smem_bytes(2, a.rows), s>>>(SweepSteps<2>{{a, b}});
 }
 
 constexpr int F3_LAYER_BYTES = ((F3_ROWS * F3_COLS * 8 + 127) / 128) * 128;
@@ -1802,9 +1838,19 @@
   cudaFuncSetAttribute(scan2d_build_kernel<0, false>, cudaFuncAttributeMaxDynamicSharedMemorySize, (int)c2_smem_bytes());
   cudaFuncSetAttribute(scan2d_build_kernel<0, true>, cudaFuncAttributeMaxDynamicSharedMemorySize, (int)c2_smem_bytes());
   cudaFuncSetAttribute(scan2d_build_kernel<1, true>, cudaFuncAttributeMaxDynamicSharedMemorySize, (int)c2_smem_bytes());
-  cudaFuncSetAttribute(scan2d_keys_build_kernel<0, false>, cudaFuncAttributeMaxDynamicSharedMemorySize, (int)k2_smem_bytes());
-  cudaFuncSetAttribute(scan2d_keys_build_kernel<0, true>, cudaFuncAttributeMaxDynamicSharedMemorySize, (int)k2_smem_bytes());
-  cudaFuncSetAttribute(scan2d_keys_build_kernel<1, true>, cudaFuncAttributeMaxDynamicSharedMemorySize, (int)k2_smem_bytes());
+  cudaFuncSetAttribute(scan2d_keys_build_kernel<0, false, 1>, cudaFuncAttributeMaxDynamicSharedMemorySize, (int)k2_smem_bytes());
+  cudaFuncSetAttribute(scan2d_keys_build_kernel<0, true, 1>, cudaFuncAttributeMaxDynamicSharedMemorySize, (int)k2_smem_bytes());
+  cudaFuncSetAttribute(scan2d_keys_build_kernel<1, true, 1>, cudaFuncAttributeMaxDynamicSharedMemorySize, (int)k2_smem_bytes());
+  cudaFuncSetAttribute(scan2d_keys_build_kernel<1, true, 2>, cudaFuncAttributeMaxDynamicSharedMemorySize, (int)k2_smem_bytes(2, SCAN2D_PAIR_MAX_ROWS));
+#ifndef FTKB_EXP_NOCARVE
+  cudaFuncSetAttribute(scan2d_keys_build_kernel<1, true, 2>, cudaFuncAttributePreferredSharedMemoryCarveout, (int)cudaSharedmemCarveoutMaxShared);
+#endif
+#ifdef FTKB_EXP_OCC
+  { int n1 = 0, n2 = 0;
+    cudaOccupancyMaxActiveBlocksPerMultiprocessor(&n1, scan2d_keys_build_kernel<1, true, 1>, (C2_CW + 1) * 32, k2_smem_bytes());
+    cudaOccupancyMaxActiveBlocksPerMultiprocessor(&n2, scan2d_keys_build_kernel<1, true, 2>, (C2_CW + 1) * 32, k2_smem_bytes(2, SCAN2D_PAIR_MAX_ROWS));
+    fprintf(stderr, "[occ] single %d pair %d smem %zu %zu\n", n1, n2, k2_smem_bytes(), k2_smem_bytes(2, SCAN2D_PAIR_MAX_ROWS)); }
+#endif
   cudaFuncSetAttribute(scan3d_build_kernel<0, false>, cudaFuncAttributeMaxDynamicSharedMemorySize, (int)s3_smem_bytes());
   cudaFuncSetAttribute(scan3d_build_kernel<0, true>, cudaFuncAttributeMaxDynamicSharedMemorySize, (int)s3_smem_bytes());
   cudaFuncSetAttribute(scan3d_build_kernel<1, true>, cudaFuncAttributeMaxDynamicSharedMemorySize, (int)s3_smem_bytes());
diff --git a/ftk_b200/csrc/kernels.h b/ftk_b200/csrc/kernels.h
--- a/ftk_b200/csrc/kernels.h
+++ b/ftk_b200/csrc/kernels.h
@@ -96,6 +96,8 @@
 size_t scan3d_cells_per_layer(const SweepParams &p);
 constexpr int SCAN2D_CELL_ROWS = 9;
 void launch_scan2d_cells(const SweepParams &p, cudaStream_t s);
+constexpr int SCAN2D_PAIR_MAX_ROWS = 45;
+void launch_scan2d_pair(const SweepParams &a, const SweepParams &b, cudaStream_t s);
 size_t scan2d_cells_per_layer(const SweepParams &p);
 constexpr int VSCAN2D_CELL_ROWS = 8;
 void launch_vscan_cells(const SweepParams &p, cudaStream_t s);
```

New measurement: 5123 billion (median of 6 runs). -8.5%, worse.
